# uci-rendering/psdr-cuda

Hardware: AMD Instinct MI355X
Metric: Mpath-samples/s renderC+renderD, cbox 512x512 spp=64; grad rel-L2 vs ref (higher is better)
Workload: dtype f32; 1 GPU; cbox 512x512 spp=64/GPU PathTracer(max_depth=3): renderC + configure + renderD + enoki.forward w.r.t. diffuse albedo, through the psdr_cuda surface; triangles=12, global_spp=64, world_size=1, device=AMD Radeon Graphics, local_rank=0

## Files before the change

### __graft_entry__.py

```python
import os
import subprocess
import sys

ROOT = os.path.dirname(os.path.abspath(__file__))
PKG = os.path.join(ROOT, "psdr-cuda_amd")
for p in (PKG, os.path.join(ROOT, "oracle"), os.path.join(ROOT, "tests")):
    if p not in sys.path:
        sys.path.insert(0, p)

HIPCC_FLAGS = ["--offload-arch=gfx950", "-O3", "-std=c++17", "-fPIC", "-munsafe-fp-atomics",
               "-fno-hip-fp32-correctly-rounded-divide-sqrt", "-fgpu-flush-denormals-to-zero", "-fno-slp-vectorize",
               "-freciprocal-math", "-fapprox-func"]
VARIANTS = (0, 1, 2, 3, 4, 6, 8, 10)


def _stale(target, sources):
    return (not os.path.exists(target)) or any(os.path.getmtime(s) > os.path.getmtime(target) for s in sources)


def build():
    csrc = os.path.join(PKG, "csrc")
    srcs = [os.path.join(csrc, f) for f in os.listdir(csrc)] + [os.path.join(ROOT, "include", "psdr_hip.h")]
    lib = os.path.join(PKG, "lib", "libpsdr_hip.so")
    os.makedirs(os.path.dirname(lib), exist_ok=True)
    defect_job = None
    if _stale(lib, srcs):
        obj_dir = os.path.join(PKG, "lib", "obj")
        os.makedirs(obj_dir, exist_ok=True)
        jobs, objs, unit_cmds = [], [], {}
        for v in VARIANTS:
            o = os.path.join(obj_dir, "variant%d.o" % v)
            objs.append(o)
            unit_cmds[o] = ["hipcc"] + HIPCC_FLAGS + ["-DPSDR_VARIANT_FLAGS=%d" % v, "-c", os.path.join(csrc, "psdr_variant.hip"), "-o", o]
            jobs.append(subprocess.Popen(unit_cmds[o]))
            o = os.path.join(obj_dir, "path_sedge%d.o" % v)
            objs.append(o)
            unit_cmds[o] = ["hipcc"] + HIPCC_FLAGS + ["-DPSDR_VARIANT_FLAGS=%d" % v, "-c", os.path.join(csrc, "psdr_path_sedge.hip"), "-o", o]
            jobs.append(subprocess.Popen(unit_cmds[o]))
        o = os.path.join(obj_dir, "logd_lean.o")
        objs.append(o)
        unit_cmds[o] = ["hipcc"] + HIPCC_FLAGS + ["-c", os.path.join(csrc, "psdr_logd_lean.hip"), "-o", o]
        jobs.append(subprocess.Popen(unit_cmds[o]))
        o = os.path.join(obj_dir, "host.o")
        objs.append(o)
        unit_cmds[o] = ["hipcc"] + HIPCC_FLAGS + ["-c", os.path.join(csrc, "psdr_hip.hip"), "-o", o]
        jobs.append(subprocess.Popen(unit_cmds[o]))
        o = os.path.join(obj_dir, "tables.o")
        objs.append(o)
        unit_cmds[o] = ["hipcc"] + HIPCC_FLAGS + ["-c", os.path.join(csrc, "psdr_tables.hip"), "-o", o]
        jobs.append(subprocess.Popen(unit_cmds[o]))
        defect_job = _start_defect_object(csrc, obj_dir)
        if any(j.wait() != 0 for j in jobs):
            raise RuntimeError("hipcc failed")
        sys.path.insert(0, os.path.join(ROOT, "tools"))
        import check_spill_exec
        fallbacks = (["-mllvm", "-amdgpu-opt-exec-mask-pre-ra=0"], ["-mllvm", "-amdgpu-spill-sgpr-to-vgpr=0"])
        from concurrent.futures import ThreadPoolExecutor
        with ThreadPoolExecutor(max_workers=8) as pool:
            first = dict(zip(unit_cmds, pool.map(lambda o_: check_spill_exec.check_library(o_, verbose=True, min_code_objects=1), list(unit_cmds))))
        for o, cmd in list(unit_cmds.items()):
            hits = first[o]
            for extra in fallbacks:
                if not hits:
                    break
                print("build(): %s trips the spill guard -- rebuilding it with %s" % (os.path.basename(o), " ".join(extra)))
                subprocess.check_call(cmd[:1] + cmd[1:-4] + extra + cmd[-4:])
                hits = check_spill_exec.check_library(o, verbose=True, min_code_objects=1)
            if hits:
                raise RuntimeError("%s: %d kernel(s) spill in front of an exec restore with every fallback (tools/check_spill_exec.py)" % (os.path.basename(o), len(hits)))
        subprocess.check_call(["hipcc", "--offload-arch=gfx950", "-shared", "-fPIC"] + objs + ["-o", lib])
        if len(check_spill_exec.code_objects(lib)) < len(objs):
            raise RuntimeError("the linked library holds fewer gfx code objects than translation units: the spill guard cannot see all of it")
    subprocess.check_call(["make", "-C", os.path.join(ROOT, "oracle"), "-s"])
    hc_dir = os.path.join(ROOT, "tests", "hostcheck")
    hc = os.path.join(hc_dir, "libhostcheck.so")
    if _stale(hc, srcs + [os.path.join(hc_dir, "hostcheck.cpp")]):
        subprocess.check_call(["hipcc", "--offload-arch=gfx950", "-O2", "-std=c++17", "-fPIC", "-shared", "-pthread",
                               os.path.join(hc_dir, "hostcheck.cpp"), "-o", hc])
    hp = os.path.join(hc_dir, "libhostcheck_path_sedge.so")
    if _stale(hp, srcs + [os.path.join(hc_dir, "hostcheck_path_sedge.cpp")]):
        subprocess.check_call(["hipcc", "--offload-arch=gfx950", "-O2", "-std=c++17", "-fPIC", "-shared", "-pthread",
                               os.path.join(hc_dir, "hostcheck_path_sedge.cpp"), "-o", hp])
    po_dir = os.path.join(ROOT, "tests", "poison")
    po = os.path.join(po_dir, "libpoison.so")
    if _stale(po, [os.path.join(po_dir, "poison.hip")]):
        subprocess.check_call(["hipcc", "--offload-arch=gfx950", "-O1", "-fPIC", "-shared", os.path.join(po_dir, "poison.hip"), "-o", po])
    try:
        build_defect_lib(defect_job)
    except Exception as e:
        print("build(): tests/poison/libpsdr_hip_defect.so not built (%s) -- only tests/test_rough_rev_order_gpu.py uses it" % e)
    import psdr_cuda
    from psdr_cuda import _abi
    _abi.load_hip()
    import oracle
    oracle.load_oracle()


def _defect_object_cmd(csrc, obj_dir):
    return ["hipcc"] + HIPCC_FLAGS + ["-DPSDR_VARIANT_FLAGS=10", "-DPSDR_SINK_REG_PRIV_ROUGH=1", "-DPSDR_DPP_ALWAYS=1", "-c",
                                      os.path.join(csrc, "psdr_variant.hip"), "-o", os.path.join(obj_dir, "variant10_defect.o")]


def _start_defect_object(csrc, obj_dir):
    try:
        return subprocess.Popen(_defect_object_cmd(csrc, obj_dir), stdout=subprocess.DEVNULL, stderr=subprocess.DEVNULL)
    except Exception:
        return None


def build_defect_lib(object_job=None):
    csrc = os.path.join(PKG, "csrc")
    srcs = [os.path.join(csrc, f) for f in os.listdir(csrc)] + [os.path.join(ROOT, "include", "psdr_hip.h")]
    obj_dir = os.path.join(PKG, "lib", "obj")
    defect_lib = os.path.join(ROOT, "tests", "poison", "libpsdr_hip_defect.so")
    objs = [os.path.join(obj_dir, "%s%d.o" % (unit, v)) for v in VARIANTS for unit in ("variant", "path_sedge")] + [os.path.join(obj_dir, "logd_lean.o"), os.path.join(obj_dir, "host.o"), os.path.join(obj_dir, "tables.o")]
    if not all(os.path.exists(o) for o in objs):
        return None
    if object_job is not None and object_job.wait() != 0:
        object_job = None
    if _stale(defect_lib, srcs + objs):
        defect_obj = os.path.join(obj_dir, "variant10_defect.o")
        if object_job is None:
            subprocess.check_call(_defect_object_cmd(csrc, obj_dir))
        subprocess.check_call(["hipcc", "--offload-arch=gfx950", "-shared", "-fPIC"] + [defect_obj if o.endswith("variant10.o") else o for o in objs] + ["-o", defect_lib])
    return defect_lib


def smoke():
    import numpy as np
    import torch
    assert torch.cuda.is_available(), "smoke() needs a GPU"
    torch.cuda.set_device(0)
    import oracle
    from helpers import GpuScene, load_scene, rel_l2, tangents_wrt
    from psdr_cuda import _abi
    sc, P = load_scene("cbox", res=32, spp=8, sppe=4, sppse=4, translate=(0, (1.0, 0.0, 0.0)))
    tb = sc.tables(0)
    g = GpuScene(tb)
    o = _abi.make_opts(integrator=_abi.INTEGRATOR_PATH, max_depth=3, spp=8)
    img = g.render_c(o)
    ref = oracle.render(tb, o)
    assert np.isfinite(img).all() and rel_l2(img, ref) < 1e-4, rel_l2(img, ref)
    o = _abi.make_opts(spp=8, sppe=4, sppse=4)
    tan = tangents_wrt(tb, P)
    img, dimg = g.render_d_fwd(o, [tan])
    rimg, rd = oracle.render(tb, o, mode=1, tangents=tan)
    assert rel_l2(img, rimg) < 1e-4 and rel_l2(dimg[0], rd) < 1e-3, (rel_l2(img, rimg), rel_l2(dimg[0], rd))
    import psdr_cuda
    from psdr_cuda.fixtures import scene_path
    s2 = psdr_cuda.Scene()
    s2.load_file(scene_path("cbox"), False)
    s2.opts.width = s2.opts.height = 32
    s2.opts.spp, s2.opts.sppe, s2.opts.sppse, s2.opts.log_level = 4, 0, 0, 0
    s2.configure()
    out = psdr_cuda.DirectIntegrator(1, 1).renderC(s2).numpy()
    assert out.shape == (32 * 32, 3) and np.isfinite(out).all() and out.mean() > 0.05
    print("smoke OK: renderC rel-L2 vs oracle %.2e" % rel_l2(img, rimg))


if __name__ == "__main__":
    build()
    if len(sys.argv) > 1 and sys.argv[1] == "smoke":
        smoke()
    if len(sys.argv) > 1 and sys.argv[1] == "defect":
        print(build_defect_lib())
```

### include/psdr_hip.h

```cpp
#ifndef PSDR_HIP_H
#define PSDR_HIP_H

#include <stdint.h>

#ifdef __cplusplus
extern "C" {
#endif

#define PSDR_TRI_STRIDE   24
#define PSDR_TRIUV_STRIDE  8
#define PSDR_SEDGE_STRIDE 16
#define PSDR_PEDGE_STRIDE  8
#define PSDR_BSDF_STRIDE  16
#define PSDR_EMITTER_F_STRIDE 8
#define PSDR_EMITTER_I_STRIDE 4
#define PSDR_CAM_WORDS    64
#define PSDR_ENV_WORDS    32

#define PSDR_TRI_FACE_NORMALS 0x40000000

#define PSDR_BSDF_DIFFUSE        0
#define PSDR_BSDF_ROUGHCONDUCTOR 1
#define PSDR_SLOT_REFLECTANCE 0
#define PSDR_SLOT_ALPHA_U     1
// ... 32 lines not shown
    const float   *tri_info;
    const float   *tri_uv;
    const int32_t *tri_mesh;
    const int32_t *mesh_bsdf;
    const int32_t *mesh_emitter;
    const int32_t *bsdf_rec;
    const float   *texels;
    const float   *emitter_f;
    const int32_t *emitter_i;
    const float   *face_cmf, *face_pmf;
    const float   *emitter_cmf, *emitter_pmf;
    float          emitter_sum;
    const float   *cam;
    const float   *sec_edge;
    const float   *sec_cmf, *sec_pmf;
    float          sec_sum;
    const float   *prim_edge;
    const float   *prim_cmf, *prim_pmf;
    float          prim_sum;
    int32_t        guide_reso[3];
    const float   *guide_cmf, *guide_pmf;
    float          guide_sum;
    int32_t        env_emitter;
    int32_t        env_tex[3];
    int32_t        env_reso[2];
    const float   *env_f;
    const float   *env_cmf, *env_pmf;
    float          env_sum;
    uint32_t       material_mask;
    const int32_t *sec_edge_faces;
    const float   *prim_edge_z;
} psdr_scene_desc;

#define PSDR_FLAG_FUSED     1
#define PSDR_FLAG_WAVEFRONT 2
#define PSDR_FLAG_LITERAL_FORMS 4
#define PSDR_FLAG_KEEP_RECORDS 8
#define PSDR_FLAG_PATH_SEDGES 16
#define PSDR_PATH_SEDGES_MAX_DEPTH 8

typedef struct psdr_render_opts {
    int32_t integrator;
    int32_t bsdf_samples, light_samples;
    int32_t max_depth;
    int32_t hide_emitters;
    int32_t field;
    int32_t spp, sppe, sppse;
    int32_t spp_begin, spp_end;
    int32_t sppe_begin, sppe_end;
    int32_t sppse_begin, sppse_end;
    int32_t flags;
    uint64_t rng_offset[3];
} psdr_render_opts;

typedef struct psdr_tangents {
    const float *d_tri_info;
    const float *d_texels;
    const float *d_emitter_rad;
    const float *d_cam_to_world;
    const float *d_sec_edge;
    const float *d_prim_edge;
    const float *d_env_f;
} psdr_tangents;

typedef struct psdr_grads {
    float *g_tri_info;
    float *g_texels;
    float *g_emitter_rad;
    float *g_cam_to_world;
    float *g_sec_edge;
    float *g_prim_edge;
    float *g_env_f;
} psdr_grads;

typedef struct psdr_scene_s *psdr_scene_t;

const char *psdr_last_error(void);
const char *psdr_version(void);
int psdr_abi_struct_sizes(int32_t out[4]);

int psdr_scene_create(psdr_scene_t *out);
int psdr_scene_destroy(psdr_scene_t h);
int psdr_scene_set_option(psdr_scene_t h, const char *name, double value);

int psdr_scene_set_tables(psdr_scene_t h, const psdr_scene_desc *desc);

int psdr_bvh_build(psdr_scene_t h, void *stream);
int psdr_bvh_stats(psdr_scene_t h, int32_t out[4]);
int psdr_scene_info(psdr_scene_t h, int32_t out[8]);

int psdr_trace(psdr_scene_t h, int32_t m,
               const float *ox, const float *oy, const float *oz,
               const float *dx, const float *dy, const float *dz,
               const float *tmax,
               int32_t *out_shape, int32_t *out_tri, float *out_u, float *out_v,
               void *stream);

int psdr_render_c(psdr_scene_t h, const psdr_render_opts *opts,
                  float *out_img, void *stream);

int psdr_render_d_fwd(psdr_scene_t h, const psdr_render_opts *opts,
                      int32_t K, const psdr_tangents *tangents,
                      float *out_img, float *out_dimg, void *stream);

int psdr_render_d_rev(psdr_scene_t h, const psdr_render_opts *opts,
                      const float *adj_img, float *out_img,
                      const psdr_grads *grads, void *stream);

int psdr_guide_build(psdr_scene_t h, const psdr_render_opts *opts,
                     const int32_t reso[4], int32_t nrounds,
                     float *out_mass, void *stream);

int psdr_cube_sample_reuse(int32_t ndim, const int32_t *reso, const float *cmf, const float *pmf, float sum,
                           int32_t n, int32_t m, float *samples, float *out_pdf, void *stream);
int psdr_sample_boundary_segment_direct(const psdr_scene_desc *desc, int32_t m, const float *sample3,
                                        const uint8_t *active, float *out_p0, float *out_edge_dir,
                                        float *out_edge2, float *out_p2, float *out_n, float *out_pdf,
                                        uint8_t *out_valid, int32_t *out_edge, float *out_s1, void *stream);

int psdr_geo_world_vertices_fwd(int32_t V, const float *v_raw, const int32_t *vmesh, const float *mats, float *v_world, void *stream);
int psdr_geo_world_vertices_rev(int32_t V, const float *v_raw, const int32_t *vmesh, const float *mats, const float *v_world, const float *a_world, float *a_raw,
                                void *stream);
int psdr_geo_world_vertices_jvp(int32_t V, const float *v_raw, const int32_t *vmesh, const float *mats, const float *v_world, const float *t_raw, const float *t_mats,
                                float *t_world, void *stream);
int psdr_geo_tri_rows_fwd(int32_t V, int32_t T, const float *v, const int32_t *faces, float *vsum, float *rows, int32_t row_stride, void *stream);
int psdr_geo_tri_rows_rev(int32_t V, int32_t T, const float *v, const int32_t *faces, const float *vsum, const float *a_rows, int32_t row_stride,
                          float *a_vsum , float *a_v, void *stream);
int psdr_geo_tri_rows_jvp(int32_t V, int32_t T, const float *v, const int32_t *faces, const float *vsum, const float *t_v, int32_t row_stride,
                          float *t_vsum , float *t_rows, void *stream);
int psdr_geo_sec_edges_fwd(int32_t E, const int32_t *edges, const float *v, const float *rows, int32_t row_stride, float *info, uint8_t *keep, void *stream);
int psdr_geo_sec_edges_rev(int32_t E, const int32_t *edges, const float *a_info, float *a_v, float *a_rows, int32_t row_stride, void *stream);
int psdr_geo_sec_edges_jvp(int32_t E, const int32_t *edges, const float *t_v, const float *t_rows, int32_t row_stride, float *t_info, void *stream);
int psdr_geo_prim_edges_fwd(int32_t E, const int32_t *edges, const uint8_t *face_normals, const float *v, const float *rows, int32_t row_stride,
                            const float *cam22, float *rows8, float *z4, uint8_t *keep, void *stream);
int psdr_geo_prim_edges_rev(int32_t E, const int32_t *edges, const float *v, const float *cam22, const float *a_rows8, float *a_v, float *a_w2s ,
                            void *stream);
int psdr_geo_prim_edges_jvp(int32_t E, const int32_t *edges, const float *v, const float *cam22, const float *t_v, const float *t_w2s , float *t_rows8,
                            void *stream);

int psdr_geo_compact_edges_fwd(int32_t E, const float *rows, int32_t S, const uint8_t *keep, int32_t w0, int32_t wn, const void *aux, int32_t aux_stride, int32_t A,
                               void *scratch, float *rows_out, void *aux_out, int32_t *pos, float *pmf, float *cmf, float *header, void *stream);
int psdr_geo_compact_edges_rev(int32_t E, int32_t S, const int32_t *pos, const float *a_rows_out, float *a_rows, void *stream);
int psdr_geo_compact_edges_jvp(int32_t E, int32_t S, const int32_t *pos, const float *t_rows, float *t_rows_out, void *stream);
int psdr_geo_emitter_tables(int32_t M, const float *rows, int32_t row_stride, const int32_t *face_offset, const int32_t *mesh_emitter, int32_t Ne, const int32_t *emitter_i,
                            const float *radiance, const float *env_weight, float *mesh_area, float *emitter_f, float *emitter_pmf, float *emitter_cmf, float *face_pmf,
                            float *face_cmf, void *stream);

int psdr_scene_rev_layout(psdr_scene_t h, int32_t out[16]);

int psdr_scene_seed_info(psdr_scene_t h, int64_t out[4]);

int psdr_scene_logd_info(psdr_scene_t h, int64_t out[4]);

int psdr_get_counters(psdr_scene_t h, uint64_t out[4]);

#ifdef __cplusplus
}
#endif
#endif
```

### psdr-cuda_amd/csrc/psdr_bvh_build.h

```cpp
#pragma once
#include "psdr_device.h"

#include <algorithm>
#include <cmath>
#include <cstdlib>
#include <cstring>
#include <vector>

namespace psdr {

inline void pack_tiny_prims(const std::vector<float4> &tris, std::vector<float4> &prims) {
    const int n = (int) tris.size() / 3;
    std::vector<char> used((size_t) n, 0);
    struct V { float x[3]; bool operator==(const V &o) const { return x[0] == o.x[0] && x[1] == o.x[1] && x[2] == o.x[2]; } };
    auto vtx = [&](int t, int k) {
        const float4 &a = tris[(size_t) t * 3], &b = tris[(size_t) t * 3 + 1], &c = tris[(size_t) t * 3 + 2];
        V v{{a.x, a.y, a.z}};
        if (k == 1) { v.x[0] += b.x; v.x[1] += b.y; v.x[2] += b.z; }
        if (k == 2) { v.x[0] += c.x; v.x[1] += c.y; v.x[2] += c.z; }
        return v;
    };
    auto tri_id = [&](int t) { int32_t id; std::memcpy(&id, &tris[(size_t) t * 3].w, 4); return id; };
    auto map_code = [](const int c[3], int32_t &code) {
        static const int cs[4] = {0, 1, 0, 1}, ct[4] = {0, 0, 1, 1};
// ... 48 lines not shown
            std::memcpy(&a.w, &ids, 4); std::memcpy(&b.w, &code, 4); std::memcpy(&c.w, &code, 4);
            prims.push_back(a); prims.push_back(b); prims.push_back(c);
        }
    }
}

inline int tiny_plane_form(const std::vector<float4> &prims_in, float4 *rows, int32_t *meta, int32_t *aa_cnt_out = nullptr, bool allow_aa = true, std::vector<int> *row_of_prim = nullptr) {
    const int n = (int) prims_in.size() / 3;
    struct Aa { int axis; double c, cu, cv, hu, hv, S[4]; };
    auto bits = [](const float4 &r) { int32_t v; std::memcpy(&v, &r.w, 4); return v; };
    auto classify = [&](const float4 &a, const float4 &b, const float4 &c, Aa &o) {
        if (((uint32_t) bits(a) >> 16) == 0xffffu) return false;
        const double p0[3] = {a.x, a.y, a.z}, e1[3] = {b.x, b.y, b.z}, e2[3] = {c.x, c.y, c.z};
        int i1 = -1, i2 = -1, n1 = 0, n2 = 0;
        for (int k = 0; k < 3; ++k) { if (e1[k] != 0.0) { i1 = k; n1++; } if (e2[k] != 0.0) { i2 = k; n2++; } }
        if (n1 != 1 || n2 != 1 || i1 == i2) return false;
        for (int k = 0; k < 3; ++k) if (!std::isfinite(p0[k]) || !std::isfinite(e1[k]) || !std::isfinite(e2[k])) return false;
        o.axis = 3 - i1 - i2;
        const int ia = o.axis == 0 ? 1 : 0, ib = o.axis == 2 ? 1 : 2;
        double ctr[3];
        for (int k = 0; k < 3; ++k) ctr[k] = p0[k] + 0.5 * (e1[k] + e2[k]);
        o.c = p0[o.axis]; o.cu = ctr[ia]; o.cv = ctr[ib];
        o.hu = 0.5 * std::fabs(i1 == ia ? e1[ia] : e2[ia]); o.hv = 0.5 * std::fabs(i1 == ib ? e1[ib] : e2[ib]);
        if (i1 == ia) { o.S[0] = 1.0 / e1[i1]; o.S[1] = 0.0; o.S[2] = 0.0; o.S[3] = 1.0 / e2[i2]; }
        else          { o.S[0] = 0.0; o.S[1] = 1.0 / e1[i1]; o.S[2] = 1.0 / e2[i2]; o.S[3] = 0.0; }
        return true;
    };
    std::vector<int> row_of((size_t) n, -1); std::vector<Aa> aa((size_t) n);
    int cnt[3] = {0, 0, 0};
    if (allow_aa && aa_cnt_out)
        for (int i = 0; i < n; ++i) {
            Aa &q = aa[(size_t) i];
            if (classify(prims_in[(size_t) i * 3], prims_in[(size_t) i * 3 + 1], prims_in[(size_t) i * 3 + 2], q) && cnt[q.axis] < kAaPerAxis) row_of[(size_t) i] = q.axis * kAaPerAxis + cnt[q.axis]++;
        }
    const int n_aa = cnt[0] + cnt[1] + cnt[2];
    int next = n_aa > 0 ? kAaSlots : 0;
    for (int r = 0; r < next; ++r) { for (int q = 0; q < 4; ++q) { rows[r * 4 + q] = float4{0.f, 0.f, 0.f, 0.f}; meta[r * 4 + q] = 0; } rows[r * 4].w = -1.f; }
    if (aa_cnt_out) *aa_cnt_out = cnt[0] | (cnt[1] << 8) | (cnt[2] << 16);
    for (int src = 0; src < n; ++src) {
        const bool is_aa = row_of[(size_t) src] >= 0;
        const int i = is_aa ? row_of[(size_t) src] : next++;
        const float4 &a = prims_in[(size_t) src * 3], &b = prims_in[(size_t) src * 3 + 1], &c = prims_in[(size_t) src * 3 + 2];
        int32_t ids = bits(a), codeA = bits(b), codeB = bits(c);
        const float lim = ((uint32_t) ids >> 16) != 0xffffu ? 1.f : 0.f;
        if (is_aa) {
            const Aa &q = aa[(size_t) src];
            const double A = q.S[0] + q.S[2], B = q.S[1] + q.S[3];
            if (B < 0.0) { ids = (int32_t) (((uint32_t) ids >> 16) | ((uint32_t) ids << 16)); std::swap(codeA, codeB); }
            const float rho = (float) (A / B);
            int32_t packed; std::memcpy(&packed, &rho, 4); packed = (packed & ~15) | i;
            rows[i * 4] = float4{(float) q.c, (float) q.cu, (float) q.cv, (float) q.hu};
            rows[i * 4 + 1] = float4{(float) q.hv, 0.f, 0.f, 0.f};
            std::memcpy(&rows[i * 4 + 1].y, &packed, 4); std::memcpy(&rows[i * 4 + 1].w, &ids, 4);
            rows[i * 4 + 2] = float4{(float) q.S[0], (float) q.S[1], (float) q.S[2], (float) q.S[3]};
        } else {
            const double p0[3] = {a.x, a.y, a.z}, e1[3] = {b.x, b.y, b.z}, e2[3] = {c.x, c.y, c.z};
            double nn[3] = {e1[1] * e2[2] - e1[2] * e2[1], e1[2] * e2[0] - e1[0] * e2[2], e1[0] * e2[1] - e1[1] * e2[0]};
            const double len = std::sqrt(nn[0] * nn[0] + nn[1] * nn[1] + nn[2] * nn[2]);
            double a1[3] = {0, 0, 0}, a2[3] = {0, 0, 0};
            if (len > 0.0 && std::isfinite(len)) {
                for (int k = 0; k < 3; ++k) nn[k] /= len;
                const double x1[3] = {e2[1] * nn[2] - e2[2] * nn[1], e2[2] * nn[0] - e2[0] * nn[2], e2[0] * nn[1] - e2[1] * nn[0]};
                const double x2[3] = {nn[1] * e1[2] - nn[2] * e1[1], nn[2] * e1[0] - nn[0] * e1[2], nn[0] * e1[1] - nn[1] * e1[0]};
                for (int k = 0; k < 3; ++k) { a1[k] = x1[k] / len; a2[k] = x2[k] / len; }
            } else nn[0] = nn[1] = nn[2] = 0.0;
            auto dot3 = [](const double *x, const double *y) { return x[0] * y[0] + x[1] * y[1] + x[2] * y[2]; };
            rows[i * 4] = float4{(float) nn[0], (float) nn[1], (float) nn[2], (float) dot3(nn, p0)};
            rows[i * 4 + 1] = float4{(float) a1[0], (float) a1[1], (float) a1[2], (float) (dot3(a1, p0) + 0.5)};
            rows[i * 4 + 2] = float4{(float) a2[0], (float) a2[1], (float) a2[2], (float) (dot3(a2, p0) + 0.5)};
            rows[i * 4 + 3] = float4{lim, 0.f, 0.f, 0.f}; std::memcpy(&rows[i * 4 + 3].y, &ids, 4);
        }
        meta[i * 4] = ids; meta[i * 4 + 1] = codeA; meta[i * 4 + 2] = codeB;
        std::memcpy(&meta[i * 4 + 3], &lim, 4);
        if (row_of_prim) { row_of_prim->resize((size_t) n, -1); (*row_of_prim)[(size_t) src] = i; }
    }
    return next;
}

inline uint32_t tiny_emitter_rows(const int32_t *meta, int n_rows, int32_t aa_cnt, const std::vector<char> &is_emitter_tri) {
    const int cnt[3] = {aa_cnt & 255, (aa_cnt >> 8) & 255, aa_cnt >> 16};
    size_t want = 0, found = 0;
    for (char c : is_emitter_tri) want += c ? 1 : 0;
    uint32_t rows = 0;
    for (int i = 0; i < n_rows && i < 32; ++i) {
        if (aa_cnt != 0 && i < kAaSlots && (i % kAaPerAxis) >= cnt[i / kAaPerAxis]) continue;
        const uint32_t ids = (uint32_t) meta[i * 4];
        const uint32_t t[2] = {ids & 0xffffu, ids >> 16};
        for (int a = 0; a < 2; ++a)
            if (t[a] != 0xffffu && t[a] < is_emitter_tri.size() && is_emitter_tri[t[a]]) { rows |= 1u << i; found++; }
    }
    return (want > 0 && found == want) ? rows : 0u;
}

inline void tiny_occluder_rows(const std::vector<float4> &prims, const std::vector<int> &row_of_prim, int num_tris, const std::vector<char> &is_emitter_tri,
                               std::vector<uint32_t> &occ) {
    const int n = (int) prims.size() / 3;
    occ.assign((size_t) num_tris * num_tris, 0xffffffffu);
    struct P { double c[4][3]; int nc; double nrm[3], d; int tris[2]; int row; };
    std::vector<P> ps((size_t) n);
    double scale = 0.0;
    for (int i = 0; i < n; ++i) {
        const float4 &a = prims[(size_t) i * 3], &b = prims[(size_t) i * 3 + 1], &c = prims[(size_t) i * 3 + 2];
        int32_t ids; std::memcpy(&ids, &a.w, 4);
        P &q = ps[(size_t) i];
        const bool quad = ((uint32_t) ids >> 16) != 0xffffu;
        q.tris[0] = ids & 0xffff; q.tris[1] = quad ? (int) ((uint32_t) ids >> 16) : -1;
        const double p0[3] = {a.x, a.y, a.z}, e1[3] = {b.x, b.y, b.z}, e2[3] = {c.x, c.y, c.z};
        q.nc = quad ? 4 : 3;
        for (int k = 0; k < 3; ++k) { q.c[0][k] = p0[k]; q.c[1][k] = p0[k] + e1[k]; q.c[2][k] = p0[k] + e2[k]; q.c[3][k] = p0[k] + e1[k] + e2[k]; }
        q.nrm[0] = e1[1] * e2[2] - e1[2] * e2[1]; q.nrm[1] = e1[2] * e2[0] - e1[0] * e2[2]; q.nrm[2] = e1[0] * e2[1] - e1[1] * e2[0];
        const double len = std::sqrt(q.nrm[0] * q.nrm[0] + q.nrm[1] * q.nrm[1] + q.nrm[2] * q.nrm[2]);
        for (int k = 0; k < 3; ++k) q.nrm[k] = len > 0.0 ? q.nrm[k] / len : 0.0;
        q.d = q.nrm[0] * p0[0] + q.nrm[1] * p0[1] + q.nrm[2] * p0[2];
        q.row = row_of_prim[(size_t) i];
        for (int v = 0; v < q.nc; ++v) for (int k = 0; k < 3; ++k) scale = std::max(scale, std::fabs(q.c[v][k]));
    }
    const double tol = 1e-6 * std::max(scale, 1e-30);
    int n_emitter_prims = 0;
    for (int i = 0; i < n; ++i) {
        bool em = false;
        for (int a = 0; a < 2; ++a) { const int t = ps[(size_t) i].tris[a]; em = em || (t >= 0 && t < num_tris && is_emitter_tri[(size_t) t]); }
        n_emitter_prims += em ? 1 : 0;
    }
    for (int r = 0; r < n; ++r)
        for (int e = 0; e < n; ++e) {
            uint32_t m = 1u << ps[(size_t) e].row;
            {
                const P &q = ps[(size_t) e];
                bool coplanar = true;
                for (int v = 0; v < ps[(size_t) r].nc; ++v) {
                    const double sd = q.nrm[0] * ps[(size_t) r].c[v][0] + q.nrm[1] * ps[(size_t) r].c[v][1] + q.nrm[2] * ps[(size_t) r].c[v][2] - q.d;
                    coplanar = coplanar && std::fabs(sd) <= tol;
                }
                if (coplanar && n_emitter_prims > 1) m = 0xffffffffu;
            }
            for (int p = 0; p < n; ++p) {
                if (p == e) continue;
                const P &q = ps[(size_t) p];
                double lo = 0.0, hi = 0.0;
                bool finite = true;
                auto side = [&](const P &x) { for (int v = 0; v < x.nc; ++v) { const double sd = q.nrm[0] * x.c[v][0] + q.nrm[1] * x.c[v][1] + q.nrm[2] * x.c[v][2] - q.d;
                                                                          if (!std::isfinite(sd)) finite = false; lo = std::min(lo, sd); hi = std::max(hi, sd); } };
                side(ps[(size_t) r]); side(ps[(size_t) e]);
                if (!finite || (lo < -tol && hi > tol)) m |= 1u << q.row;
            }
            for (int a = 0; a < 2; ++a)
                for (int b = 0; b < 2; ++b) {
                    const int tr = ps[(size_t) r].tris[a], te = ps[(size_t) e].tris[b];
                    if (tr >= 0 && te >= 0 && tr < num_tris && te < num_tris && is_emitter_tri[(size_t) te]) occ[(size_t) tr * num_tris + te] = m;
                }
        }
}

struct BuildTri { float lo[3], hi[3], c[3]; };
struct Builder {
    const float *rows; int T;
    std::vector<BuildTri> tris;
    std::vector<int> order;
    std::vector<BvhNode> nodes;
    std::vector<float4> btris;
    int max_depth = 0;
    float pad = 0.f;
    int kMaxLeaf = 4;
    float kTraversalCost = 2.0f;

    static float area(const float *lo, const float *hi) {
        const float dx = hi[0] - lo[0], dy = hi[1] - lo[1], dz = hi[2] - lo[2];
        return dx * dy + dy * dz + dz * dx;
    }
    void bounds(int first, int count, float *lo, float *hi, float *clo, float *chi) const {
        for (int k = 0; k < 3; ++k) { lo[k] = clo[k] = INFINITY; hi[k] = chi[k] = -INFINITY; }
        for (int i = first; i < first + count; ++i) {
            const BuildTri &t = tris[order[i]];
            for (int k = 0; k < 3; ++k) {
                lo[k] = std::min(lo[k], t.lo[k]); hi[k] = std::max(hi[k], t.hi[k]);
                clo[k] = std::min(clo[k], t.c[k]); chi[k] = std::max(chi[k], t.c[k]);
            }
        }
    }
    int32_t make_leaf(int first, int count) {
        const int base = (int) btris.size() / 3;
        for (int i = first; i < first + count; ++i) {
            const int id = order[i];
            const float *r = rows + (size_t) id * PSDR_TRI_STRIDE;
            float4 a{r[0], r[1], r[2], 0.f};
            std::memcpy(&a.w, &id, 4);
            btris.push_back(a);
            btris.push_back(float4{r[3], r[4], r[5], 0.f});
            btris.push_back(float4{r[6], r[7], r[8], 0.f});
        }
        return ~((base << 3) | (count - 1));
    }
    int32_t build(int first, int count, int depth, float *lo, float *hi) {
        float clo[3], chi[3];
        bounds(first, count, lo, hi, clo, chi);
        max_depth = std::max(max_depth, depth);
        auto leaf_here = [&]() {
            const int32_t leaf = make_leaf(first, count);
            for (int k = 0; k < 3; ++k) { lo[k] -= pad; hi[k] += pad; }
            return leaf;
        };
        if (count == 1) return leaf_here();
        int mid = -1;
        int ax = 0;
        for (int k = 1; k < 3; ++k) if (chi[k] - clo[k] > chi[ax] - clo[ax]) ax = k;
        if (depth < 20 && chi[ax] > clo[ax]) {
            constexpr int NB = 16;
            float best = INFINITY; int best_ax = -1, best_b = -1;
            for (int a = 0; a < 3; ++a) {
                if (!(chi[a] > clo[a])) continue;
                int cnt[NB] = {0}; float blo[NB][3], bhi[NB][3];
                for (int b = 0; b < NB; ++b) for (int k = 0; k < 3; ++k) { blo[b][k] = INFINITY; bhi[b][k] = -INFINITY; }
                const float scale = NB / (chi[a] - clo[a]);
                for (int i = first; i < first + count; ++i) {
                    const BuildTri &t = tris[order[i]];
                    int b = std::min(NB - 1, std::max(0, (int) ((t.c[a] - clo[a]) * scale)));
                    cnt[b]++;
                    for (int k = 0; k < 3; ++k) { blo[b][k] = std::min(blo[b][k], t.lo[k]); bhi[b][k] = std::max(bhi[b][k], t.hi[k]); }
                }
                float ra[NB]; int rc[NB];
                float lo_[3] = {INFINITY, INFINITY, INFINITY}, hi_[3] = {-INFINITY, -INFINITY, -INFINITY}; int c = 0;
                for (int b = NB - 1; b > 0; --b) {
                    for (int k = 0; k < 3; ++k) { lo_[k] = std::min(lo_[k], blo[b][k]); hi_[k] = std::max(hi_[k], bhi[b][k]); }
                    c += cnt[b]; rc[b] = c; ra[b] = c ? area(lo_, hi_) : 0.f;
                }
                for (int k = 0; k < 3; ++k) { lo_[k] = INFINITY; hi_[k] = -INFINITY; }
                c = 0;
                for (int b = 0; b < NB - 1; ++b) {
                    for (int k = 0; k < 3; ++k) { lo_[k] = std::min(lo_[k], blo[b][k]); hi_[k] = std::max(hi_[k], bhi[b][k]); }
                    c += cnt[b];
                    if (c == 0 || rc[b + 1] == 0) continue;
                    const float cost = area(lo_, hi_) * c + ra[b + 1] * rc[b + 1];
                    if (cost < best) { best = cost; best_ax = a; best_b = b; }
                }
            }
            if (count <= kMaxLeaf) {
                const float parent = area(lo, hi);
                const float split_cost = best_ax >= 0 && parent > 0.f ? kTraversalCost + best / parent : INFINITY;
                if (!(split_cost < (float) count)) return leaf_here();
            }
            if (best_ax >= 0) {
                const float scale = NB / (chi[best_ax] - clo[best_ax]);
                auto it = std::partition(order.begin() + first, order.begin() + first + count, [&](int id) {
                    int b = std::min(NB - 1, std::max(0, (int) ((tris[id].c[best_ax] - clo[best_ax]) * scale)));
                    return b <= best_b;
                });
                mid = (int) (it - order.begin());
                if (mid == first || mid == first + count) mid = -1;
            }
        }
        if (mid < 0 && count <= kMaxLeaf) return leaf_here();
        if (mid < 0) {
            mid = first + count / 2;
            std::nth_element(order.begin() + first, order.begin() + mid, order.begin() + first + count,
                             [&](int a, int b) { return tris[a].c[ax] < tris[b].c[ax]; });
        }
        const int idx = (int) nodes.size();
        nodes.push_back(BvhNode{});
        BvhNode n{};
        n.c0 = build(first, mid - first, depth + 1, n.lo0, n.hi0);
        n.c1 = build(mid, first + count - mid, depth + 1, n.lo1, n.hi1);
        nodes[idx] = n;
        return idx;
    }
    const char *run(const float *rows_, int T_, int32_t &root) {
        rows = rows_; T = T_;
        tris.resize(T); order.resize(T);
        float slo[3] = {INFINITY, INFINITY, INFINITY}, shi[3] = {-INFINITY, -INFINITY, -INFINITY};
        for (int i = 0; i < T; ++i) {
            const float *r = rows + (size_t) i * PSDR_TRI_STRIDE;
            BuildTri &t = tris[i];
            for (int k = 0; k < 3; ++k) {
                const float p = r[k], q = r[k] + r[3 + k], w = r[k] + r[6 + k];
                if (!std::isfinite(p) || !std::isfinite(q) || !std::isfinite(w)) return "psdr_bvh_build: non-finite vertex";
                t.lo[k] = std::min(p, std::min(q, w)); t.hi[k] = std::max(p, std::max(q, w));
                t.c[k] = 0.5f * (t.lo[k] + t.hi[k]);
                slo[k] = std::min(slo[k], t.lo[k]); shi[k] = std::max(shi[k], t.hi[k]);
            }
            order[i] = i;
        }
        const float ext = std::max(shi[0] - slo[0], std::max(shi[1] - slo[1], shi[2] - slo[2]));
        pad = std::max(1e-6f, 1e-5f * ext);
        nodes.clear(); btris.clear();
        nodes.reserve(T); btris.reserve((size_t) T * 3);
        float lo[3], hi[3];
        root = build(0, T, 0, lo, hi);
        if (max_depth > kBvhStack - 2) return "psdr_bvh_build: tree too deep for the traversal stack";
        if (root >= 0) {
            std::vector<int> order_bfs; order_bfs.reserve(nodes.size());
            std::vector<int> newid(nodes.size(), -1);
            order_bfs.push_back(root);
            for (size_t i = 0; i < order_bfs.size(); ++i) {
                const BvhNode &n = nodes[order_bfs[i]];
                if (n.c0 >= 0) order_bfs.push_back(n.c0);
                if (n.c1 >= 0) order_bfs.push_back(n.c1);
            }
            for (size_t i = 0; i < order_bfs.size(); ++i) newid[order_bfs[i]] = (int) i;
            std::vector<BvhNode> out(order_bfs.size());
            for (size_t i = 0; i < order_bfs.size(); ++i) {
                BvhNode n = nodes[order_bfs[i]];
                if (n.c0 >= 0) n.c0 = newid[n.c0];
                if (n.c1 >= 0) n.c1 = newid[n.c1];
                out[i] = n;
            }
            nodes.swap(out);
            root = 0;
// ... 185 lines not shown
```

### psdr-cuda_amd/csrc/psdr_hip.hip

```cpp
#define PSDR_WIDE_TREE 2
#include "psdr_host.h"
#include "psdr_bvh_build.h"

#include <cstdlib>
#include <cstring>
#include <rocprim/rocprim.hpp>

namespace {
__global__ __launch_bounds__(kBlock) void k_trace(LaunchCtx cx, int m, const float *__restrict__ ox, const float *__restrict__ oy,
                                                  const float *__restrict__ oz, const float *__restrict__ dx,
                                                  const float *__restrict__ dy, const float *__restrict__ dz,
                                                  const float *__restrict__ tmax, int32_t *__restrict__ out_shape,
                                                  int32_t *__restrict__ out_tri, float *__restrict__ out_u, float *__restrict__ out_v) {
    TraversalStack st; setup_lds(cx, st);
    const SceneView &sc = cx.sc;
    for (int i = blockIdx.x * kBlock + threadIdx.x; i < m; i += gridDim.x * kBlock) {
        const Hit h = closest_hit<false, -1>(sc, st, Vec3f{ox[i], oy[i], oz[i]}, Vec3f{dx[i], dy[i], dz[i]}, tmax[i]);
        out_tri[i] = h.tri;
        out_shape[i] = h.tri >= 0 ? (sc.d.tri_mesh[h.tri] & ~PSDR_TRI_FACE_NORMALS) : -1;
        out_u[i] = h.u; out_v[i] = h.v;
    }
}


// ... 575 lines not shown
int begin_call(psdr_scene_s *h, hipStream_t s) {
    h->last_stream = s;
    if (int rc = ensure_tree_kind(h, s)) return rc;
    h->slots[0] = h->slots[1] = h->slots[2] = 0; h->last_path_depth = 0;
    HIP_TRY(hipMemsetAsync(h->d_counters, 0, sizeof(unsigned long long) * kRayCounters * kRayCounterStride, s));
    return 0;
}


int primary_edge_order(psdr_scene_s *h, const LaunchCtx &cx, long long i0, long long n, const uint32_t **order, hipStream_t s) {
    *order = nullptr;
    if (!h->sort_edges || n < 65536 || n > 0x7fffffffLL) return 0;
    size_t temp = 0;
    const unsigned long long tiles = (unsigned long long) ((cx.sc.d.width + 7) >> 3) * (unsigned long long) ((cx.sc.d.height + 7) >> 3);
    unsigned tile_bits = 0;
    while ((1ull << tile_bits) < tiles) ++tile_bits;
    if (tile_bits + 6 >= 32) return 0;
    const unsigned end_bit = tile_bits + 7;
    const uint32_t invalid_key = 1u << (tile_bits + 6);
    uint32_t *nul = nullptr;
    HIP_TRY(rocprim::radix_sort_pairs(nullptr, temp, nul, nul, nul, nul, (size_t) n, 0, end_bit, s));
    const size_t need = 4 * sizeof(uint32_t) * (size_t) n + temp + 256;
    if (int rc = scratch_reserve(&h->d_sort, &h->sort_bytes, need, s, "primary-edge sort scratch")) return rc;
    uint32_t *k_in = reinterpret_cast<uint32_t *>(h->d_sort), *k_out = k_in + n, *v_in = k_out + n, *v_out = v_in + n;
    void *tmp = reinterpret_cast<void *>((reinterpret_cast<uintptr_t>(v_out + n) + 255) & ~(uintptr_t) 255);
    hipLaunchKernelGGL(k_primary_edge_keys, dim3((unsigned) ((n + kBlock - 1) / kBlock)), dim3(kBlock), 0, s, cx.sc, cx.jump, i0, n, k_in, v_in, invalid_key);
    HIP_TRY(hipGetLastError());
    HIP_TRY(rocprim::radix_sort_pairs(tmp, temp, k_in, k_out, v_in, v_out, (size_t) n, 0, end_bit, s));
    *order = v_out;
    return 0;
}

struct LbvhScratch {
    LbvhInfo *info; uint32_t *bounds; int32_t *node_parent, *leaf_parent; uint32_t *arrivals;
    uint32_t *keys, *keys2; int32_t *vals, *vals2; void *sort_tmp; size_t sort_tmp_bytes, total;
};
LbvhScratch lbvh_layout(void *base, int T, size_t sort_tmp_bytes) {
    LbvhScratch L{};
    size_t off = 0;
    auto take = [&](size_t bytes) { void *p = base ? (char *) base + off : nullptr; off += (bytes + 255) & ~(size_t) 255; return p; };
    L.info = (LbvhInfo *) take(sizeof(LbvhInfo)); L.bounds = (uint32_t *) take(6 * 4);
    L.node_parent = (int32_t *) take((size_t) T * 4); L.leaf_parent = (int32_t *) take((size_t) T * 4);
    L.arrivals = (uint32_t *) take((size_t) T * 4);
    L.keys = (uint32_t *) take((size_t) T * 4); L.keys2 = (uint32_t *) take((size_t) T * 4);
    L.vals = (int32_t *) take((size_t) T * 4); L.vals2 = (int32_t *) take((size_t) T * 4);
    L.sort_tmp = take(sort_tmp_bytes); L.sort_tmp_bytes = sort_tmp_bytes;
    L.total = off;
    return L;
}
int lbvh_fit(psdr_scene_s *h, const LbvhScratch &L, float pad, hipStream_t s) {
    const int T = h->desc.num_tris;
    HIP_TRY(hipMemsetAsync(L.arrivals, 0, (size_t) T * 4, s));
    HIP_TRY(hipMemsetAsync(h->d_refit_area, 0, sizeof(float), s));
    hipLaunchKernelGGL(k_lbvh_fit, dim3((T + kBlock - 1) / kBlock), dim3(kBlock), 0, s, T, h->d_nodes, h->d_btris, L.node_parent, L.leaf_parent, L.arrivals,
                       h->d_refit_area, pad);
    HIP_TRY(hipGetLastError());
    return 0;
}
int lbvh_refit(psdr_scene_s *h, hipStream_t s) {
    const int T = h->tree_tris;
    const LbvhScratch L = lbvh_layout(h->d_lbvh, T, 0);
    hipLaunchKernelGGL(k_refit_leaves, dim3((T + kBlock - 1) / kBlock), dim3(kBlock), 0, s, h->d_btris, h->desc.tri_info, T);
    return lbvh_fit(h, L, h->bvh_pad, s);
}
int lbvh_build(psdr_scene_s *h, hipStream_t s, bool &fallback) {
    const int T = h->desc.num_tris;
    fallback = T <= kLbvhLeaf;
    if (fallback) return 0;
    size_t t1 = 0, t2 = 0;
    uint32_t *nk = nullptr; int32_t *nv = nullptr;
    HIP_TRY(rocprim::radix_sort_pairs(nullptr, t1, nk, nk, nv, nv, (size_t) T, 0, 30, s));
    HIP_TRY(rocprim::radix_sort_pairs_desc(nullptr, t2, nk, nk, nv, nv, (size_t) T, 0, 32, s));
    const size_t sort_tmp = std::max(t1, t2);
    const size_t need = lbvh_layout(nullptr, T, sort_tmp).total;
    if (need > h->lbvh_bytes) {
        if (h->d_lbvh) (void) hipFree(h->d_lbvh);
        h->d_lbvh = nullptr; h->lbvh_bytes = 0;
        HIP_TRY(hipMalloc(&h->d_lbvh, need));
        h->lbvh_bytes = need;
    }
    const LbvhScratch L = lbvh_layout(h->d_lbvh, T, sort_tmp);
    if ((size_t) (T - 1) > h->cap_nodes) {
        if (h->d_nodes) (void) hipFree(h->d_nodes);
        h->cap_nodes = std::max<size_t>((size_t) T, 16);
        HIP_TRY(hipMalloc(&h->d_nodes, h->cap_nodes * sizeof(BvhNode)));
    }
    if ((size_t) T * 3 > h->cap_btris) {
        if (h->d_btris) (void) hipFree(h->d_btris);
        h->cap_btris = (size_t) T * 3;
        HIP_TRY(hipMalloc(&h->d_btris, h->cap_btris * sizeof(float4)));
    }
    if (!h->d_refit_area) HIP_TRY(hipMalloc(&h->d_refit_area, sizeof(float)));
    const dim3 gT((T + kBlock - 1) / kBlock), blk(kBlock);
    HIP_TRY(hipMemsetAsync(L.info, 0, sizeof(LbvhInfo), s));
    HIP_TRY(hipMemsetAsync(L.bounds, 0xff, 3 * 4, s));
    HIP_TRY(hipMemsetAsync(L.bounds + 3, 0, 3 * 4, s));
    hipLaunchKernelGGL(k_lbvh_bounds, gT, blk, 0, s, h->desc.tri_info, T, L.bounds, L.info);
    hipLaunchKernelGGL(k_lbvh_codes, gT, blk, 0, s, h->desc.tri_info, T, L.bounds, L.keys, L.vals, L.info);
    HIP_TRY(hipGetLastError());
    size_t tmp_bytes = L.sort_tmp_bytes;
    HIP_TRY(rocprim::radix_sort_pairs(L.sort_tmp, tmp_bytes, L.keys, L.keys2, L.vals, L.vals2, (size_t) T, 0, 30, s));
    HIP_TRY(hipMemsetAsync(L.leaf_parent, 0xff, (size_t) T * 4, s));
    hipLaunchKernelGGL(k_lbvh_tris, gT, blk, 0, s, h->desc.tri_info, T, L.vals2, h->d_btris);
    hipLaunchKernelGGL(k_lbvh_hierarchy, gT, blk, 0, s, L.keys2, T, h->d_nodes, L.node_parent, L.leaf_parent);
    HIP_TRY(hipGetLastError());
    LbvhInfo info{};
    HIP_TRY(hipMemcpyAsync(&info, L.info, sizeof(info), hipMemcpyDeviceToHost, s));
    HIP_TRY(hipStreamSynchronize(s));
    if (info.bad) return fail("psdr_bvh_build: non-finite vertex");
    if (int rc = lbvh_fit(h, L, info.pad, s)) return rc;
    hipLaunchKernelGGL(k_lbvh_depth, gT, blk, 0, s, T, L.node_parent, L.leaf_parent, L.info);
    constexpr int kMaxHotRows = 200;
    hipLaunchKernelGGL(k_lbvh_area_keys, gT, blk, 0, s, h->desc.tri_info, T, L.keys, L.vals);
    HIP_TRY(hipGetLastError());
    tmp_bytes = L.sort_tmp_bytes;
    HIP_TRY(rocprim::radix_sort_pairs_desc(L.sort_tmp, tmp_bytes, L.keys, L.keys2, L.vals, L.vals2, (size_t) T, 0, 32, s));
    float area = 0.f;
    const int top = std::min(T, kMaxHotRows);
    std::vector<int32_t> by_area((size_t) top);
    HIP_TRY(hipMemcpyAsync(&info, L.info, sizeof(info), hipMemcpyDeviceToHost, s));
    HIP_TRY(hipMemcpyAsync(&area, h->d_refit_area, sizeof(float), hipMemcpyDeviceToHost, s));
    HIP_TRY(hipMemcpyAsync(by_area.data(), L.vals2, (size_t) top * 4, hipMemcpyDeviceToHost, s));
    h->emitter_i.assign((size_t) std::max(h->desc.num_emitters, 0) * PSDR_EMITTER_I_STRIDE, 0);
    if (h->desc.num_emitters > 0 && h->desc.emitter_i)
        HIP_TRY(hipMemcpyAsync(h->emitter_i.data(), h->desc.emitter_i, h->emitter_i.size() * sizeof(int32_t), hipMemcpyDeviceToHost, s));
    HIP_TRY(hipStreamSynchronize(s));
    if (info.depth > kBvhStack - 2) { fallback = true; return 0; }
    std::vector<int32_t> tris;
    {
        auto add = [&](int t) {
            if (t < 0 || t >= T || (int) tris.size() >= kMaxHotRows) return;
            if (std::find(tris.begin(), tris.end(), t) == tris.end()) tris.push_back(t);
        };
        for (int e = 0; e < h->desc.num_emitters; ++e) {
            const int32_t *ei = h->emitter_i.data() + (size_t) e * PSDR_EMITTER_I_STRIDE;
            for (int f = 0; f < ei[2] && f < 64; ++f) add(ei[1] + f);
        }
        for (int i = 0; i < top; ++i) add(by_area[(size_t) i]);
    }
    if ((size_t) T > h->hot_cap) {
        if (h->d_hot_map) (void) hipFree(h->d_hot_map);
        if (h->d_hot_tris) (void) hipFree(h->d_hot_tris);
        h->hot_cap = (size_t) T;
        HIP_TRY(hipMalloc(&h->d_hot_map, h->hot_cap * sizeof(int32_t)));
        HIP_TRY(hipMalloc(&h->d_hot_tris, kMaxHotRows * sizeof(int32_t)));
    }
    HIP_TRY(hipMemsetAsync(h->d_hot_map, 0xff, (size_t) T * sizeof(int32_t), s));
    HIP_TRY(hipMemcpyAsync(h->d_hot_tris, tris.data(), tris.size() * sizeof(int32_t), hipMemcpyHostToDevice, s));
    hipLaunchKernelGGL(k_scatter_hot, dim3(1), dim3(256), 0, s, h->d_hot_map, h->d_hot_tris, (int) tris.size());
    HIP_TRY(hipGetLastError());
    HIP_TRY(hipStreamSynchronize(s));
    h->hot_rows = (int) tris.size(); h->hot_identity = false;
    h->root = 0; h->bvh_depth = info.depth; h->num_nodes = T - 1; h->num_btris = T;
    h->n_tiny = 0; h->aa_cnt = 0; h->n_blas = 0; h->n_inline = 0; h->have_occ = false; h->emit_rows = 0;
    if (use_wide_tree(h, false)) {
        std::vector<BvhNode> host_nodes((size_t) T - 1);
        HIP_TRY(hipMemcpyAsync(host_nodes.data(), h->d_nodes, host_nodes.size() * sizeof(BvhNode), hipMemcpyDeviceToHost, s));
        HIP_TRY(hipStreamSynchronize(s));
        if (int rc = bvh4_build(h, host_nodes, std::vector<int32_t>{0}, false, s)) return rc;
    } else { h->wide = false; h->num_nodes4 = 0; h->stack_need4 = 0; }
    h->tree_tris = T; h->refits_since_build = 0; h->num_builds++; h->bvh_pad = info.pad; h->built_area = area;
    h->level_start.clear();
    h->refit_ok = true; h->lbvh = true; h->have_bvh = true;
    return 0;
}

int bvh4_refill(psdr_scene_s *h, hipStream_t s) {
    if (h->num_nodes4 <= 0) return 0;
    hipLaunchKernelGGL(k_bvh4_fill, dim3((h->num_nodes4 + kBlock - 1) / kBlock), dim3(kBlock), 0, s, h->d_nodes4, h->d_nodes, h->d_topo4,
                       h->d_topo4 + (size_t) h->num_nodes4 * 4, h->num_nodes4);
    HIP_TRY(hipGetLastError());
    return 0;
}
int bvh4_build(psdr_scene_s *h, const std::vector<BvhNode> &nodes, const std::vector<int32_t> &roots2, bool forest, hipStream_t s) {
    h->wide = use_wide_tree(h, forest);
    if (!h->wide && !forest) { h->num_nodes4 = 0; h->stack_need4 = 0; return 0; }
    Bvh4Topology tp;
    collapse_bvh4(nodes, roots2, tp);
    h->num_nodes4 = tp.n4; h->stack_need4 = tp.stack_need;
    h->root4 = roots2.size() == 1 ? tp.roots[0] : 0;
    for (size_t k = 0; k < roots2.size() && k < (size_t) kMaxBlas; ++k) h->blas_root4[k] = tp.roots[k];
    if (tp.n4 == 0) return 0;
    if ((size_t) tp.n4 > h->cap_nodes4) {
        if (h->d_nodes4) (void) hipFree(h->d_nodes4);
        if (h->d_topo4) (void) hipFree(h->d_topo4);
        h->d_nodes4 = nullptr; h->d_topo4 = nullptr;
        h->cap_nodes4 = (size_t) tp.n4;
        HIP_TRY(hipMalloc(&h->d_nodes4, h->cap_nodes4 * sizeof(Bvh4Node)));
        HIP_TRY(hipMalloc(&h->d_topo4, h->cap_nodes4 * 8 * sizeof(int32_t)));
    }
    HIP_TRY(hipMemcpyAsync(h->d_topo4, tp.child.data(), (size_t) tp.n4 * 4 * sizeof(int32_t), hipMemcpyHostToDevice, s));
    HIP_TRY(hipMemcpyAsync(h->d_topo4 + (size_t) tp.n4 * 4, tp.src.data(), (size_t) tp.n4 * 4 * sizeof(int32_t), hipMemcpyHostToDevice, s));
    if (int rc = bvh4_refill(h, s)) return rc;
    HIP_TRY(hipStreamSynchronize(s));
    return 0;
}

bool traced_wavefront(const psdr_scene_s *h) { return h->traced_enabled && h->n_blas > 0 && h->num_nodes4 > 0 && h->d_nodes4 != nullptr; }
int launch_wf_trace(psdr_scene_s *h, const float4 *req, const int32_t *count, long long sub_cap, float4 *hit, hipStream_t s, bool ign) {
    TraceArgs a{};
    a.sec_edge_faces = h->desc.sec_edge_faces;
    if (ign && !a.sec_edge_faces) ign = false;
    std::memcpy(a.blas_lo, h->blas_lo, sizeof(a.blas_lo));
    std::memcpy(a.blas_hi, h->blas_hi, sizeof(a.blas_hi));
    for (int k = 0; k < h->n_blas; ++k) std::memcpy(&a.blas_hi[k].w, &h->blas_root4[k], 4);
    a.nodes4 = h->d_nodes4; a.btris = h->d_btris; a.req = req; a.count = count; a.hit = hit; a.sub_cap = sub_cap; a.n_blas = h->n_blas;
    const int full_S = std::min(h->stack_need4, kTraceStackMax);
    const bool tree_fits = (long long) h->num_nodes4 * kTraceNodeStride + (long long) (full_S + 1) * kTraceBlock * 4 + 1024 <= (long long) h->lds_limit;
    const bool wg2 = h->lds_limit >= 160 * 1024 && (h->opt.trace_wg2 > 0 || (h->opt.trace_wg2 < 0 && (!tree_fits || sub_cap * kWfSub >= (1ll << 25))));
    const int S = std::min(h->stack_need4, wg2 ? std::min(h->opt.trace_wg2 > 0 ? h->opt.trace_wg2 : 8, kTraceStackMax) : kTraceStackMax);
    const bool ovf = h->stack_need4 > S;
    const int stack_bytes = (S + 1) * kTraceBlock * 4;
    const int room = (wg2 ? h->lds_limit / 2 : h->lds_limit) - 1024 - stack_bytes;
    a.n_lnodes = std::max(0, std::min(h->num_nodes4, room / kTraceNodeStride));
    a.off_stack = a.n_lnodes * kTraceNodeStride;
    a.stack_entries = S;
    const int grid = wg2 ? 2 * h->num_cus : h->num_cus;
    if (ovf) {
        a.ovf_stride = grid * kTraceBlock;
        const size_t need = (size_t) a.ovf_stride * (size_t) (h->stack_need4 - S) * sizeof(int32_t);
        if (int rc = scratch_reserve(reinterpret_cast<void **>(&h->d_trace_ovf), &h->trace_ovf_bytes, need, s, "trace kernel's overflow stack columns")) return rc;
        a.ovf = h->d_trace_ovf;
    }
    const int dyn = a.off_stack + stack_bytes;
#define PSDR_LAUNCH_TRACE_I(MULTI, OVF, IGN, WPE)                                                                                                           \
    do { static bool attr_set = false;                                                                                                                      \
         if (!attr_set) { HIP_TRY(hipFuncSetAttribute(reinterpret_cast<const void *>(&k_wf_trace<MULTI, OVF, IGN, WPE>), hipFuncAttributeMaxDynamicSharedMemorySize, 160 * 1024 - 1024)); attr_set = true; } \
         hipLaunchKernelGGL(HIP_KERNEL_NAME(k_wf_trace<MULTI, OVF, IGN, WPE>), dim3(grid), dim3(kTraceBlock), dyn, s, a); } while (0)
#define PSDR_LAUNCH_TRACE(MULTI, OVF) do { if (ign) { if (wg2) PSDR_LAUNCH_TRACE_I(MULTI, OVF, true, 8); else PSDR_LAUNCH_TRACE_I(MULTI, OVF, true, 4); } else if (wg2) PSDR_LAUNCH_TRACE_I(MULTI, OVF, false, 8); else PSDR_LAUNCH_TRACE_I(MULTI, OVF, false, 4); } while (0)
    if (h->n_blas > 1) { if (ovf) PSDR_LAUNCH_TRACE(true, true); else PSDR_LAUNCH_TRACE(true, false); }
    else { if (ovf) PSDR_LAUNCH_TRACE(false, true); else PSDR_LAUNCH_TRACE(false, false); }
#undef PSDR_LAUNCH_TRACE_I
#undef PSDR_LAUNCH_TRACE
    HIP_TRY(hipGetLastError());
    return 0;
}

int probe_buffers(psdr_scene_s *h, long long slots, int rays_per_slot, ProbeBuffers &pb, hipStream_t s, int per_cu) {
    const long long rays = slots * rays_per_slot;
    const long long blocks = ((long long) launch_blocks(h, slots, per_cu) + kWfSub - 1) / kWfSub * kWfSub;
    const long long trips = (slots + blocks * kBlock - 1) / (blocks * kBlock);
    pb.sub_cap = (blocks / kWfSub) * trips * kBlock * rays_per_slot;
    const size_t cnt_bytes = (size_t) kWfSub * kWfCountStride * sizeof(int32_t);
    const size_t need = cnt_bytes + (size_t) rays * sizeof(float4) + (((size_t) slots * 4 + 255) & ~(size_t) 255) + (size_t) 2 * pb.sub_cap * kWfSub * sizeof(float4);
    if (int rc = scratch_reserve(&h->d_probe, &h->probe_bytes, need, s, "probe buffers (hit rows, masks, trace requests)")) return rc;
    char *p = reinterpret_cast<char *>(h->d_probe);
    pb.count = reinterpret_cast<int32_t *>(p); p += cnt_bytes;
    pb.hit = reinterpret_cast<float4 *>(p); p += (size_t) rays * sizeof(float4);
    pb.mask = reinterpret_cast<uint32_t *>(p); p += ((size_t) slots * 4 + 255) & ~(size_t) 255;
    pb.req = reinterpret_cast<float4 *>(p);
    HIP_TRY(hipMemsetAsync(pb.count, 0, cnt_bytes, s));
    return 0;
}

const VariantOps *variant_of(const psdr_scene_s *h) {
    int fl = (h->desc.env_emitter >= 0 ? kSceneEnv : 0) | (h->has_rough ? kSceneRough : 0) | (h->n_blas > 0 ? kSceneForest : 0);
    if (tiny_tables_ok(h)) fl |= kSceneTiny;
    switch (fl) {
        case 0: return variant_ops_0();
        case 1: return variant_ops_1();
        case 2: return variant_ops_2();
        case 3: return variant_ops_3();
        case 4: return variant_ops_4();
        case 8: return variant_ops_8();
        case 10: return variant_ops_10();
        default: return variant_ops_6();
    }
}
const PathSedgeOps *path_sedge_of(const psdr_scene_s *h) {
    int fl = (h->desc.env_emitter >= 0 ? kSceneEnv : 0) | (h->has_rough ? kSceneRough : 0) | (h->n_blas > 0 ? kSceneForest : 0);
    if (tiny_tables_ok(h)) fl |= kSceneTiny;
    switch (fl) {
        case 0: return path_sedge_ops_0();
        case 1: return path_sedge_ops_1();
        case 2: return path_sedge_ops_2();
        case 3: return path_sedge_ops_3();
        case 4: return path_sedge_ops_4();
        case 8: return path_sedge_ops_8();
        case 10: return path_sedge_ops_10();
        default: return path_sedge_ops_6();
    }
}
}
using namespace psdr_host;

extern "C" {

const char *psdr_last_error(void) { return g_err.c_str(); }
const char *psdr_version(void) { return "psdr-hip 0.1 gfx950"; }
int psdr_abi_struct_sizes(int32_t out[4]) {
    out[0] = (int32_t) sizeof(psdr_scene_desc); out[1] = (int32_t) sizeof(psdr_render_opts);
    out[2] = (int32_t) sizeof(psdr_tangents); out[3] = (int32_t) sizeof(psdr_grads);
    return 0;
}

int psdr_scene_create(psdr_scene_t *out) {
    if (!out) return fail("psdr_scene_create: null output");
    psdr_scene_s *h = new psdr_scene_s();
    hipError_t e = hipMalloc(&h->d_counters, sizeof(unsigned long long) * kRayCounters * kRayCounterStride);
    if (e != hipSuccess) { delete h; return fail(std::string("hipMalloc: ") + hipGetErrorString(e)); }
    int dev = 0; hipDeviceProp_t prop;
    if (hipGetDevice(&dev) == hipSuccess && hipGetDeviceProperties(&prop, dev) == hipSuccess) {
        h->num_cus = prop.multiProcessorCount;
        h->lds_limit = (int) std::min<size_t>(prop.sharedMemPerBlock, 160 * 1024);
    }
    *out = h;
    return 0;
}

int psdr_scene_set_option(psdr_scene_t h, const char *name, double value) {
    if (!h || !name) return fail("psdr_scene_set_option: null argument");
    const std::string n(name);
    const int iv = (int) value;
    if (n == "bvh_refit") h->refit_enabled = iv != 0;
    else if (n == "forest_min_inline") { h->forest_min_inline = iv; h->have_bvh = false; }
    else if (n == "scratch_plain") g_scratch_plain = iv;
    else if (n == "own_pixels") h->opt.own_pixels = iv;
    else if (n == "emitter_pretest") h->opt.emitter_pretest = iv;
    else if (n == "occ_rows") { h->opt.occ_rows = iv; h->have_bvh = false; }
    else if (n == "aa_prims") { h->aa_enabled = iv != 0; h->have_bvh = false; }
    else if (n == "tiny_scene") h->tiny_enabled = iv != 0;
    else if (n == "two_level") h->two_level_enabled = iv != 0;
    else if (n == "wf_binned") h->wf_binned = iv != 0;
    else if (n == "wf_traced") h->traced_enabled = iv != 0;
    else if (n == "bvh_build") h->bvh_device_mode = iv;
    else if (n == "sort_edges") h->sort_edges = iv != 0;
    else if (n == "blocks_per_cu") h->opt.blocks_per_cu = iv;
    else if (n == "camera_blocks") h->opt.camera_blocks = iv;
    else if (n == "tiny_variants") h->opt.tiny_variants = iv;
    else if (n == "wide") h->opt.wide = iv;
    else if (n == "lds_budget") h->opt.lds_budget = iv;
    else if (n == "sink_rep") h->opt.sink_rep = std::max(1, std::min(16, iv));
    else if (n == "sink_private") h->opt.sink_private = iv;
    else if (n == "rev_split") h->opt.rev_split = iv;
    else if (n == "tangent_live") h->opt.tangent_live = iv;
    else if (n == "wf_geo") h->opt.wf_geo = iv;
    else if (n == "logd") h->opt.logd = iv;
    else if (n == "seed_cache") h->opt.seed_cache = iv;
    else if (n == "logd_park") h->opt.logd_park = iv;
    else if (n == "seed_cache_log2") h->opt.seed_cache_log2 = std::max(0, std::min(40, iv));
    else if (n == "keep_records") h->opt.keep_records = iv;
    else if (n == "rev_sorted") h->opt.rev_sorted = iv;
    else if (n == "sedge_split") h->opt.sedge_split = iv;
    else if (n == "pt_sedge") h->opt.pt_sedge = iv & 3;
    else if (n == "pt_sedge_walk") h->opt.pt_sedge_walk = iv;
    else if (n == "probe") h->opt.probe = iv;
    else if (n == "trace_wg2") h->opt.trace_wg2 = iv;
    else if (n == "chunk_log2") h->opt.chunk_log2 = std::max(0, std::min(30, iv));
    else if (n == "bvh_maxleaf") h->opt.bvh_maxleaf = std::max(1, std::min(8, iv));
    else if (n == "bvh_tcost") h->opt.bvh_tcost = (float) value;
    else return fail("psdr_scene_set_option: unknown option '" + n + "'");
    h->kept.valid = false;
    if (n == "tiny_scene" || n == "two_level" || n == "bvh_build" || n == "wide" || n == "bvh_maxleaf" || n == "bvh_tcost" || n == "tiny_variants") h->have_bvh = false;
    return 0;
}

int psdr_scene_destroy(psdr_scene_t h) {
    if (!h) return 0;
    if (h->d_nodes) (void) hipFree(h->d_nodes);
    if (h->d_btris) (void) hipFree(h->d_btris);
    if (h->d_counters) (void) hipFree(h->d_counters);
    if (h->d_refit_area) (void) hipFree(h->d_refit_area);
    if (h->d_sort) (void) hipFree(h->d_sort);
    if (h->d_ws) (void) hipFree(h->d_ws);
    if (h->d_live) (void) hipFree(h->d_live);
    if (h->d_logd_bad) (void) hipFree(h->d_logd_bad);
    if (h->d_seed) (void) hipFree(h->d_seed);
    if (h->seed_event) (void) hipEventDestroy(h->seed_event);
    if (h->d_hot_map) (void) hipFree(h->d_hot_map);
    if (h->d_hot_tris) (void) hipFree(h->d_hot_tris);
    if (h->d_occ) (void) hipFree(h->d_occ);
    if (h->d_top) (void) hipFree(h->d_top);
    if (h->d_inline_ids) (void) hipFree(h->d_inline_ids);
    if (h->d_lbvh) (void) hipFree(h->d_lbvh);
    if (h->d_nodes4) (void) hipFree(h->d_nodes4);
    if (h->d_topo4) (void) hipFree(h->d_topo4);
    if (h->d_rev) (void) hipFree(h->d_rev);
    if (h->d_se_list) (void) hipFree(h->d_se_list);
    if (h->d_rev_deep) (void) hipFree(h->d_rev_deep);
    if (h->d_pe_rep) (void) hipFree(h->d_pe_rep);
    if (h->d_trace_ovf) (void) hipFree(h->d_trace_ovf);
    if (h->d_probe) (void) hipFree(h->d_probe);
    delete h;
    return 0;
}

int psdr_scene_set_tables(psdr_scene_t h, const psdr_scene_desc *desc) {
    if (!h || !desc) return fail("psdr_scene_set_tables: null argument");
    psdr_scene_desc d = *desc;
    if (d.num_tris <= 0 || !d.tri_info || !d.tri_mesh) return fail("Missing meshes!");
    if (!d.cam) return fail("Missing sensor!");
    if (reinterpret_cast<uintptr_t>(d.tri_info) & 15) return fail("psdr_scene_set_tables: tri_info must be 16-byte aligned");
    if (d.width <= 0 || d.height <= 0) return fail("Invalid film resolution");
    if (d.num_meshes <= 0 || !d.mesh_bsdf || !d.mesh_emitter) return fail("psdr_scene_set_tables: mesh_bsdf / mesh_emitter missing");
    if (d.num_bsdfs > 0 && (!d.bsdf_rec || !d.texels)) return fail("psdr_scene_set_tables: bsdf_rec / texels missing");
    if (d.num_emitters > 0 && (!d.emitter_f || !d.emitter_i)) return fail("psdr_scene_set_tables: emitter tables missing");
    if (d.num_emitters > 1 && (!d.emitter_cmf || !d.emitter_pmf)) return fail("psdr_scene_set_tables: emitter distribution missing");
    if (d.num_sec_edges > 0 && (!d.sec_edge || !d.sec_cmf || !d.sec_pmf)) return fail("psdr_scene_set_tables: secondary-edge tables missing");
    if (d.num_prim_edges > 0 && (!d.prim_edge || !d.prim_cmf || !d.prim_pmf)) return fail("psdr_scene_set_tables: primary-edge tables missing");
    if (d.num_prim_edges <= 0) d.prim_edge_z = nullptr;
    if (d.num_guide_cells > 0 && (!d.guide_cmf || !d.guide_pmf)) return fail("psdr_scene_set_tables: guiding tables missing");
    if (!d.env_f) d.env_emitter = -1;
    if (d.env_emitter >= 0) {
        if (d.env_emitter >= d.num_emitters || !d.env_cmf || !d.env_pmf || d.env_reso[0] <= 0 || d.env_reso[1] <= 0 || d.env_tex[1] < 2 ||
            d.env_tex[2] < 2)
            return fail("psdr_scene_set_tables: inconsistent environment-map record");
    }
    if (h->have_tables && (d.tri_info != h->desc.tri_info || d.num_tris != h->desc.num_tris)) h->have_bvh = false;
    if (h->have_tables && (d.emitter_i != h->desc.emitter_i || d.num_emitters != h->desc.num_emitters)) h->have_bvh = false;
    if (!h->have_tables || std::memcmp(&h->desc, &d, sizeof(d)) != 0) { ++h->tables_gen; h->kept.valid = false; }
    h->desc = d;
    h->has_rough = d.material_mask == 0 || (d.material_mask & (1u << PSDR_BSDF_ROUGHCONDUCTOR)) != 0;
    h->have_tables = true;
    return 0;
}

static hipError_t copy_on_stream(void *dst, const void *src, size_t bytes, hipMemcpyKind kind, hipStream_t s) {
    if (hipError_t e = hipMemcpyAsync(dst, src, bytes, kind, s)) return e;
    return hipStreamSynchronize(s);
}
static void update_emit_rows(psdr_scene_s *h) {
    std::vector<char> is_em((size_t) std::max(h->desc.num_tris, 0), 0);
    for (int e = 0; e < h->desc.num_emitters && (size_t) (e + 1) * PSDR_EMITTER_I_STRIDE <= h->emitter_i.size(); ++e) {
        const int32_t *ei = h->emitter_i.data() + (size_t) e * PSDR_EMITTER_I_STRIDE;
        if (e == h->desc.env_emitter) { h->emit_rows = 0; return; }
        for (int f = 0; f < ei[2]; ++f) if (ei[1] + f >= 0 && ei[1] + f < h->desc.num_tris) is_em[(size_t) (ei[1] + f)] = 1;
    }
    h->emit_rows = h->n_tiny > 0 ? tiny_emitter_rows(h->tiny_meta, h->n_tiny, h->aa_cnt, is_em) : 0u;
}
int psdr_bvh_build(psdr_scene_t h, void *stream) {
    if (!h || !h->have_tables) return fail("Scene not loaded yet!");
    hipStream_t s = (hipStream_t) stream;
    const int T = h->desc.num_tris;
    h->kept.valid = false;
    const bool tiny = h->tiny_enabled && T <= kTinyTris;
    bool emitters_same = (size_t) std::max(h->desc.num_emitters, 0) * PSDR_EMITTER_I_STRIDE == h->emitter_i.size();
    if (emitters_same && !h->emitter_i.empty() && h->refit_enabled && !tiny && h->refit_ok && h->tree_tris == T && h->num_nodes > 0) {
        std::vector<int32_t> now(h->emitter_i.size());
        emitters_same = h->desc.emitter_i != nullptr;
        if (emitters_same) {
            HIP_TRY(copy_on_stream(now.data(), h->desc.emitter_i, now.size() * sizeof(int32_t), hipMemcpyDeviceToHost, s));
            emitters_same = std::memcmp(now.data(), h->emitter_i.data(), now.size() * sizeof(int32_t)) == 0;
        }
    }
    const bool forest_stands = !(forest_tables(h) && !small_tables_fit(h));
    if (h->refit_enabled && !tiny && h->refit_ok && emitters_same && forest_stands && h->tree_tris == T && h->num_nodes > 0 && h->refits_since_build < kMaxRefits) {
        float prev_area = h->built_area;
        if (h->refits_since_build > 0) {
            HIP_TRY(hipMemcpyAsync(&prev_area, h->d_refit_area, sizeof(float), hipMemcpyDeviceToHost, h->refit_stream));
            HIP_TRY(hipStreamSynchronize(h->refit_stream));
        }
        if (prev_area <= kRefitAreaGrowth * h->built_area && h->lbvh) {
            h->refit_stream = s;
            if (int rc = lbvh_refit(h, s)) return rc;
            if (int rc = bvh4_refill(h, s)) return rc;
            h->refits_since_build++;
            h->num_refits++;
            h->have_bvh = true;
            return 0;
        }
        if (prev_area <= kRefitAreaGrowth * h->built_area) {
            bool refit_fits = true;
            h->refit_stream = s;
            HIP_TRY(hipMemsetAsync(h->d_refit_area, 0, sizeof(float), s));
            hipLaunchKernelGGL(k_refit_leaves, dim3((h->num_btris + kBlock - 1) / kBlock), dim3(kBlock), 0, s, h->d_btris, h->desc.tri_info, h->num_btris);
            for (int l = (int) h->level_start.size() - 2; l >= 0; --l) {
                const int first = h->level_start[l], count = h->level_start[l + 1] - first;
                hipLaunchKernelGGL(k_refit_level, dim3((count + kBlock - 1) / kBlock), dim3(kBlock), 0, s, h->d_nodes, h->d_btris, first, count, h->bvh_pad,
                                   h->d_refit_area);
            }
            HIP_TRY(hipGetLastError());
            if (int rc = bvh4_refill(h, s)) return rc;
            if (h->n_blas > 0) {
                float4 top[kMaxInlineTris * 3 + 2 * kMaxBlas];
                hipLaunchKernelGGL(k_gather_top, dim3(1), dim3(64), 0, s, h->d_top, h->d_nodes, h->desc.tri_info, h->d_inline_ids, h->n_inline, h->n_blas);
                HIP_TRY(hipMemcpyAsync(top, h->d_top, sizeof(top), hipMemcpyDeviceToHost, s));
                HIP_TRY(hipStreamSynchronize(s));
                std::vector<float4> tris(top, top + 3 * (size_t) h->n_inline), prims;
                pack_tiny_prims(tris, prims);
                refit_fits = (int) prims.size() / 3 <= kTinyTris;
                if (refit_fits) {
                    h->n_tiny = tiny_plane_form(prims, h->tiny, h->tiny_meta, &h->aa_cnt, h->aa_enabled);
                    update_emit_rows(h);
                    for (int k = 0; k < h->n_blas; ++k) {
                        const float w = h->blas_lo[k].w;
                        h->blas_lo[k] = top[kMaxInlineTris * 3 + k]; h->blas_lo[k].w = w;
                        h->blas_hi[k] = top[kMaxInlineTris * 3 + kMaxBlas + k];
                    }
                }
            }
            if (refit_fits) {
                h->refits_since_build++;
                h->num_refits++;
                h->have_bvh = true;
                return 0;
            }
        }
    }
    h->lbvh = false;
    if (!tiny && (h->bvh_device_mode == 1 || (h->bvh_device_mode < 0 && T >= kLbvhAutoTris))) {
        bool fallback = false;
        if (int rc = lbvh_build(h, s, fallback)) return rc;
        if (!fallback) return 0;
    }
    std::vector<float> rows((size_t) T * PSDR_TRI_STRIDE);
    HIP_TRY(hipMemcpyAsync(rows.data(), h->desc.tri_info, rows.size() * sizeof(float), hipMemcpyDeviceToHost, s));
    HIP_TRY(hipStreamSynchronize(s));
    h->emitter_i.assign((size_t) std::max(h->desc.num_emitters, 0) * PSDR_EMITTER_I_STRIDE, 0);
    if (h->desc.num_emitters > 0 && h->desc.emitter_i)
        HIP_TRY(copy_on_stream(h->emitter_i.data(), h->desc.emitter_i, h->emitter_i.size() * sizeof(int32_t), hipMemcpyDeviceToHost, s));
    std::vector<int32_t> tri_mesh;
    bool forest = false;
    if (h->two_level_enabled && h->tiny_enabled && T > kTinyTris && h->desc.num_meshes > 0 && h->desc.env_emitter < 0) {
        tri_mesh.resize((size_t) T);
        HIP_TRY(copy_on_stream(tri_mesh.data(), h->desc.tri_mesh, tri_mesh.size() * sizeof(int32_t), hipMemcpyDeviceToHost, s));
        forest = ForestBuilder::eligible(tri_mesh.data(), T, h->desc.num_meshes) && (!PSDR_FOREST_LDS_TABLES || small_tables_fit(h));
    }
    Builder b;
    ForestBuilder fb;
    b.kMaxLeaf = fb.max_leaf = h->opt.bvh_maxleaf; b.kTraversalCost = fb.traversal_cost = h->opt.bvh_tcost;
    std::vector<float4> top_prims;
    int32_t root = 0;
    if (forest) {
        if (const char *err = fb.run(rows.data(), tri_mesh.data(), T, h->desc.num_meshes)) return fail(err);
        pack_tiny_prims(fb.inline_tris, top_prims);
        if ((int) top_prims.size() / 3 > kTinyTris || (int) fb.inline_tris.size() / 3 < h->forest_min_inline) { forest = false; fb = ForestBuilder(); }
    }
    if (!forest) { if (const char *err = b.run(rows.data(), T, root)) return fail(err); }
    std::vector<BvhNode> &nodes = forest ? fb.nodes : b.nodes;
    std::vector<float4> &btris = forest ? fb.btris : b.btris;
    if (nodes.size() > h->cap_nodes) {
        if (h->d_nodes) (void) hipFree(h->d_nodes);
        h->cap_nodes = std::max<size_t>(nodes.size(), 16);
        HIP_TRY(hipMalloc(&h->d_nodes, h->cap_nodes * sizeof(BvhNode)));
    }
    if (btris.size() > h->cap_btris) {
        if (h->d_btris) (void) hipFree(h->d_btris);
        h->cap_btris = btris.size();
        HIP_TRY(hipMalloc(&h->d_btris, h->cap_btris * sizeof(float4)));
    }
    if (!nodes.empty()) HIP_TRY(hipMemcpyAsync(h->d_nodes, nodes.data(), nodes.size() * sizeof(BvhNode), hipMemcpyHostToDevice, s));
    HIP_TRY(hipMemcpyAsync(h->d_btris, btris.data(), btris.size() * sizeof(float4), hipMemcpyHostToDevice, s));
    HIP_TRY(hipStreamSynchronize(s));
    {
        constexpr int kMaxHotRows = 200;
        std::vector<int32_t> map((size_t) T, -1), tris;
        auto add = [&](int t) { if (t >= 0 && t < T && map[t] < 0 && (int) tris.size() < kMaxHotRows) { map[t] = (int32_t) tris.size(); tris.push_back(t); } };
        h->hot_identity = tiny;
        if (tiny) for (int t = 0; t < T; ++t) add(t);
        for (int e = 0; e < h->desc.num_emitters; ++e) {
            const int32_t *ei = h->emitter_i.data() + (size_t) e * PSDR_EMITTER_I_STRIDE;
            for (int f = 0; f < ei[2] && f < 64; ++f) add(ei[1] + f);
        }
        std::vector<int> by_area((size_t) T);
        for (int i = 0; i < T; ++i) by_area[i] = i;
        const int top = std::min(T, kMaxHotRows);
        std::partial_sort(by_area.begin(), by_area.begin() + top, by_area.end(),
                          [&](int a, int c) { return rows[(size_t) a * PSDR_TRI_STRIDE + 21] > rows[(size_t) c * PSDR_TRI_STRIDE + 21]; });
        for (int i = 0; i < top; ++i) add(by_area[i]);
        if ((size_t) T > h->hot_cap) {
            if (h->d_hot_map) (void) hipFree(h->d_hot_map);
            if (h->d_hot_tris) (void) hipFree(h->d_hot_tris);
            h->hot_cap = (size_t) T;
            HIP_TRY(hipMalloc(&h->d_hot_map, h->hot_cap * sizeof(int32_t)));
            HIP_TRY(hipMalloc(&h->d_hot_tris, kMaxHotRows * sizeof(int32_t)));
        }
        HIP_TRY(copy_on_stream(h->d_hot_map, map.data(), map.size() * sizeof(int32_t), hipMemcpyHostToDevice, s));
        HIP_TRY(copy_on_stream(h->d_hot_tris, tris.data(), tris.size() * sizeof(int32_t), hipMemcpyHostToDevice, s));
        h->hot_rows = (int) tris.size();
    }
    h->root = root;
    h->bvh_depth = forest ? fb.max_depth : b.max_depth; h->num_nodes = (int) nodes.size(); h->num_btris = (int) btris.size() / 3;
    if (int rc = bvh4_build(h, nodes, forest ? fb.roots : std::vector<int32_t>{root}, forest, s)) return rc;
    h->have_bvh = true;
    h->n_tiny = 0; h->aa_cnt = 0; h->n_blas = 0; h->n_inline = 0; h->have_occ = false; h->emit_rows = 0;
    if (forest) {
        h->n_tiny = tiny_plane_form(top_prims, h->tiny, h->tiny_meta, &h->aa_cnt, h->aa_enabled);
        update_emit_rows(h);
        h->n_inline = (int) fb.inline_ids.size();
        h->n_blas = (int) fb.roots.size();
        for (int k = 0; k < h->n_blas; ++k) {
            float lo[3], hi[3];
            fb.tree_box(k, lo, hi);
            h->blas_lo[k] = float4{lo[0], lo[1], lo[2], 0.f}; h->blas_hi[k] = float4{hi[0], hi[1], hi[2], 0.f};
            std::memcpy(&h->blas_lo[k].w, &fb.roots[(size_t) k], 4);
        }
        if (!h->d_top) HIP_TRY(hipMalloc(&h->d_top, sizeof(float4) * (kMaxInlineTris * 3 + 2 * kMaxBlas)));
        if (!h->d_inline_ids) HIP_TRY(hipMalloc(&h->d_inline_ids, sizeof(int32_t) * kMaxInlineTris));
        if (h->n_inline) HIP_TRY(copy_on_stream(h->d_inline_ids, fb.inline_ids.data(), sizeof(int32_t) * (size_t) h->n_inline, hipMemcpyHostToDevice, s));
    } else if (tiny) {
        std::vector<float4> prims;
        std::vector<int> row_of_prim;
        pack_tiny_prims(b.btris, prims);
        h->n_tiny = tiny_plane_form(prims, h->tiny, h->tiny_meta, &h->aa_cnt, h->aa_enabled, &row_of_prim);
        update_emit_rows(h);
        h->have_occ = false;
        if (T <= 32 && h->n_tiny <= 32) {
            std::vector<char> is_em((size_t) T, 0);
            for (int e = 0; e < h->desc.num_emitters; ++e) {
                const int32_t *ei = h->emitter_i.data() + (size_t) e * PSDR_EMITTER_I_STRIDE;
                for (int f = 0; f < ei[2]; ++f) if (ei[1] + f >= 0 && ei[1] + f < T) is_em[(size_t) (ei[1] + f)] = 1;
            }
            std::vector<uint32_t> occ;
            if (h->opt.occ_rows != 0) tiny_occluder_rows(prims, row_of_prim, T, is_em, occ);
            else occ.assign((size_t) T * T, 0xffffffffu);
            if (occ.size() > h->occ_cap) {
                if (h->d_occ) (void) hipFree(h->d_occ);
                h->occ_cap = std::max<size_t>(occ.size(), 32 * 32);
                HIP_TRY(hipMalloc(&h->d_occ, h->occ_cap * sizeof(uint32_t)));
            }
            HIP_TRY(copy_on_stream(h->d_occ, occ.data(), occ.size() * sizeof(uint32_t), hipMemcpyHostToDevice, s));
            h->have_occ = true;
            h->occ_max_rows = 0;
            for (int r = 0; r < T; ++r) for (int e = 0; e < T; ++e) if (is_em[(size_t) e]) h->occ_max_rows = std::max(h->occ_max_rows, (int) __builtin_popcount(occ[(size_t) r * T + e] & ((1u << h->n_tiny) - 1u)));
        }
    }
    h->tree_tris = T; h->refits_since_build = 0; h->num_builds++; h->bvh_pad = forest ? fb.pad : b.pad;
    h->level_start.clear();
    double area = 0.0;
    auto node_area = [](const BvhNode &n) {
        const float dx = std::max(n.hi0[0], n.hi1[0]) - std::min(n.lo0[0], n.lo1[0]), dy = std::max(n.hi0[1], n.hi1[1]) - std::min(n.lo0[1], n.lo1[1]),
                    dz = std::max(n.hi0[2], n.hi1[2]) - std::min(n.lo0[2], n.lo1[2]);
        return (double) (dx * dy + dy * dz + dz * dx);
    };
    if (forest) {
        h->level_start = fb.level_start;
        for (const BvhNode &n : nodes) area += node_area(n);
    } else if (root >= 0) {
        std::vector<int> depth(b.nodes.size(), 0);
        for (size_t i = 0; i < b.nodes.size(); ++i) {
            const BvhNode &n = b.nodes[i];
            if (n.c0 >= 0) depth[n.c0] = depth[i] + 1;
            if (n.c1 >= 0) depth[n.c1] = depth[i] + 1;
            if (i == 0 || depth[i] != depth[i - 1]) h->level_start.push_back((int) i);
            area += node_area(n);
        }
        h->level_start.push_back((int) b.nodes.size());
    }
    h->refit_ok = true;
    if (forest) for (int32_t r : fb.roots) if (r < 0) h->refit_ok = false;
    h->built_area = (float) area;
    if (!h->d_refit_area) HIP_TRY(hipMalloc(&h->d_refit_area, sizeof(float)));
    return 0;
}

int psdr_trace(psdr_scene_t h, int32_t m, const float *ox, const float *oy, const float *oz, const float *dx, const float *dy,
               const float *dz, const float *tmax, int32_t *out_shape, int32_t *out_tri, float *out_u, float *out_v, void *stream) {
    if (!h || !h->have_tables) return fail("Scene not loaded yet!");
    if (!h->have_bvh) return fail("Input scene must be configured!");
    if (m <= 0) return 0;
    LaunchCtx cx{};
    cx.sc.d = h->desc; cx.sc.nodes = h->d_nodes; cx.sc.btris = h->d_btris; cx.sc.root = h->root;
    fill_top(h, cx.sc);
    plan_lds(h, cx);
    hipLaunchKernelGGL(k_trace, dim3(launch_blocks(h, m)), dim3(kBlock), lds_bytes(cx, h), (hipStream_t) stream, cx, m, ox, oy, oz, dx, dy, dz, tmax,
                       out_shape, out_tri, out_u, out_v);
    HIP_TRY(hipGetLastError());
    return 0;
}

int psdr_render_c(psdr_scene_t h, const psdr_render_opts *o, float *out_img, void *stream) {
    if (!h || !o || !out_img) return fail("psdr_render_c: null argument");
    if (!h->have_tables) return fail("Scene not loaded yet!");
    if (int rc = check_counts(h, o)) return rc;
    hipStream_t s = (hipStream_t) stream;
    if (int rc = begin_call(h, s)) return rc;
    if (o->integrator == PSDR_INTEGRATOR_PATH) h->last_path_depth = o->max_depth;
    const long long WH = (long long) h->desc.width * h->desc.height;
    HIP_TRY(hipMemsetAsync(out_img, 0, sizeof(float) * WH * 3, s));
    return variant_of(h)->render_c(h, o, out_img, s);
}

int psdr_render_d_fwd(psdr_scene_t h, const psdr_render_opts *o, int32_t K, const psdr_tangents *tangents, float *out_img,
                      float *out_dimg, void *stream) {
    if (!h || !o || !out_img || !out_dimg || !tangents) return fail("psdr_render_d_fwd: null argument");
    if (!h->have_tables) return fail("Scene not loaded yet!");
    if (int rc = check_counts(h, o)) return rc;
    if (int rc = check_path_sedges(o)) return rc;
    hipStream_t s = (hipStream_t) stream;
    if (int rc = begin_call(h, s)) return rc;
    if (K != 1 && K != 3) return fail("psdr_render_d_fwd: K must be 1 or 3");
    if (int rc = variant_of(h)->render_fwd(h, o, K, tangents, out_img, out_dimg, s)) return rc;
    return path_sedge_of(h)->fwd(h, o, K, tangents, out_dimg, s);
}

int psdr_render_d_rev(psdr_scene_t h, const psdr_render_opts *o, const float *adj_img, float *out_img, const psdr_grads *grads,
                      void *stream) {
    if (!h || !o || !adj_img || !grads) return fail("psdr_render_d_rev: null argument");
    if (!h->have_tables) return fail("Scene not loaded yet!");
    if (int rc = check_counts(h, o)) return rc;
    if (int rc = check_path_sedges(o)) return rc;
    if (o->flags & PSDR_FLAG_LITERAL_FORMS) return fail("psdr_render_d_rev: PSDR_FLAG_LITERAL_FORMS is a forward-mode diagnostic (no literal-form adjoint)");
    if (o->integrator == PSDR_INTEGRATOR_PATH && o->max_depth > kMaxRevDepthDeep)
        return fail("psdr_render_d_rev: PathTracer max_depth > 250 is not supported in reverse mode");
    hipStream_t s = (hipStream_t) stream;
    if (int rc = begin_call(h, s)) return rc;
    std::fill(std::begin(h->rev_layout), std::end(h->rev_layout), 0);
    h->rev_layout[8] = -1;
    if (int rc = variant_of(h)->render_rev(h, o, adj_img, out_img, grads, s)) return rc;
    return path_sedge_of(h)->rev(h, o, adj_img, grads, s);
}

int psdr_guide_build(psdr_scene_t h, const psdr_render_opts *o, const int32_t reso[4], int32_t nrounds, float *out_mass, void *stream) {
    if (!h || !o || !reso || !out_mass) return fail("psdr_guide_build: null argument");
    if (nrounds <= 0) return fail("psdr_guide_build: nrounds must be positive");
    if (h->desc.num_sec_edges <= 0) return fail("psdr_guide_build: scene has no secondary edges");
    hipStream_t s = (hipStream_t) stream;
    if (int rc = begin_call(h, s)) return rc;
    LaunchCtx cx;
    if (int rc = make_ctx(h, o, 2, cx)) return rc;
    cx.sc.d.guide_cmf = nullptr; cx.sc.d.num_guide_cells = 0;
    const long long cells = (long long) reso[0] * reso[1] * reso[2];
    const long long n = cells * reso[3];
    if (n <= 0 || n > 0x7fffffffLL) return fail("psdr_guide_build: invalid resolution");
    HIP_TRY(hipMemsetAsync(out_mass, 0, sizeof(float) * cells, s));
    return variant_of(h)->guide(h, cx, reso, nrounds, n, out_mass, s);
}

int psdr_cube_sample_reuse(int32_t ndim, const int32_t *reso, const float *cmf, const float *pmf, float sum, int32_t n, int32_t m, float *samples,
                           float *out_pdf, void *stream) {
    if (!reso || !cmf || !pmf || !samples || !out_pdf) return fail("psdr_cube_sample_reuse: null argument");
    if (ndim != 2 && ndim != 3) return fail("psdr_cube_sample_reuse: ndim must be 2 or 3");
    long long cells = 1;
    for (int d = 0; d < ndim; ++d) {
        if (reso[d] <= 0) return fail("psdr_cube_sample_reuse: invalid resolution");
        cells *= reso[d];
    }
    if (cells != (long long) n) return fail("psdr_cube_sample_reuse: n must be the product of the resolution");
    if (m < 0) return fail("psdr_cube_sample_reuse: negative sample count");
    if (m == 0) return 0;
    const dim3 grid((unsigned) ((m + kBlock - 1) / kBlock));
    hipStream_t s = (hipStream_t) stream;
    if (ndim == 2)
        hipLaunchKernelGGL(k_cube_sample_reuse<2>, grid, dim3(kBlock), 0, s, m, cmf, pmf, sum, n, reso[0], reso[1], 1, samples, out_pdf);
    else
        hipLaunchKernelGGL(k_cube_sample_reuse<3>, grid, dim3(kBlock), 0, s, m, cmf, pmf, sum, n, reso[0], reso[1], reso[2], samples, out_pdf);
    HIP_TRY(hipGetLastError());
    return 0;
}

int psdr_sample_boundary_segment_direct(const psdr_scene_desc *desc, int32_t m, const float *sample3, const uint8_t *active, float *out_p0,
                                        float *out_edge_dir, float *out_edge2, float *out_p2, float *out_n, float *out_pdf, uint8_t *out_valid,
                                        int32_t *out_edge, float *out_s1, void *stream) {
    if (!desc || !sample3 || !out_p0 || !out_edge_dir || !out_edge2 || !out_p2 || !out_n || !out_pdf || !out_valid || !out_edge || !out_s1)
        return fail("psdr_sample_boundary_segment_direct: null argument");
    const psdr_scene_desc &d = *desc;
    if (d.num_sec_edges <= 0 || !d.sec_edge || !d.sec_cmf || !d.sec_pmf) return fail("Scene has no secondary edges");
    if (d.num_emitters <= 0 || !d.emitter_f || !d.emitter_i) return fail("No Emitter!");
    if (d.num_emitters > 1 && (!d.emitter_cmf || !d.emitter_pmf)) return fail("psdr_sample_boundary_segment_direct: emitter distribution missing");
    const bool env = d.env_f != nullptr && d.env_emitter >= 0;
    if (env && (d.env_emitter >= d.num_emitters || !d.env_cmf || !d.env_pmf || d.env_reso[0] <= 0 || d.env_reso[1] <= 0))
        return fail("psdr_sample_boundary_segment_direct: inconsistent environment-map record");
    if (d.num_emitters > (env ? 1 : 0) && (d.num_tris <= 0 || !d.tri_info || !d.face_cmf || !d.face_pmf))
        return fail("psdr_sample_boundary_segment_direct: area-light tables missing");
    if (m < 0) return fail("psdr_sample_boundary_segment_direct: negative sample count");
    if (m == 0) return 0;
    SceneView sc{};
    sc.d = d;
    if (!env) sc.d.env_emitter = -1;
    const dim3 grid((unsigned) ((m + kBlock - 1) / kBlock));
    hipStream_t s = (hipStream_t) stream;
    if (env)
        hipLaunchKernelGGL(k_boundary_segment_direct<kSceneEnv>, grid, dim3(kBlock), 0, s, sc, m, sample3, active, out_p0, out_edge_dir, out_edge2, out_p2, out_n,
                           out_pdf, out_valid, out_edge, out_s1);
    else
        hipLaunchKernelGGL(k_boundary_segment_direct<0>, grid, dim3(kBlock), 0, s, sc, m, sample3, active, out_p0, out_edge_dir, out_edge2, out_p2, out_n,
                           out_pdf, out_valid, out_edge, out_s1);
    HIP_TRY(hipGetLastError());
    return 0;
}

int psdr_bvh_stats(psdr_scene_t h, int32_t out[4]) {
    if (!h || !out) return fail("psdr_bvh_stats: null argument");
    out[0] = h->num_builds; out[1] = h->num_refits; out[2] = h->num_nodes; out[3] = h->bvh_depth;
    return 0;
}

int psdr_scene_info(psdr_scene_t h, int32_t out[8]) {
    if (!h || !out) return fail("psdr_scene_info: null argument");
    const int n_slab = (h->aa_cnt & 255) + ((h->aa_cnt >> 8) & 255) + (h->aa_cnt >> 16);
    out[0] = h->n_tiny - (h->aa_cnt != 0 ? kAaSlots - n_slab : 0); out[1] = h->n_blas; out[2] = h->n_inline; out[3] = h->num_btris; out[4] = h->lbvh ? 1 : 0;
    out[5] = n_slab; out[6] = h->have_occ ? 1 : 0; out[7] = h->have_occ ? h->occ_max_rows : 0;
    return 0;
}

int psdr_scene_rev_layout(psdr_scene_t h, int32_t out[16]) {
    if (!h || !out) return fail("psdr_scene_rev_layout: null argument");
    std::copy(std::begin(h->rev_layout), std::end(h->rev_layout), out);
    return 0;
}

int psdr_scene_logd_info(psdr_scene_t h, int64_t out[4]) {
    if (!h || !out) return fail("psdr_scene_logd_info: null argument");
    out[0] = h->logd_launches; out[1] = h->logd_lean_launches; out[2] = h->logd_lean_seeded; out[3] = (int64_t) h->logd_lean_lds + h->logd_lean_park;
    return 0;
}
int psdr_scene_seed_info(psdr_scene_t h, int64_t out[4]) {
    if (!h || !out) return fail("psdr_scene_seed_info: null argument");
    out[0] = h->seed_valid ? h->seed_key[0] * h->seed_key[3] : 0; out[1] = (int64_t) (h->seed_cap * sizeof(ulonglong2)); out[2] = h->seed_fills; out[3] = h->seed_launches;
    return 0;
}

int psdr_get_counters(psdr_scene_t h, uint64_t out[4]) {
    if (!h || !out) return fail("psdr_get_counters: null argument");
    unsigned long long all[kRayCounters * kRayCounterStride], c[1] = {0};
    HIP_TRY(hipMemcpyAsync(all, h->d_counters, sizeof(all), hipMemcpyDeviceToHost, h->last_stream));
    HIP_TRY(hipStreamSynchronize(h->last_stream));
    for (int i = 0; i < kRayCounters; ++i) c[0] += all[i * kRayCounterStride];
#ifdef PSDR_STAGE_CLOCKS
    {
        unsigned long long ph[12] = {0};
        for (int i = 0; i < kRayCounters; ++i) for (int k = 0; k < 12; ++k) ph[k] += all[i * kRayCounterStride + 1 + k];
        std::fprintf(stderr, "stage clocks:");
        for (int k = 0; k < 12; ++k) std::fprintf(stderr, " %llu", ph[k]);
        std::fprintf(stderr, "\n");
    }
#endif
    out[0] = c[0]; out[1] = h->slots[0]; out[2] = h->slots[1]; out[3] = h->slots[2];
    return 0;
}

}
```

### psdr-cuda_amd/csrc/psdr_host.h

```cpp
#pragma once
#include "psdr_device.h"
#include "psdr_reverse.h"

#include <algorithm>
#include <type_traits>
#include <cmath>
#include <cstdio>
#include <cstdlib>
#include <cstring>
#include <string>
#include <vector>

using namespace psdr;

struct LaunchCtx {
    SceneView sc;
    LiParams lp;
    RngJump jump;
    int32_t off_stack;
    int32_t off_pathrec;
    int32_t off_sink;
    int32_t off_park;
};

static_assert(offsetof(LaunchCtx, sc) == 0, "closest_hit reads SceneView::tiny through the kernel-argument segment pointer: LaunchCtx (SceneView first) must be the first kernel argument");

__device__ __forceinline__ void setup_lds(const LaunchCtx &cx, TraversalStack &st) {
#if defined(__HIP_DEVICE_COMPILE__)
    const SceneView &sc = cx.sc;
    float4 *dst = reinterpret_cast<float4 *>(psdr_dyn_lds);
    const float4 *src = sc.nodes4 != nullptr ? reinterpret_cast<const float4 *>(sc.nodes4) : reinterpret_cast<const float4 *>(sc.nodes);
    for (int i = threadIdx.x; i < sc.n_lnodes * 4; i += kBlock) dst[sc.off_lnodes / 16 + (i >> 2) * (kLdsNodeStride / 16) + (i & 3)] = src[i];
    for (int i = threadIdx.x; i < sc.n_lbtris * 3; i += kBlock) dst[sc.off_lbtris / 16 + i] = sc.btris[i];
    src = reinterpret_cast<const float4 *>(sc.d.tri_info);
    for (int i = threadIdx.x; i < sc.n_ltri * 6; i += kBlock) dst[sc.off_ltri / 16 + i] = src[i];
    {
        float *m = reinterpret_cast<float *>(psdr_dyn_lds + sc.off_lprim);
#pragma unroll 1
        for (int i = 0; i < sc.n_tiny; ++i) {
            int32_t tri; float k[6];
            const int w = threadIdx.x & 7;
            const float4 Sm = sc.tiny[i * 4 + 2];
            const float S[4] = {Sm.x, Sm.y, Sm.z, Sm.w};
            tiny_hit_row(sc.tiny_meta + i * 4, (threadIdx.x >> 3) & 1, tri, k, (sc.aa_cnt != 0 && i < kAaSlots) ? S : nullptr);
            const float val = w == 0 ? __int_as_float(tri) : (w == 1 ? k[0] : w == 2 ? k[1] : w == 3 ? k[2] : w == 4 ? k[3] : w == 5 ? k[4] : w == 6 ? k[5] : 0.f);
            if (threadIdx.x < kTinyHitWords) m[i * kTinyHitWords + threadIdx.x] = val;
        }
    }
    if (sc.lt_meshbsdf >= 0) {
        auto stage = [&](int off, const void *table, int words) {
            if (off < 0 || table == nullptr) return;
            const uint32_t *g = static_cast<const uint32_t *>(table);
            uint32_t *l = reinterpret_cast<uint32_t *>(psdr_dyn_lds + off);
#pragma unroll 1
            for (int i = threadIdx.x; i < words; i += kBlock) l[i] = g[i];
        };
        stage(sc.lt_trimesh, sc.d.tri_mesh, sc.d.num_tris);
        stage(sc.lt_meshbsdf, sc.d.mesh_bsdf, sc.d.num_meshes);
        stage(sc.lt_meshemitter, sc.d.mesh_emitter, sc.d.num_meshes);
        stage(sc.lt_bsdf, sc.d.bsdf_rec, sc.d.num_bsdfs * PSDR_BSDF_STRIDE);
        stage(sc.lt_emf, sc.d.emitter_f, sc.d.num_emitters * PSDR_EMITTER_F_STRIDE);
        stage(sc.lt_emi, sc.d.emitter_i, sc.d.num_emitters * PSDR_EMITTER_I_STRIDE);
        stage(sc.lt_ecmf, sc.d.emitter_cmf, sc.d.num_emitters);
        stage(sc.lt_epmf, sc.d.emitter_pmf, sc.d.num_emitters);
        stage(sc.lt_fcmf, sc.d.face_cmf, sc.lt_nfaces);
        stage(sc.lt_fpmf, sc.d.face_pmf, sc.lt_nfaces);
        stage(sc.lt_uv, sc.d.tri_uv, sc.d.num_tris * PSDR_TRIUV_STRIDE);
        stage(sc.lt_tex, sc.d.texels, sc.d.num_texels);
        stage(sc.lt_occ, sc.occ, sc.d.num_tris * sc.d.num_tris);
    }
    st.base = reinterpret_cast<int32_t *>(psdr_dyn_lds + cx.off_stack) + threadIdx.x;
    __syncthreads();
#else
    (void) cx; (void) st;
#endif
}
template <class TVT> __device__ __forceinline__ void setup_lds(const LaunchCtx &cx, TraversalStack &st, const TVT &tv) {
    setup_lds(cx, st);
#if defined(__HIP_DEVICE_COMPILE__)
    if constexpr (Tab<TVT::flags>::lds_small && TVT::k > 0) {
        constexpr int K = TVT::k;
        static_assert(K <= 3, "plan_lds reserves three tangent texel pools");
        if (cx.sc.lt_tex >= 0) {
            float *l = reinterpret_cast<float *>(psdr_dyn_lds + cx.sc.lt_tex);
            const int nt = cx.sc.d.num_texels;
            for (int k = 0; k < K; ++k) {
                const float *g = tv.t[k].d_texels;
                for (int i = threadIdx.x; i < nt; i += kBlock) l[(k + 1) * nt + i] = g ? g[i] : 0.f;
            }
            __syncthreads();
        }
    }
#endif
}

constexpr int kSinkCacheWords = 6144;
struct SinkLayout {
    int tex_off, tex_n;
    int rad_off, rad_n;
    int cam_off;
    int env_off, env_n;
    int hot_off, hot_rows;
    const int32_t *hot_map, *hot_tris;
    int total;
    int rep, stride;
    int priv_off, priv_rows;
    int priv_tri[2], priv_slot[2], priv_emitter;
    int priv_regs;
    int pend_off, pend_rows;
};
constexpr int kPendWords = 10;
constexpr int kPrivRowWords = 13;
constexpr int kPrivWords = 2 * kPrivRowWords + 3;

struct psdr_scene_options {
    int blocks_per_cu = 0;
    int camera_blocks = 0;
    int tiny_variants = 1;
    int wide = -1;
    int lds_budget = 0;
    int sink_rep = 4;
    int sink_private = 1;
    int rev_split = -1;
    int tangent_live = 1;
    int wf_geo = 1;
    int own_pixels = 1;
    int emitter_pretest = 1;
    int occ_rows = 1;
    int logd = 1;
    int keep_records = 1;
    int rev_sorted = 1;
    int pt_sedge = 3;
    int pt_sedge_walk = 1;
    int sedge_split = -1;
    int chunk_log2 = 0;
    int probe = 1;
    int trace_wg2 = -1;
    int seed_cache = 1;
    int seed_cache_log2 = 25;
    int logd_park = 1;
    int bvh_maxleaf = 4;
    float bvh_tcost = 2.0f;
};

struct psdr_scene_s {
    psdr_scene_options opt;
    psdr_scene_desc desc{};
    bool have_tables = false;
    bool has_rough = true;
    int num_cus = 256;
    int lds_limit = 64 * 1024;

    BvhNode *d_nodes = nullptr;
    float4 *d_btris = nullptr;
    size_t cap_nodes = 0, cap_btris = 0;
    int32_t root = 0;
    bool have_bvh = false;
    int bvh_depth = 0, num_nodes = 0, num_btris = 0;
    Bvh4Node *d_nodes4 = nullptr;
    int32_t *d_topo4 = nullptr;
    size_t cap_nodes4 = 0;
    int num_nodes4 = 0, stack_need4 = 0;
    bool wide = false;
    int32_t *d_trace_ovf = nullptr;
    size_t trace_ovf_bytes = 0;
    bool traced_enabled = true;
    int32_t root4 = 0, blas_root4[kMaxBlas] = {};
    bool refit_enabled = true;
    int tree_tris = -1, refits_since_build = 0, num_builds = 0, num_refits = 0;
    std::vector<int> level_start;
    float bvh_pad = 0.f, built_area = 0.f;
    float *d_refit_area = nullptr;

    int bvh_device_mode = -1;
    bool lbvh = false;
    int lbvh_leaves = 0;
    void *d_lbvh = nullptr;
    size_t lbvh_bytes = 0;

    bool tiny_enabled = true, aa_enabled = true;
    int n_tiny = 0, aa_cnt = 0;
    float4 tiny[kTinyRows * 4] = {};
    int32_t tiny_meta[kTinyRows * 4] = {};
    bool two_level_enabled = true, refit_ok = true, wf_binned = true;
    int n_blas = 0, n_inline = 0;
    float4 blas_lo[kMaxBlas] = {}, blas_hi[kMaxBlas] = {};
    float4 *d_top = nullptr;
    int32_t *d_inline_ids = nullptr;

    unsigned long long *d_counters = nullptr;
    hipStream_t last_stream = nullptr;
    hipStream_t refit_stream = nullptr;
    uint64_t slots[3] = {0, 0, 0};
    int last_path_depth = 0;
    int32_t rev_layout[16] = {};

    std::vector<int32_t> emitter_i;
    int32_t *d_hot_map = nullptr, *d_hot_tris = nullptr;
    uint32_t *d_occ = nullptr; size_t occ_cap = 0; bool have_occ = false; int occ_max_rows = 0;
    int hot_rows = 0;
    bool hot_identity = false;
    size_t hot_cap = 0;

    bool sort_edges = true;
    void *d_sort = nullptr;
    size_t sort_bytes = 0;

    void *d_pe_rep = nullptr;
    size_t pe_rep_bytes = 0;

    void *d_rev_deep = nullptr;
    size_t rev_deep_bytes = 0;

    void *d_se_list = nullptr;
    size_t se_list_bytes = 0;

    void *d_rev = nullptr;
    size_t rev_bytes = 0;
    void *d_logd_bad = nullptr; size_t logd_bad_bytes = 0;
    struct KeptRecords { bool valid = false; psdr_render_opts o{}; uint64_t gen = 0; long long n = 0; int kind = 0; } kept;
    uint64_t tables_gen = 0;

    void *d_seed = nullptr;
    size_t seed_cap = 0;
    long long seed_key[4] = {0, 0, 0, 0};
    bool seed_valid = false;
    hipStream_t seed_stream = nullptr;
    hipEvent_t seed_event = nullptr;
    long long seed_fills = 0, seed_launches = 0;
    long long logd_launches = 0, logd_lean_launches = 0, logd_lean_seeded = 0;
    int logd_lean_lds = 0, logd_lean_park = 0;
    void *d_ws = nullptr;
    size_t ws_bytes = 0;
    void *d_live = nullptr;
    size_t live_bytes = 0;
    void *d_probe = nullptr;
    size_t probe_bytes = 0;
    uint32_t emit_rows = 0;
    int forest_min_inline = 0;
};

constexpr int kRayCounters = 64, kRayCounterStride = 16;
constexpr int kWfSub = 64, kWfCountStride = 32;

namespace psdr_host {
int fail(const std::string &m);
int scratch_reserve(void **buf, size_t *have, size_t need, hipStream_t s, const char *what);
long long fit_chunk(long long chunk, size_t bytes_per_slot, size_t fixed_bytes, size_t have);
inline int workspace_reserve(psdr_scene_s *h, size_t need, hipStream_t s) { return scratch_reserve(&h->d_ws, &h->ws_bytes, need, s, "wavefront workspace (path-state streams + trace requests)"); }
int launch_blocks(const psdr_scene_s *h, long long n, int per_cu = 16);
int plan_lds(const psdr_scene_s *h, LaunchCtx &cx, int reserved = 0);
int lds_bytes(const LaunchCtx &cx, const psdr_scene_s *h);
void fill_top(const psdr_scene_s *h, SceneView &sc);
constexpr int kMaxInlineTris = 2 * kTinyTris;
int make_ctx(psdr_scene_s *h, const psdr_render_opts *o, int sampler, LaunchCtx &cx);
bool use_wavefront(const psdr_scene_s *h, const psdr_render_opts *o);
bool traced_wavefront(const psdr_scene_s *h);
int launch_wf_trace(psdr_scene_s *h, const float4 *req, const int32_t *count, long long sub_cap, float4 *hit, hipStream_t s, bool ign = false);
struct ProbeBuffers { float4 *hit; uint32_t *mask; float4 *req; int32_t *count; long long sub_cap; };
int probe_buffers(psdr_scene_s *h, long long slots, int rays_per_slot, ProbeBuffers &pb, hipStream_t s, int per_cu = 16);
SinkLayout make_sink_layout(const psdr_scene_s *h, const psdr_grads *g);
inline int sink_bytes_base(const SinkLayout &L) { return (L.priv_rows > 0 && !L.priv_regs) ? (L.priv_off + kPrivWords * kBlock) * 4 : (L.rep * L.stride * 4 + 15) / 16 * 16; }
inline int sink_bytes(const SinkLayout &L) { return L.pend_rows > 0 ? (L.pend_off + L.pend_rows * kPendWords * kBlock) * 4 : sink_bytes_base(L); }
inline void sink_reserve_pending(SinkLayout &L, int rows) { L.pend_rows = 0; L.pend_off = (sink_bytes_base(L) / 4 + 3) / 4 * 4; L.pend_rows = rows; }
int check_counts(const psdr_scene_s *h, const psdr_render_opts *o);
int begin_call(psdr_scene_s *h, hipStream_t s);
int primary_edge_order(psdr_scene_s *h, const LaunchCtx &cx, long long i0, long long n, const uint32_t **order, hipStream_t s);
constexpr int kMaxRefits = 64;
constexpr float kRefitAreaGrowth = 1.3f;

struct VariantOps {
    int (*render_c)(psdr_scene_s *h, const psdr_render_opts *o, float *img, hipStream_t s);
    int (*render_fwd)(psdr_scene_s *h, const psdr_render_opts *o, int K, const psdr_tangents *tangents, float *img, float *dimg, hipStream_t s);
    int (*render_rev)(psdr_scene_s *h, const psdr_render_opts *o, const float *adj_img, float *out_img, const psdr_grads *grads, hipStream_t s);
    int (*guide)(psdr_scene_s *h, LaunchCtx &cx, const int32_t reso[4], int nrounds, long long n, float *out_mass, hipStream_t s);
};
struct PathSedgeOps {
    int (*fwd)(psdr_scene_s *h, const psdr_render_opts *o, int K, const psdr_tangents *tangents, float *dimg, hipStream_t s);
    int (*rev)(psdr_scene_s *h, const psdr_render_opts *o, const float *adj_img, const psdr_grads *grads, hipStream_t s);
};
const PathSedgeOps *path_sedge_ops_0();
const PathSedgeOps *path_sedge_ops_1();
const PathSedgeOps *path_sedge_ops_2();
const PathSedgeOps *path_sedge_ops_3();
const PathSedgeOps *path_sedge_ops_4();
const PathSedgeOps *path_sedge_ops_6();
const PathSedgeOps *path_sedge_ops_8();
const PathSedgeOps *path_sedge_ops_10();
int logd_lean_launch_8(psdr_scene_s *h, const psdr_render_opts *o, const LaunchCtx &cx, const psdr::TangentView<1, psdr::kSceneTiny> &tv, float *img, float *dimg, hipStream_t s, bool *ran);
const VariantOps *variant_ops_0();
const VariantOps *variant_ops_1();
const VariantOps *variant_ops_2();
const VariantOps *variant_ops_3();
const VariantOps *variant_ops_4();
const VariantOps *variant_ops_6();
const VariantOps *variant_ops_8();
const VariantOps *variant_ops_10();
}

#define HIP_TRY(expr)                                                                              \
    do { hipError_t e_ = (expr); if (e_ != hipSuccess) return psdr_host::fail(std::string(#expr) + ": " + hipGetErrorString(e_)); } while (0)
```

### psdr-cuda_amd/csrc/psdr_kernels.h

```cpp
#pragma once
#include "psdr_host.h"

namespace {
using namespace psdr_host;

__device__ __forceinline__ float wave_shfl_down(float v, int off) { return __shfl_down(v, off, 64); }

template <int CTRL, int ROW_MASK> __device__ __forceinline__ float dpp_add(float v) {
    return v + __int_as_float(__builtin_amdgcn_update_dpp(0, __float_as_int(v), CTRL, ROW_MASK, 0xf, true));
}
__device__ __forceinline__ float wave_total(float v) {
    v = dpp_add<0x111, 0xf>(v); v = dpp_add<0x112, 0xf>(v); v = dpp_add<0x114, 0xf>(v); v = dpp_add<0x118, 0xf>(v);
    v = dpp_add<0x142, 0xa>(v); v = dpp_add<0x143, 0xc>(v);
    return __int_as_float(__builtin_amdgcn_readlane(__float_as_int(v), 63));
}
#ifndef PSDR_DPP_ALWAYS
#define PSDR_DPP_ALWAYS 0
#endif
template <int N, bool DPP = (N <= 6 || PSDR_DPP_ALWAYS)> __device__ __forceinline__ bool wave_segmented_sum(int key, float (&v)[N]) {
    const int lane = threadIdx.x & 63;
    if (DPP && __ballot(key != __builtin_amdgcn_readfirstlane(key)) == 0ull) {
#pragma unroll
        for (int i = 0; i < N; ++i) v[i] = wave_total(v[i]);
        return lane == 0;
// ... 1409 lines not shown
    }
    sink.n_pending = 0;
}

template <int FL> struct PrimaryEdgeSink {
    static constexpr int flags = FL;
    static constexpr bool has_env = (FL & kSceneEnv) != 0;
    float *g_prim_edge;
    long long rep_stride;
    int reps;
    __device__ __forceinline__ void add_pedge(int e, int word, float v) const {
        if (v != 0.f && isfinite(v)) atomicAdd(g_prim_edge + (size_t) (blockIdx.x % (unsigned) reps) * rep_stride + (size_t) e * PSDR_PEDGE_STRIDE + word, v);
    }
};
__global__ __launch_bounds__(kBlock) void k_sum_replicas(float *__restrict__ dst, const float *__restrict__ rep, long long n, int reps) {
    const long long i = (long long) blockIdx.x * kBlock + threadIdx.x;
    if (i >= n) return;
    float s = 0.f;
    for (int r = 0; r < reps; ++r) s += rep[(size_t) r * n + i];
    if (s != 0.f) dst[i] += s;
}
template <int FL, int INTEG>
__global__ __launch_bounds__(kBlock, PSDR_WAVES_PE) void k_primary_edge_rev(LaunchCtx cx, PrimaryEdgeSink<FL> sink, long long i0, long long n, float inv_sppe,
                                                                            const float *__restrict__ adj_img, unsigned long long *counters,
                                                                            const uint32_t *__restrict__ order) {
    TraversalStack st; setup_lds(cx, st);
    uint32_t nrays = 0;
    const long long nceil = (n + kBlock - 1) / kBlock * kBlock;
    for (long long j = (long long) blockIdx.x * kBlock + threadIdx.x; j < nceil; j += (long long) gridDim.x * kBlock) {
        float w[4] = {0.f, 0.f, 0.f, 0.f};
        int edge = -1;
        if (j < n)
            edge = primary_edge_reverse_values<INTEG, FL>(cx.sc, st, cx.lp, cx.jump, (uint64_t) (i0 + (order ? (long long) order[j] : j)), inv_sppe, adj_img,
                                                          nrays, w);
        const bool head = wave_run_sum<4>(edge, w);
        if (head && edge >= 0) {
#pragma unroll
            for (int i = 0; i < 4; ++i) sink.add_pedge(edge, i, w[i]);
        }
    }
    count_rays(counters, nrays);
}

template <int FL>
__global__ __launch_bounds__(kBlock) void k_secondary_edge_rev(LaunchCtx cx, DeviceSink<FL> sink, long long i0, long long n, float inv_sppse,
                                                               const float *__restrict__ adj_img, unsigned long long *counters,
                                                               const uint32_t *__restrict__ list, const int *__restrict__ list_n) {
    TraversalStack st; setup_lds(cx, st);
    sink.begin(dyn_lds_floats(cx.off_sink));
    uint32_t nrays = 0;
    const bool guided = cx.sc.d.guide_cmf != nullptr && cx.sc.d.num_guide_cells > 0;
    if (list != nullptr) n = *list_n;
    for (long long jj = (long long) blockIdx.x * kBlock + threadIdx.x; jj < n; jj += (long long) gridDim.x * kBlock) {
        const long long j = list != nullptr ? (long long) list[jj] : jj;
        Rng rng; rng.init((uint64_t) (i0 + j), cx.jump);
        float s3[3] = {rng.next(), rng.next(), rng.next()};
        const float pdf0 = guided ? guide_sample_reuse(cx.sc, s3) : 1.f;
        secondary_edge_reverse(sink, cx.sc, st, s3, (pdf0 > kEpsilon ? 1.f / pdf0 : 1.f) * inv_sppse, adj_img, nrays, list == nullptr);
    }
    sink.end();
    count_rays(counters, nrays);
}


inline int camera_blocks_per_cu(const psdr_scene_s *h, long long n) {
    if (h->opt.camera_blocks > 0) return h->opt.camera_blocks;
    if (h->has_rough) return 16;
    if (h->n_tiny > 0 && h->n_blas == 0) return 40;
    const long long fit = n / ((long long) kBlock * h->num_cus * 2);
    return (int) std::max(16LL, std::min(64LL, fit));
}
inline int big_launch_per_cu(const psdr_scene_s *h, long long n) { return (int) std::max(16LL, std::min(40LL, n / ((long long) kBlock * h->num_cus * 8))); }
inline long long launch_chunk(const psdr_scene_s *h, int log2_default) { return 1ll << (h->opt.chunk_log2 > 0 ? h->opt.chunk_log2 : log2_default); }
inline bool probe_direct(const psdr_scene_s *h, const psdr_render_opts *o, long long n) {
    return traced_wavefront(h) && h->opt.probe != 0 && o->bsdf_samples == 1 && o->light_samples == 1 && !(o->flags & PSDR_FLAG_FUSED) && n >= (1ll << 16);
}
inline const ulonglong2 *seed_table(psdr_scene_s *h, const psdr_render_opts *o, long long WH, int nsp, long long n, hipStream_t s) {
    if (h->opt.seed_cache == 0 || n <= 0 || n > (1ll << std::max(0, std::min(40, h->opt.seed_cache_log2)))) return nullptr;
    const long long key[4] = {WH, (long long) o->spp, (long long) o->spp_begin, (long long) nsp};
    if (h->d_seed != nullptr && h->seed_valid && std::equal(key, key + 4, h->seed_key)) {
        if (s != h->seed_stream && h->seed_event != nullptr && hipStreamWaitEvent(s, h->seed_event, 0) != hipSuccess) { (void) hipGetLastError(); return nullptr; }
        return reinterpret_cast<const ulonglong2 *>(h->d_seed);
    }
    h->seed_valid = false;
    if ((size_t) n > h->seed_cap) {
        if (h->d_seed) { (void) hipFreeAsync(h->d_seed, s); h->d_seed = nullptr; h->seed_cap = 0; }
        void *nb = nullptr;
        if (hipMallocAsync(&nb, (size_t) n * sizeof(ulonglong2), s) != hipSuccess) { (void) hipGetLastError(); return nullptr; }
        h->d_seed = nb; h->seed_cap = (size_t) n;
    }
    if (h->seed_event == nullptr && hipEventCreateWithFlags(&h->seed_event, hipEventDisableTiming) != hipSuccess) { (void) hipGetLastError(); h->seed_event = nullptr; return nullptr; }
    hipLaunchKernelGGL(k_seed_fill, dim3((unsigned) ((n + kBlock - 1) / kBlock)), dim3(kBlock), 0, s, reinterpret_cast<ulonglong2 *>(h->d_seed), n, o->spp, o->spp_begin, SlotDiv(nsp));
    if (hipGetLastError() != hipSuccess || hipEventRecord(h->seed_event, s) != hipSuccess) { (void) hipGetLastError(); return nullptr; }
    std::copy(key, key + 4, h->seed_key);
    h->seed_valid = true; h->seed_stream = s; h->seed_fills++;
    return reinterpret_cast<const ulonglong2 *>(h->d_seed);
}
template <class G, class R, int FL> constexpr bool seeded_render_c() { return (FL & kSceneTiny) != 0 && (FL & kScenePre) == 0 && std::is_same<G, float>::value && std::is_same<R, float>::value; }
template <class G, class R, int FL>
int run_camera(psdr_scene_s *h, const psdr_render_opts *o, const TV<R, FL> &tv, float *img, float *dimg, hipStream_t s) {
    const long long WH = (long long) h->desc.width * h->desc.height;
    const int nsp = o->spp_end - o->spp_begin;
    if (o->spp <= 0 || nsp <= 0) return 0;
    LaunchCtx cx;
    if (int rc = make_ctx(h, o, 0, cx)) return rc;
    const long long n = WH * nsp;
    h->slots[0] += (uint64_t) n;
    const int own = (h->opt.own_pixels != 0 && nsp <= 64 && 64 % nsp == 0) ? 1 : 0;
    if constexpr ((FL & kSceneForest) != 0) {
        if (o->integrator == PSDR_INTEGRATOR_DIRECT && probe_direct(h, o, n)) {
            const TangentView<0, FL> tv0{};
            TV<R, FL | kScenePre> tvp;
            for (int k = 0; k < (ad_traits<R>::K > 0 ? ad_traits<R>::K : 1); ++k) tvp.t[k] = tv.t[k];
            tvp.live = tv.live;
            LaunchCtx cxp = cx;
            plan_lds(h, cxp, 1 << 30);
            cxp.sc.n_lnodes = cxp.sc.n_lbtris = cxp.sc.n_ltri = 0;
            const long long chunk = std::min<long long>(n, launch_chunk(h, 25));
            for (long long c0 = 0; c0 < n; c0 += chunk) {
                const long long nc = std::min(chunk, n - c0);
                ProbeBuffers pb;
                const int probe_per_cu = big_launch_per_cu(h, nc);
                if (int rc = probe_buffers(h, nc, 3, pb, s, probe_per_cu)) return rc;
                const TraceQueue tq{pb.req, pb.count, pb.sub_cap};
                const int blocks = (launch_blocks(h, nc, probe_per_cu) + kWfSub - 1) / kWfSub * kWfSub;
                hipLaunchKernelGGL(k_direct_probe<FL>, dim3(blocks), dim3(kBlock), lds_bytes(cx, h), s, cx, tv0, o->spp, o->spp_begin, SlotDiv(nsp), c0, nc, tq, pb.hit, pb.mask,
                                   make_rng_jump(o->rng_offset[0] + 2));
                HIP_TRY(hipGetLastError());
                if (int rc = launch_wf_trace(h, pb.req, pb.count, pb.sub_cap, pb.hit, s)) return rc;
                hipLaunchKernelGGL(HIP_KERNEL_NAME(k_camera<G, R, PSDR_INTEGRATOR_DIRECT, FL | kScenePre, false>), dim3(launch_blocks(h, nc, camera_blocks_per_cu(h, nc))), dim3(kBlock), cxp.off_stack, s,
                                   cxp, tvp, o->spp, o->spp_begin, SlotDiv(nsp), nc, 1.f / (float) o->spp, img, dimg, WH * 3, h->d_counters, c0, ProbeView{pb.hit, pb.mask}, own);
                HIP_TRY(hipGetLastError());
            }
            return 0;
        }
    }
    bool gated = false;
    if constexpr (logd_instance<G, R, PSDR_INTEGRATOR_PATH, FL>()) {
        constexpr int K = ad_traits<R>::K;
        bool texels_only = o->integrator == PSDR_INTEGRATOR_PATH && h->opt.logd != 0 && h->desc.num_texels > 0 && h->desc.texels != nullptr;
        for (int k = 0; k < K && texels_only; ++k) {
            const psdr_tangents &t = tv.t[k];
            texels_only = t.d_texels != nullptr && !t.d_tri_info && !t.d_emitter_rad && !t.d_cam_to_world && !t.d_sec_edge && !t.d_prim_edge && !t.d_env_f;
        }
        if (texels_only) {
            if (int rc = scratch_reserve(&h->d_logd_bad, &h->logd_bad_bytes, sizeof(int), s, "log-derivative gate")) return rc;
            int *bad = reinterpret_cast<int *>(h->d_logd_bad);
            HIP_TRY(hipMemsetAsync(bad, 0, sizeof(int), s));
            TangentView<K, 0> tvk;
            for (int k = 0; k < K; ++k) tvk.t[k] = tv.t[k];
            hipLaunchKernelGGL(k_logd_check<K>, dim3((unsigned) ((h->desc.num_texels + kBlock - 1) / kBlock)), dim3(kBlock), 0, s, h->desc.texels, tvk, h->desc.num_texels, h->d_counters, bad);
            hipLaunchKernelGGL(k_logd_gate, dim3(1), dim3(64), 0, s, h->d_counters, bad);
            bool lean = false;
            if constexpr (K == 1 && FL == kSceneTiny) { if (int rc = logd_lean_launch_8(h, o, cx, tv, img, dimg, s, &lean)) return rc; }
            if (!lean)
                hipLaunchKernelGGL(HIP_KERNEL_NAME(k_camera_logd<K, FL, ((FL & kSceneTiny) != 0)>), dim3(launch_blocks(h, n, camera_blocks_per_cu(h, n))), dim3(kBlock), lds_bytes(cx, h), s, cx, tv,
                                   o->spp, o->spp_begin, SlotDiv(nsp), n, 1.f / (float) o->spp, img, dimg, WH * 3, h->d_counters, own);
            HIP_TRY(hipGetLastError());
            h->logd_launches++;
            gated = true;
        }
    }
#define PSDR_LAUNCH_CAMERA_T(INTEG, NOTREE)                                                                                        \
    hipLaunchKernelGGL(HIP_KERNEL_NAME(k_camera<G, R, INTEG, FL, NOTREE>), dim3(launch_blocks(h, n, camera_blocks_per_cu(h, n))), dim3(kBlock), lds_bytes(cx, h), s, cx, tv, o->spp, \
                       o->spp_begin, nsp, n, 1.f / (float) o->spp, img, dimg, WH * 3, h->d_counters, 0ll, ProbeView{nullptr, nullptr}, own)
#define PSDR_LAUNCH_CAMERA(INTEG) PSDR_LAUNCH_CAMERA_T(INTEG, ((FL & kSceneTiny) != 0))
    if constexpr (seeded_render_c<G, R, FL>()) {
        if (o->integrator == PSDR_INTEGRATOR_PATH) {
            if (const ulonglong2 *seed = seed_table(h, o, WH, nsp, n, s)) {
                hipLaunchKernelGGL(HIP_KERNEL_NAME(k_camera_seeded<G, R, PSDR_INTEGRATOR_PATH, FL, true>), dim3(launch_blocks(h, n, camera_blocks_per_cu(h, n))), dim3(kBlock), lds_bytes(cx, h), s, cx, tv,
                                   o->spp, o->spp_begin, SlotDiv(nsp), n, 1.f / (float) o->spp, img, dimg, WH * 3, h->d_counters, own, seed);
                HIP_TRY(hipGetLastError());
                h->seed_launches++;
                return 0;
            }
        }
    }
    switch (o->integrator) {
        case PSDR_INTEGRATOR_DIRECT: PSDR_LAUNCH_CAMERA(PSDR_INTEGRATOR_DIRECT); break;
        case PSDR_INTEGRATOR_PATH: PSDR_LAUNCH_CAMERA(PSDR_INTEGRATOR_PATH); break;
        case PSDR_INTEGRATOR_FIELD: PSDR_LAUNCH_CAMERA(PSDR_INTEGRATOR_FIELD); break;
        default: return fail("Unknown integrator");
    }
#undef PSDR_LAUNCH_CAMERA
#undef PSDR_LAUNCH_CAMERA_T
    HIP_TRY(hipGetLastError());
    if (gated) HIP_TRY(hipMemsetAsync(h->d_counters + kLogdGateWord, 0, sizeof(unsigned long long), s));
    return 0;
}


constexpr int kWfMaxDepth = 256;
struct WfRecArgs { float *disk; long long stride, c0, nc; };
template <class M, int FL>
int run_camera_wavefront(psdr_scene_s *h, const psdr_render_opts *o, const TV<M, FL> &tv, float *img, float *dimg, hipStream_t s, const WfRecArgs *rec = nullptr) {
    constexpr int K = ad_traits<M>::K;
    const long long WH = (long long) h->desc.width * h->desc.height;
    const int nsp = o->spp_end - o->spp_begin;
    if (o->spp <= 0 || nsp <= 0) return 0;
    const long long n_all = WH * nsp;
    const long long n = rec ? rec->nc : n_all;
    bool traced = false;
    if constexpr ((FL & kSceneForest) != 0) traced = traced_wavefront(h);
    const bool binned = !traced && (FL & kSceneForest) != 0 && h->n_blas > 0 && h->wf_binned;
    const int depth = o->max_depth;
    const size_t words = 8 + 6 * (1 + K) + (traced ? 8 : 0);
    const long long cap = rec ? n : std::min(n, fit_chunk(binned ? launch_chunk(h, 24) : launch_chunk(h, traced ? 26 : 25), 2 * words * 4 * 5 / 4 + (traced ? 80 : 0), 64u << 20, h->ws_bytes));
    const auto wf_per_cu = [&](long long slots) { return traced ? big_launch_per_cu(h, slots) : 16; };
    const long long max_blocks = ((long long) launch_blocks(h, cap, wf_per_cu(cap)) + kWfSub - 1) / kWfSub * kWfSub;
    const long long binned_sub_cap = (((cap + kBlock - 1) / kBlock + kWfSub) / kWfGroups + 2) * kBlock;
    const long long cap_alloc = ((binned ? binned_sub_cap * kWfSub : cap + max_blocks * kBlock) + 63) / 64 * 64;
    const size_t cnt_ints = (size_t) (kWfMaxDepth + 1) * kWfStageInts + (traced ? (size_t) (kWfMaxDepth + 1) * kWfSub * kWfCountStride : 0);
    const size_t cnt_bytes = cnt_ints * sizeof(int32_t);
    const size_t req_bytes = traced ? (size_t) 2 * cap_alloc * 2 * sizeof(float4) : 0;
    const size_t need = 2 * words * 4 * (size_t) cap_alloc + cnt_bytes + req_bytes;
    if (int rc = workspace_reserve(h, need, s)) return rc;
    int32_t *cnt = reinterpret_cast<int32_t *>(h->d_ws);
    int32_t *req_cnt = cnt + (size_t) (kWfMaxDepth + 1) * kWfStageInts;
    PathStream st[2];
    for (int i = 0; i < 2; ++i) {
        float *b = reinterpret_cast<float *>(reinterpret_cast<char *>(h->d_ws) + cnt_bytes) + (size_t) i * words * cap_alloc;
        const long long c = cap_alloc;
        st[i].cap = c;
        st[i].pixel = reinterpret_cast<int32_t *>(b); st[i].slot = reinterpret_cast<uint32_t *>(b + c); st[i].tri = reinterpret_cast<int32_t *>(b + 2 * c);
        st[i].hu = b + 3 * c; st[i].hv = b + 4 * c; st[i].dir = b + 5 * c; st[i].beta = b + 8 * c; st[i].acc = b + (8 + 3 * (1 + K)) * c;
        st[i].hit = traced ? reinterpret_cast<float4 *>(b + (8 + 6 * (1 + K)) * c) : nullptr;
        st[i].prev_t = nullptr;
        st[i].binned = binned ? 1 : 0;
    }
    TraceQueue tq{};
    tq.req = traced ? reinterpret_cast<float4 *>(reinterpret_cast<char *>(h->d_ws) + cnt_bytes + 2 * words * 4 * (size_t) cap_alloc) : nullptr;
    if (!rec) h->slots[0] += (uint64_t) n;
    const float inv_spp = 1.f / (float) o->spp;
    const long long j_first = rec ? rec->c0 : 0;
    for (long long j0 = j_first; j0 < j_first + n; j0 += cap) {
        const long long cn = std::min(cap, j_first + n - j0);
        LaunchCtx cx;
        if (int rc = make_ctx(h, o, 0, cx)) return rc;
        HIP_TRY(hipMemsetAsync(cnt, 0, (size_t) (std::min(depth, kWfMaxDepth) + 1) * kWfStageInts * sizeof(int32_t), s));
        if (traced) HIP_TRY(hipMemsetAsync(req_cnt, 0, (size_t) (std::min(depth, kWfMaxDepth) + 1) * kWfSub * kWfCountStride * sizeof(int32_t), s));
        const int blocks = (launch_blocks(h, cn, wf_per_cu(cn)) + kWfSub - 1) / kWfSub * kWfSub;
        const long long trips = (cn + (long long) blocks * kBlock - 1) / ((long long) blocks * kBlock);
        st[0].sub_cap = st[1].sub_cap = binned ? binned_sub_cap : (blocks / kWfSub) * trips * kBlock;
        st[0].count = cnt;
        if constexpr ((FL & kSceneForest) != 0) {
            if (traced) {
                tq.sub_cap = 2 * st[0].sub_cap;
                tq.count = req_cnt;
                LaunchCtx cxp = cx;
                plan_lds(h, cxp, 1 << 30);
                cxp.sc.n_lnodes = cxp.sc.n_lbtris = cxp.sc.n_ltri = 0;
                const int dyn_p = cxp.off_stack;
                WfRec wr{};
                bool recording = false;
                if constexpr (K == 0) {
                    if (rec) { recording = true; wr = WfRec{rec->disk + (j0 - rec->c0), rec->stride, o->spp, o->spp_begin, nsp, j0, 0}; }
                }
                if (recording) {
                    if constexpr (K == 0)
                        hipLaunchKernelGGL(HIP_KERNEL_NAME(k_wf_camera<M, FL, true, true>), dim3(blocks), dim3(kBlock), lds_bytes(cx, h), s, cx, tv, o->spp, o->spp_begin, nsp, j0, cn,
                                           inv_spp, img, dimg, WH * 3, st[0], 1 | (depth == 1 ? 2 : 0), h->d_counters, make_rng_jump(o->rng_offset[0] + 2), tq, wr);
                } else
                hipLaunchKernelGGL(HIP_KERNEL_NAME(k_wf_camera<M, FL, true>), dim3(blocks), dim3(kBlock), lds_bytes(cx, h), s, cx, tv, o->spp, o->spp_begin, nsp, j0, cn,
                                   inv_spp, img, dimg, WH * 3, st[0], 1 | (depth == 1 ? 2 : 0), h->d_counters, make_rng_jump(o->rng_offset[0] + 2), tq, wr);
                HIP_TRY(hipGetLastError());
                for (int k = 0; k < depth; ++k) {
                    if (int rc = launch_wf_trace(h, tq.req, tq.count, tq.sub_cap, st[k & 1].hit, s)) return rc;
                    st[(k + 1) & 1].count = cnt + (size_t) (k + 1) * kWfStageInts;
                    tq.count = req_cnt + (size_t) (k + 1) * kWfSub * kWfCountStride;
                    cxp.jump = make_rng_jump(o->rng_offset[0] + 2 + 5 * (uint64_t) k);
                    wr.stage = k;
                    if (recording) {
                        if constexpr (K == 0)
                            hipLaunchKernelGGL(HIP_KERNEL_NAME(k_wf_bounce<M, FL, true, true>), dim3(blocks), dim3(kBlock), dyn_p, s, cxp, tv, inv_spp, img, dimg, WH * 3,
                                               st[k & 1], st[(k + 1) & 1], (k + 1 < depth ? 1 : 0) | (k + 2 == depth ? 2 : 0), h->d_counters, make_rng_jump(o->rng_offset[0] + 2 + 5 * (uint64_t) (k + 1)), tq, wr);
                    } else
                    hipLaunchKernelGGL(HIP_KERNEL_NAME(k_wf_bounce<M, FL, true>), dim3(blocks), dim3(kBlock), dyn_p, s, cxp, tv, inv_spp, img, dimg, WH * 3,
                                       st[k & 1], st[(k + 1) & 1], (k + 1 < depth ? 1 : 0) | (k + 2 == depth ? 2 : 0), h->d_counters, make_rng_jump(o->rng_offset[0] + 2 + 5 * (uint64_t) (k + 1)), tq, wr);
                    HIP_TRY(hipGetLastError());
                }
                continue;
            }
        }
        if (binned) {
            hipLaunchKernelGGL(HIP_KERNEL_NAME(k_wf_camera<M, FL>), dim3(blocks), dim3(kBlock), lds_bytes(cx, h), s, cx, tv, o->spp, o->spp_begin, nsp, j0, cn,
                               inv_spp, img, dimg, WH * 3, st[0], 1 | (depth == 1 ? 2 : 0), h->d_counters, make_rng_jump(o->rng_offset[0] + 2), tq, WfRec{});
            HIP_TRY(hipGetLastError());
            for (int k = 0; k < depth; ++k) {
                st[(k + 1) & 1].count = cnt + (size_t) (k + 1) * kWfStageInts;
                cx.jump = make_rng_jump(o->rng_offset[0] + 2 + 5 * (uint64_t) k);
                hipLaunchKernelGGL(HIP_KERNEL_NAME(k_wf_bounce<M, FL>), dim3(blocks), dim3(kBlock), lds_bytes(cx, h), s, cx, tv, inv_spp, img, dimg, WH * 3,
                                   st[k & 1], st[(k + 1) & 1], (k + 1 < depth ? 1 : 0) | (k + 2 == depth ? 2 : 0), h->d_counters, make_rng_jump(o->rng_offset[0] + 2 + 5 * (uint64_t) (k + 1)), tq, WfRec{});
                HIP_TRY(hipGetLastError());
            }
            continue;
        }
        hipLaunchKernelGGL(HIP_KERNEL_NAME(k_wf_camera<M, FL>), dim3(blocks), dim3(kBlock), lds_bytes(cx, h), s, cx, tv, o->spp, o->spp_begin, nsp, j0, cn,
                           inv_spp, img, dimg, WH * 3, st[0], (depth > 1 ? 1 : 0) | (depth == 2 ? 2 : 0), h->d_counters, make_rng_jump(o->rng_offset[0] + 2 + 5), tq, WfRec{});
        HIP_TRY(hipGetLastError());
        for (int k = 1; k < depth; ++k) {
            st[k & 1].count = cnt + (size_t) k * kWfStageInts;
            cx.jump = make_rng_jump(o->rng_offset[0] + 2 + 5 * (uint64_t) k);
            hipLaunchKernelGGL(HIP_KERNEL_NAME(k_wf_bounce<M, FL>), dim3(blocks), dim3(kBlock), lds_bytes(cx, h), s, cx, tv, inv_spp, img, dimg, WH * 3,
                               st[(k - 1) & 1], st[k & 1], (k + 1 < depth ? 1 : 0) | (k + 2 == depth ? 2 : 0), h->d_counters, make_rng_jump(o->rng_offset[0] + 2 + 5 * (uint64_t) (k + 1)), tq, WfRec{});
            HIP_TRY(hipGetLastError());
        }
    }
    return 0;
}

template <int K, int FL>
int run_camera_wavefront_geo(psdr_scene_s *h, const psdr_render_opts *o, const TangentView<K, FL> &tv, float *img, float *dimg, hipStream_t s) {
    const long long WH = (long long) h->desc.width * h->desc.height;
    const int nsp = o->spp_end - o->spp_begin;
    if (o->spp <= 0 || nsp <= 0) return 0;
    const long long n = WH * nsp;
    const int depth = o->max_depth;
    const size_t words = 8 + 6 * (1 + K) + 3 * K + 8;
    const long long cap = std::min(n, fit_chunk(launch_chunk(h, 26), 2 * words * 4 * 5 / 4 + 80, 64u << 20, h->ws_bytes));
    const auto wf_per_cu = [&](long long slots) { return big_launch_per_cu(h, slots); };
    const long long max_blocks = ((long long) launch_blocks(h, cap, wf_per_cu(cap)) + kWfSub - 1) / kWfSub * kWfSub;
// ... 477 lines not shown
```

### psdr-cuda_amd/csrc/psdr_logd_lean.hip

```cpp
#define PSDR_WIDE_TREE 0
#define PSDR_LEAF_PAIR 0
#include "psdr_kernels.h"
#include "psdr_logd_lean.h"

namespace {

constexpr int kLeanFlags = kSceneTiny;

template <int K, int FL, bool SEEDED>
__global__ __launch_bounds__(kBlock, PSDR_LOGD_WAVES_K1) void k_camera_logd_lean(LaunchCtx cx, TV<Dual<K>, FL> tv, int spp, int s_begin, SlotDiv nsp, long long n, float inv_spp,
                                                                                  float *__restrict__ img, float *__restrict__ dimg, long long plane, unsigned long long *counters, int own,
                                                                                  const ulonglong2 *__restrict__ seed) {
    constexpr int NV = 3 * (1 + K);
    if (counters[kLogdGateWord] != 1ull) return;
    TraversalStack st; setup_lds(cx, st, tv);
    Park pk{nullptr};
#if defined(__HIP_DEVICE_COMPILE__)
    pk.base = reinterpret_cast<float *>(psdr_dyn_lds + cx.off_park) + threadIdx.x;
#endif
    uint32_t nrays = 0;
    const long long nceil = (n + kBlock - 1) / kBlock * kBlock;
    for (long long jb = (long long) blockIdx.x * kBlock; jb < nceil; jb += (long long) gridDim.x * kBlock) {
        const long long j = jb + threadIdx.x;
        const bool in = j < n;
        int pixel = 0x7fffffff, s_in = 0;
        if (in) slot_to_pixel(j, nsp, pixel, s_in);
        Rng rng;
        if constexpr (SEEDED) {
            const ulonglong2 sd = in ? seed[j] : ulonglong2{0ull, 0ull};
            rng.init_seeded(sd.x, sd.y, cx.jump);
        } else {
            rng.init((uint64_t) pixel * (uint64_t) spp + (uint64_t) (s_begin + s_in), cx.jump);
        }
        const float j0 = rng.next(), j1 = rng.next();
        const int W = cx.sc.d.width;
        const float sx = ((float) (pixel % W) + j0) / (float) W, sy = ((float) (pixel / W) + j1) / (float) cx.sc.d.height;
        const TangentView<0, FL> tv0{};
        const RayT<float> ray = primary_ray<float>(cx.sc, tv0, sx, sy);
        const Vec3<Dual<K>> r = zero_nonfinite(li_path_logd_lean<K>(cx.sc, tv, st, cx.lp, rng, ray, in, nrays, pk));
        float v[NV];
        v[0] = in ? r.x.v * inv_spp : 0.f; v[1] = in ? r.y.v * inv_spp : 0.f; v[2] = in ? r.z.v * inv_spp : 0.f;
#pragma unroll
        for (int k = 0; k < K; ++k) { v[3 + 3 * k] = in ? r.x.d[k] * inv_spp : 0.f; v[4 + 3 * k] = in ? r.y.d[k] * inv_spp : 0.f; v[5 + 3 * k] = in ? r.z.d[k] * inv_spp : 0.f; }
        const bool head = wave_segmented_sum<NV>(pixel, v);
        if (head && in) {
            float *p = img + (size_t) pixel * 3;
            if (own) {
                p[0] = v[0]; p[1] = v[1]; p[2] = v[2];
#pragma unroll
                for (int k = 0; k < K; ++k) { float *q = dimg + (size_t) k * plane + (size_t) pixel * 3; q[0] = v[3 + 3 * k]; q[1] = v[4 + 3 * k]; q[2] = v[5 + 3 * k]; }
            } else {
                if (v[0] != 0.f) atomicAdd(p, v[0]);
                if (v[1] != 0.f) atomicAdd(p + 1, v[1]);
                if (v[2] != 0.f) atomicAdd(p + 2, v[2]);
#pragma unroll
                for (int k = 0; k < K; ++k) {
                    float *q = dimg + (size_t) k * plane + (size_t) pixel * 3;
                    if (v[3 + 3 * k] != 0.f) atomicAdd(q, v[3 + 3 * k]);
                    if (v[4 + 3 * k] != 0.f) atomicAdd(q + 1, v[4 + 3 * k]);
                    if (v[5 + 3 * k] != 0.f) atomicAdd(q + 2, v[5 + 3 * k]);
                }
            }
        }
    }
    count_rays(counters, nrays);
}

}

namespace psdr_host {
int logd_lean_launch_8(psdr_scene_s *h, const psdr_render_opts *o, const LaunchCtx &cx0, const psdr::TangentView<1, psdr::kSceneTiny> &tv, float *img, float *dimg, hipStream_t s, bool *ran) {
    *ran = false;
    if (h->opt.logd_park == 0) return 0;
    constexpr int kCuLds = 160 * 1024, park = ParkLayout<1>::cols * kBlock * 4;
    const int lds = (lds_bytes(cx0, h) + 15) / 16 * 16;
    const int limit = h->opt.lds_budget > 0 ? std::min(h->opt.lds_budget, kCuLds / PSDR_LOGD_WAVES_K1) : kCuLds / PSDR_LOGD_WAVES_K1;
    if (lds + park > limit) return 0;
    LaunchCtx cx = cx0;
    cx.off_park = lds;
    const long long WH = (long long) h->desc.width * h->desc.height;
    const int nsp = o->spp_end - o->spp_begin;
    const long long n = WH * nsp;
    const int own = (h->opt.own_pixels != 0 && nsp <= 64 && 64 % nsp == 0) ? 1 : 0;
    const dim3 grid(launch_blocks(h, n, camera_blocks_per_cu(h, n)));
    const ulonglong2 *seed = seed_table(h, o, WH, nsp, n, s);
    if (seed != nullptr)
        hipLaunchKernelGGL(HIP_KERNEL_NAME(k_camera_logd_lean<1, kLeanFlags, true>), grid, dim3(kBlock), lds + park, s, cx, tv, o->spp, o->spp_begin, SlotDiv(nsp), n, 1.f / (float) o->spp, img, dimg,
                           WH * 3, h->d_counters, own, seed);
    else
        hipLaunchKernelGGL(HIP_KERNEL_NAME(k_camera_logd_lean<1, kLeanFlags, false>), grid, dim3(kBlock), lds + park, s, cx, tv, o->spp, o->spp_begin, SlotDiv(nsp), n, 1.f / (float) o->spp, img, dimg,
                           WH * 3, h->d_counters, own, seed);
    h->logd_lean_launches++;
    if (seed != nullptr) { h->logd_lean_seeded++; h->seed_launches++; }
    h->logd_lean_lds = lds; h->logd_lean_park = park;
    *ran = true;
    return 0;
}
}
```

### psdr-cuda_amd/psdr_cuda/_abi.py

```python
import ctypes as C
import os

_HERE = os.path.dirname(os.path.abspath(__file__))
PKG_ROOT = os.path.dirname(_HERE)
REPO_ROOT = os.path.dirname(PKG_ROOT)

TRI_STRIDE = 24
TRIUV_STRIDE = 8
SEDGE_STRIDE = 16
PEDGE_STRIDE = 8
BSDF_STRIDE = 16
EMITTER_F_STRIDE = 8
EMITTER_I_STRIDE = 4
CAM_WORDS = 64
ENV_WORDS = 32
TRI_FACE_NORMALS = 0x40000000

BSDF_DIFFUSE, BSDF_ROUGHCONDUCTOR = 0, 1
SLOT_REFLECTANCE, SLOT_ALPHA_U, SLOT_ALPHA_V, SLOT_ETA, SLOT_K = range(5)
CAM_SAMPLE_TO_CAMERA, CAM_TO_WORLD, CAM_WORLD_TO_SAMPLE, CAM_POS, CAM_DIR, CAM_INV_AREA = 0, 16, 32, 48, 51, 54
INTEGRATOR_DIRECT, INTEGRATOR_PATH, INTEGRATOR_FIELD = 0, 1, 2
FLAG_FUSED, FLAG_WAVEFRONT, FLAG_LITERAL_FORMS, FLAG_KEEP_RECORDS, FLAG_PATH_SEDGES = 1, 2, 4, 8, 16
MAX_PATH_SEDGE_DEPTH = 8
FIELDS = {"silhouette": 0, "position": 1, "depth": 2, "geoNormal": 3, "shNormal": 4, "uv": 5}

_fp = C.c_void_p


class SceneDesc(C.Structure):
    _fields_ = [
        ("width", C.c_int32), ("height", C.c_int32),
        ("num_tris", C.c_int32), ("num_meshes", C.c_int32), ("num_bsdfs", C.c_int32), ("num_emitters", C.c_int32),
        ("num_sec_edges", C.c_int32), ("num_prim_edges", C.c_int32), ("num_texels", C.c_int32),
        ("num_guide_cells", C.c_int32),
        ("tri_info", _fp), ("tri_uv", _fp), ("tri_mesh", _fp), ("mesh_bsdf", _fp), ("mesh_emitter", _fp),
        ("bsdf_rec", _fp), ("texels", _fp), ("emitter_f", _fp), ("emitter_i", _fp),
        ("face_cmf", _fp), ("face_pmf", _fp), ("emitter_cmf", _fp), ("emitter_pmf", _fp),
        ("emitter_sum", C.c_float),
        ("cam", _fp),
        ("sec_edge", _fp), ("sec_cmf", _fp), ("sec_pmf", _fp), ("sec_sum", C.c_float),
        ("prim_edge", _fp), ("prim_cmf", _fp), ("prim_pmf", _fp), ("prim_sum", C.c_float),
        ("guide_reso", C.c_int32 * 3),
        ("guide_cmf", _fp), ("guide_pmf", _fp), ("guide_sum", C.c_float),
        ("env_emitter", C.c_int32), ("env_tex", C.c_int32 * 3), ("env_reso", C.c_int32 * 2),
        ("env_f", _fp), ("env_cmf", _fp), ("env_pmf", _fp), ("env_sum", C.c_float),
        ("material_mask", C.c_uint32),
        ("sec_edge_faces", _fp),
        ("prim_edge_z", _fp),
    ]


class RenderOpts(C.Structure):
    _fields_ = [
        ("integrator", C.c_int32), ("bsdf_samples", C.c_int32), ("light_samples", C.c_int32),
        ("max_depth", C.c_int32), ("hide_emitters", C.c_int32), ("field", C.c_int32),
        ("spp", C.c_int32), ("sppe", C.c_int32), ("sppse", C.c_int32),
        ("spp_begin", C.c_int32), ("spp_end", C.c_int32),
        ("sppe_begin", C.c_int32), ("sppe_end", C.c_int32),
        ("sppse_begin", C.c_int32), ("sppse_end", C.c_int32),
        ("flags", C.c_int32),
        ("rng_offset", C.c_uint64 * 3),
    ]


class Tangents(C.Structure):
    _fields_ = [("d_tri_info", _fp), ("d_texels", _fp), ("d_emitter_rad", _fp), ("d_cam_to_world", _fp),
                ("d_sec_edge", _fp), ("d_prim_edge", _fp), ("d_env_f", _fp)]


class Grads(C.Structure):
    _fields_ = [("g_tri_info", _fp), ("g_texels", _fp), ("g_emitter_rad", _fp), ("g_cam_to_world", _fp),
                ("g_sec_edge", _fp), ("g_prim_edge", _fp), ("g_env_f", _fp)]


TANGENT_FIELDS = ("tri_info", "texels", "emitter_rad", "cam_to_world", "sec_edge", "prim_edge", "env_f")

HIP_SYMBOLS = (
    "psdr_last_error", "psdr_version", "psdr_abi_struct_sizes", "psdr_scene_create", "psdr_scene_destroy", "psdr_scene_set_option", "psdr_scene_set_tables",
    "psdr_bvh_build", "psdr_bvh_stats", "psdr_scene_info", "psdr_trace", "psdr_render_c", "psdr_render_d_fwd", "psdr_render_d_rev",
    "psdr_guide_build", "psdr_get_counters", "psdr_scene_rev_layout", "psdr_scene_seed_info", "psdr_scene_logd_info",
    "psdr_geo_world_vertices_fwd", "psdr_geo_world_vertices_rev", "psdr_geo_tri_rows_fwd", "psdr_geo_tri_rows_rev", "psdr_geo_sec_edges_fwd", "psdr_geo_sec_edges_rev", "psdr_geo_prim_edges_fwd", "psdr_geo_prim_edges_rev",
    "psdr_geo_compact_edges_fwd", "psdr_geo_compact_edges_rev", "psdr_geo_emitter_tables",
    "psdr_geo_world_vertices_jvp", "psdr_geo_tri_rows_jvp", "psdr_geo_sec_edges_jvp", "psdr_geo_prim_edges_jvp", "psdr_geo_compact_edges_jvp",
    "psdr_cube_sample_reuse", "psdr_sample_boundary_segment_direct",
)

HIP_LIB_PATH = os.path.join(PKG_ROOT, "lib", "libpsdr_hip.so")


def use_library(path):
    global HIP_LIB_PATH
    if _hip is not None:
        raise RuntimeError("psdr_cuda._abi.use_library: the library is already loaded (%s)" % HIP_LIB_PATH)
    HIP_LIB_PATH = os.path.abspath(path)


_hip = None


def load_hip():
    global _hip
    if _hip is not None:
        return _hip
    if not os.path.exists(HIP_LIB_PATH):
        raise RuntimeError("libpsdr_hip.so not built (%s): run `python -c 'import __graft_entry__ as g; g.build()'`"
                           % HIP_LIB_PATH)
    lib = C.CDLL(HIP_LIB_PATH)
    lib.psdr_last_error.restype = C.c_char_p
    lib.psdr_version.restype = C.c_char_p
    vp, i32 = C.c_void_p, C.c_int32
    lib.psdr_scene_create.argtypes = [C.POINTER(vp)]
    lib.psdr_scene_destroy.argtypes = [vp]
    lib.psdr_scene_set_option.argtypes = [vp, C.c_char_p, C.c_double]
    lib.psdr_scene_set_tables.argtypes = [vp, C.POINTER(SceneDesc)]
    lib.psdr_bvh_build.argtypes = [vp, vp]
    lib.psdr_trace.argtypes = [vp, i32] + [vp] * 7 + [vp] * 4 + [vp]
    lib.psdr_render_c.argtypes = [vp, C.POINTER(RenderOpts), vp, vp]
    lib.psdr_render_d_fwd.argtypes = [vp, C.POINTER(RenderOpts), i32, C.POINTER(Tangents), vp, vp, vp]
    lib.psdr_render_d_rev.argtypes = [vp, C.POINTER(RenderOpts), vp, vp, C.POINTER(Grads), vp]
    lib.psdr_guide_build.argtypes = [vp, C.POINTER(RenderOpts), C.POINTER(i32), i32, vp, vp]
    lib.psdr_get_counters.argtypes = [vp, C.POINTER(C.c_uint64)]
    lib.psdr_scene_info.argtypes = [vp, C.POINTER(i32)]
    lib.psdr_scene_rev_layout.argtypes = [vp, C.POINTER(i32)]
    lib.psdr_scene_seed_info.argtypes = [vp, C.POINTER(C.c_int64)]
    lib.psdr_scene_logd_info.argtypes = [vp, C.POINTER(C.c_int64)]
    lib.psdr_geo_world_vertices_fwd.argtypes = [i32, vp, vp, vp, vp, vp]
    lib.psdr_geo_world_vertices_rev.argtypes = [i32, vp, vp, vp, vp, vp, vp, vp]
    lib.psdr_geo_tri_rows_fwd.argtypes = [i32, i32, vp, vp, vp, vp, i32, vp]
    lib.psdr_geo_tri_rows_rev.argtypes = [i32, i32, vp, vp, vp, vp, i32, vp, vp, vp]
    lib.psdr_geo_sec_edges_fwd.argtypes = [i32, vp, vp, vp, i32, vp, vp, vp]
    lib.psdr_geo_sec_edges_rev.argtypes = [i32, vp, vp, vp, vp, i32, vp]
    lib.psdr_geo_prim_edges_fwd.argtypes = [i32, vp, vp, vp, vp, i32, vp, vp, vp, vp, vp]
    lib.psdr_geo_prim_edges_rev.argtypes = [i32, vp, vp, vp, vp, vp, vp, vp]
    lib.psdr_geo_compact_edges_fwd.argtypes = [i32, vp, i32, vp, i32, i32, vp, i32, i32, vp, vp, vp, vp, vp, vp, vp, vp]
    lib.psdr_geo_compact_edges_rev.argtypes = [i32, i32, vp, vp, vp, vp]
    lib.psdr_geo_world_vertices_jvp.argtypes = [i32, vp, vp, vp, vp, vp, vp, vp, vp]
    lib.psdr_geo_tri_rows_jvp.argtypes = [i32, i32, vp, vp, vp, vp, i32, vp, vp, vp]
    lib.psdr_geo_sec_edges_jvp.argtypes = [i32, vp, vp, vp, i32, vp, vp]
    lib.psdr_geo_prim_edges_jvp.argtypes = [i32, vp, vp, vp, vp, vp, vp, vp]
    lib.psdr_geo_compact_edges_jvp.argtypes = [i32, i32, vp, vp, vp, vp]
    lib.psdr_geo_emitter_tables.argtypes = [i32, vp, i32, vp, vp, i32, vp, vp, vp, vp, vp, vp, vp, vp, vp, vp]
    lib.psdr_cube_sample_reuse.argtypes = [i32, C.POINTER(i32), vp, vp, C.c_float, i32, i32, vp, vp, vp]
    lib.psdr_sample_boundary_segment_direct.argtypes = [C.POINTER(SceneDesc), i32] + [vp] * 12
    for name in HIP_SYMBOLS:
        if name not in ("psdr_last_error", "psdr_version"):
            getattr(lib, name).restype = C.c_int
    sizes = (C.c_int32 * 4)()
    lib.psdr_abi_struct_sizes(sizes)
    mine = (C.sizeof(SceneDesc), C.sizeof(RenderOpts), C.sizeof(Tangents), C.sizeof(Grads))
    if tuple(sizes) != mine:
        raise RuntimeError("psdr_cuda/_abi.py is out of sync with include/psdr_hip.h: %s vs %s" % (tuple(sizes), mine))
    _hip = lib
    return lib


def check(lib, rc):
    if rc != 0:
        msg = lib.psdr_last_error()
        raise RuntimeError(msg.decode() if msg else "psdr_hip call failed (rc=%d)" % rc)


def scene_stats(handle):
    lib = load_hip()
    out = (C.c_int32 * 8)()
    check(lib, lib.psdr_scene_info(handle, out))
    return {"n_tiny": out[0], "n_blas": out[1], "n_inline": out[2], "leaf_tris": out[3], "device_built": out[4], "n_slab": out[5], "occ_rows": out[6], "occ_max_rows": out[7]}


REV_LAUNCH_KINDS = {-1: "none", 0: "fused", 1: "split", 2: "split_wavefront", 3: "kept_records", 4: "probe"}


def rev_layout(handle):
    lib = load_hip()
    out = (C.c_int32 * 16)()
    check(lib, lib.psdr_scene_rev_layout(handle, out))
    return {"tex_n": out[0], "rad_n": out[1], "env_n": out[2], "hot_rows": out[3], "rep": out[4], "priv_rows": out[5], "priv_regs": out[6],
            "pend_rows": out[7], "launch": REV_LAUNCH_KINDS[out[8]], "pe_reps": out[9], "hot_identity": out[10], "deep_rec": out[11],
            "priv_slot": (out[12], out[13]), "tree_hot_rows": out[14], "pe_sorted": out[15]}


def seed_cache_info(handle):
    lib = load_hip()
    out = (C.c_int64 * 4)()
    check(lib, lib.psdr_scene_seed_info(handle, out))
    return {"slots": int(out[0]), "bytes": int(out[1]), "fills": int(out[2]), "launches": int(out[3])}


def logd_info(handle):
    lib = load_hip()
    out = (C.c_int64 * 4)()
    check(lib, lib.psdr_scene_logd_info(handle, out))
    return {"launches": int(out[0]), "lean": int(out[1]), "lean_seeded": int(out[2]), "lean_lds_bytes": int(out[3])}


def make_opts(integrator=INTEGRATOR_DIRECT, bsdf_samples=1, light_samples=1, max_depth=1, hide_emitters=False,
              field=0, spp=1, sppe=0, sppse=0, spp_range=None, sppe_range=None, sppse_range=None,
              rng_offset=(0, 0, 0), flags=0):
    o = RenderOpts()
    o.flags = flags
    o.integrator, o.bsdf_samples, o.light_samples = integrator, bsdf_samples, light_samples
    o.max_depth, o.hide_emitters, o.field = max_depth, int(bool(hide_emitters)), field
    o.spp, o.sppe, o.sppse = spp, sppe, sppse
    o.spp_begin, o.spp_end = spp_range if spp_range is not None else (0, spp)
    o.sppe_begin, o.sppe_end = sppe_range if sppe_range is not None else (0, sppe)
    o.sppse_begin, o.sppse_end = sppse_range if sppse_range is not None else (0, sppse)
    for i in range(3):
        o.rng_offset[i] = int(rng_offset[i])
    return o


def draws_per_slot(opts):
    if opts.integrator == INTEGRATOR_DIRECT:
        li = 3 * opts.bsdf_samples + 2 * opts.light_samples
    elif opts.integrator == INTEGRATOR_PATH:
        li = 5 * opts.max_depth
    else:
        li = 0
    se = 3
    if opts.integrator == INTEGRATOR_PATH and (opts.flags & FLAG_PATH_SEDGES) and opts.max_depth >= 2:
        se = 11 * opts.max_depth - 9
    return (2 + li, 1 + 2 * li, se)
```

Baseline: 20830 Mpath-samples/s.

## Add terminal-bounce row masks to prune tiny-scene tests in path kernels

Precomputes on the host, for each triangle, a bitmask of the tiny-plane rows that can occlude a path's last bounce toward any emitter. The mask table is uploaded to device, staged into LDS, and used by new specialized renderC and logd kernels (k_camera_term, k_camera_logd_term) so the final-bounce shadow/emitter tests only visit the relevant rows. The lighter last-bounce intersection fill also skips frame and UV work. These kernels take priority over the existing seeded and lean paths, at the cost of extra LDS per block, which may reduce occupancy.

Measured after the change: 20410 Mpath-samples/s. -2.1%, worse.

```diff
diff --git a/__graft_entry__.py b/__graft_entry__.py
--- a/__graft_entry__.py
+++ b/__graft_entry__.py
@@ -41,6 +41,10 @@
         objs.append(o)
         unit_cmds[o] = ["hipcc"] + HIPCC_FLAGS + ["-c", os.path.join(csrc, "psdr_logd_lean.hip"), "-o", o]
         jobs.append(subprocess.Popen(unit_cmds[o]))
+        o = os.path.join(obj_dir, "term.o")
+        objs.append(o)
+        unit_cmds[o] = ["hipcc"] + HIPCC_FLAGS + ["-c", os.path.join(csrc, "psdr_term.hip"), "-o", o]
+        jobs.append(subprocess.Popen(unit_cmds[o]))
         o = os.path.join(obj_dir, "host.o")
         objs.append(o)
         unit_cmds[o] = ["hipcc"] + HIPCC_FLAGS + ["-c", os.path.join(csrc, "psdr_hip.hip"), "-o", o]
@@ -81,6 +85,10 @@
     if _stale(hp, srcs + [os.path.join(hc_dir, "hostcheck_path_sedge.cpp")]):
         subprocess.check_call(["hipcc", "--offload-arch=gfx950", "-O2", "-std=c++17", "-fPIC", "-shared", "-pthread",
                                os.path.join(hc_dir, "hostcheck_path_sedge.cpp"), "-o", hp])
+    ht = os.path.join(hc_dir, "libhostcheck_term.so")
+    if _stale(ht, srcs + [os.path.join(hc_dir, "hostcheck_term.cpp")]):
+        subprocess.check_call(["hipcc", "--offload-arch=gfx950", "-O2", "-std=c++17", "-fPIC", "-shared",
+                               os.path.join(hc_dir, "hostcheck_term.cpp"), "-o", ht])
     po_dir = os.path.join(ROOT, "tests", "poison")
     po = os.path.join(po_dir, "libpoison.so")
     if _stale(po, [os.path.join(po_dir, "poison.hip")]):
@@ -113,7 +121,7 @@
     srcs = [os.path.join(csrc, f) for f in os.listdir(csrc)] + [os.path.join(ROOT, "include", "psdr_hip.h")]
     obj_dir = os.path.join(PKG, "lib", "obj")
     defect_lib = os.path.join(ROOT, "tests", "poison", "libpsdr_hip_defect.so")
-    objs = [os.path.join(obj_dir, "%s%d.o" % (unit, v)) for v in VARIANTS for unit in ("variant", "path_sedge")] + [os.path.join(obj_dir, "logd_lean.o"), os.path.join(obj_dir, "host.o"), os.path.join(obj_dir, "tables.o")]
+    objs = [os.path.join(obj_dir, "%s%d.o" % (unit, v)) for v in VARIANTS for unit in ("variant", "path_sedge")] + [os.path.join(obj_dir, "logd_lean.o"), os.path.join(obj_dir, "term.o"), os.path.join(obj_dir, "host.o"), os.path.join(obj_dir, "tables.o")]
     if not all(os.path.exists(o) for o in objs):
         return None
     if object_job is not None and object_job.wait() != 0:
diff --git a/include/psdr_hip.h b/include/psdr_hip.h
--- a/include/psdr_hip.h
+++ b/include/psdr_hip.h
@@ -208,6 +208,8 @@
 
 int psdr_scene_logd_info(psdr_scene_t h, int64_t out[4]);
 
+int psdr_scene_term_info(psdr_scene_t h, int64_t out[4]);
+
 int psdr_get_counters(psdr_scene_t h, uint64_t out[4]);
 
 #ifdef __cplusplus
diff --git a/psdr-cuda_amd/csrc/psdr_bvh_build.h b/psdr-cuda_amd/csrc/psdr_bvh_build.h
--- a/psdr-cuda_amd/csrc/psdr_bvh_build.h
+++ b/psdr-cuda_amd/csrc/psdr_bvh_build.h
@@ -224,6 +224,57 @@
         }
 }
 
+inline void tiny_terminal_rows(const std::vector<float4> &prims, const std::vector<int> &row_of_prim, int num_tris, const std::vector<char> &is_emitter_tri, int slab_rows,
+                               std::vector<uint32_t> &term) {
+    const int n = (int) prims.size() / 3;
+    term.assign((size_t) num_tris, 0xffffffffu);
+    struct P { double c[4][3]; int nc; double nrm[3], d; int tris[2]; int row; bool em; };
+    std::vector<P> ps((size_t) n);
+    double scale = 0.0;
+    bool any_emitter = false;
+    for (int i = 0; i < n; ++i) {
+        const float4 &a = prims[(size_t) i * 3], &b = prims[(size_t) i * 3 + 1], &c = prims[(size_t) i * 3 + 2];
+        int32_t ids; std::memcpy(&ids, &a.w, 4);
+        P &q = ps[(size_t) i];
+        const bool quad = ((uint32_t) ids >> 16) != 0xffffu;
+        q.tris[0] = ids & 0xffff; q.tris[1] = quad ? (int) ((uint32_t) ids >> 16) : -1;
+        const double p0[3] = {a.x, a.y, a.z}, e1[3] = {b.x, b.y, b.z}, e2[3] = {c.x, c.y, c.z};
+        q.nc = quad ? 4 : 3;
+        for (int k = 0; k < 3; ++k) { q.c[0][k] = p0[k]; q.c[1][k] = p0[k] + e1[k]; q.c[2][k] = p0[k] + e2[k]; q.c[3][k] = p0[k] + e1[k] + e2[k]; }
+        q.nrm[0] = e1[1] * e2[2] - e1[2] * e2[1]; q.nrm[1] = e1[2] * e2[0] - e1[0] * e2[2]; q.nrm[2] = e1[0] * e2[1] - e1[1] * e2[0];
+        const double len = std::sqrt(q.nrm[0] * q.nrm[0] + q.nrm[1] * q.nrm[1] + q.nrm[2] * q.nrm[2]);
+        for (int k = 0; k < 3; ++k) q.nrm[k] = len > 0.0 ? q.nrm[k] / len : 0.0;
+        q.d = q.nrm[0] * p0[0] + q.nrm[1] * p0[1] + q.nrm[2] * p0[2];
+        q.row = row_of_prim[(size_t) i];
+        q.em = false;
+        for (int a2 = 0; a2 < 2; ++a2) { const int t = q.tris[a2]; q.em = q.em || (t >= 0 && t < num_tris && is_emitter_tri[(size_t) t]); }
+        any_emitter = any_emitter || q.em;
+        if (q.row < 0 || q.row >= 32) return;
+        for (int v = 0; v < q.nc; ++v) for (int k = 0; k < 3; ++k) scale = std::max(scale, std::fabs(q.c[v][k]));
+    }
+    if (!any_emitter) return;
+    const double tol = 1e-6 * std::max(scale, 1e-30);
+    for (int r = 0; r < n; ++r) {
+        uint32_t m = ps[(size_t) r].row >= slab_rows ? 1u << ps[(size_t) r].row : 0u;
+        for (int e = 0; e < n; ++e) {
+            if (!ps[(size_t) e].em) continue;
+            m |= 1u << ps[(size_t) e].row;
+            for (int p = 0; p < n; ++p) {
+                if (p == e) continue;
+                const P &q = ps[(size_t) p];
+                double lo = 0.0, hi = 0.0;
+                bool finite = true, touches = false;
+                auto side = [&](const P &x, bool emitter) { for (int v = 0; v < x.nc; ++v) { const double sd = q.nrm[0] * x.c[v][0] + q.nrm[1] * x.c[v][1] + q.nrm[2] * x.c[v][2] - q.d;
+                                                                                         if (!std::isfinite(sd)) finite = false; lo = std::min(lo, sd); hi = std::max(hi, sd);
+                                                                                         if (emitter && std::fabs(sd) <= tol) touches = true; } };
+                side(ps[(size_t) r], false); side(ps[(size_t) e], true);
+                if (!finite || touches || (lo < -tol && hi > tol)) m |= 1u << q.row;
+            }
+        }
+        for (int a = 0; a < 2; ++a) { const int tr = ps[(size_t) r].tris[a]; if (tr >= 0 && tr < num_tris) term[(size_t) tr] = m; }
+    }
+}
+
 struct BuildTri { float lo[3], hi[3], c[3]; };
 struct Builder {
     const float *rows; int T;
diff --git a/psdr-cuda_amd/csrc/psdr_hip.hip b/psdr-cuda_amd/csrc/psdr_hip.hip
--- a/psdr-cuda_amd/csrc/psdr_hip.hip
+++ b/psdr-cuda_amd/csrc/psdr_hip.hip
@@ -751,7 +751,7 @@
     HIP_TRY(hipStreamSynchronize(s));
     h->hot_rows = (int) tris.size(); h->hot_identity = false;
     h->root = 0; h->bvh_depth = info.depth; h->num_nodes = T - 1; h->num_btris = T;
-    h->n_tiny = 0; h->aa_cnt = 0; h->n_blas = 0; h->n_inline = 0; h->have_occ = false; h->emit_rows = 0;
+    h->n_tiny = 0; h->aa_cnt = 0; h->n_blas = 0; h->n_inline = 0; h->have_occ = false; h->have_term = false; h->emit_rows = 0;
     if (use_wide_tree(h, false)) {
         std::vector<BvhNode> host_nodes((size_t) T - 1);
         HIP_TRY(hipMemcpyAsync(host_nodes.data(), h->d_nodes, host_nodes.size() * sizeof(BvhNode), hipMemcpyDeviceToHost, s));
@@ -936,6 +936,7 @@
     else if (n == "wf_geo") h->opt.wf_geo = iv;
     else if (n == "logd") h->opt.logd = iv;
     else if (n == "seed_cache") h->opt.seed_cache = iv;
+    else if (n == "terminal_rows") h->opt.terminal_rows = iv;
     else if (n == "logd_park") h->opt.logd_park = iv;
     else if (n == "seed_cache_log2") h->opt.seed_cache_log2 = std::max(0, std::min(40, iv));
     else if (n == "keep_records") h->opt.keep_records = iv;
@@ -969,6 +970,7 @@
     if (h->d_hot_map) (void) hipFree(h->d_hot_map);
     if (h->d_hot_tris) (void) hipFree(h->d_hot_tris);
     if (h->d_occ) (void) hipFree(h->d_occ);
+    if (h->d_term) (void) hipFree(h->d_term);
     if (h->d_top) (void) hipFree(h->d_top);
     if (h->d_inline_ids) (void) hipFree(h->d_inline_ids);
     if (h->d_lbvh) (void) hipFree(h->d_lbvh);
@@ -1172,7 +1174,7 @@
     h->bvh_depth = forest ? fb.max_depth : b.max_depth; h->num_nodes = (int) nodes.size(); h->num_btris = (int) btris.size() / 3;
     if (int rc = bvh4_build(h, nodes, forest ? fb.roots : std::vector<int32_t>{root}, forest, s)) return rc;
     h->have_bvh = true;
-    h->n_tiny = 0; h->aa_cnt = 0; h->n_blas = 0; h->n_inline = 0; h->have_occ = false; h->emit_rows = 0;
+    h->n_tiny = 0; h->aa_cnt = 0; h->n_blas = 0; h->n_inline = 0; h->have_occ = false; h->have_term = false; h->emit_rows = 0;
     if (forest) {
         h->n_tiny = tiny_plane_form(top_prims, h->tiny, h->tiny_meta, &h->aa_cnt, h->aa_enabled);
         update_emit_rows(h);
@@ -1210,6 +1212,19 @@
             }
             HIP_TRY(copy_on_stream(h->d_occ, occ.data(), occ.size() * sizeof(uint32_t), hipMemcpyHostToDevice, s));
             h->have_occ = true;
+            std::vector<uint32_t> term;
+            tiny_terminal_rows(prims, row_of_prim, T, is_em, h->aa_cnt != 0 ? kAaSlots : 0, term);
+            if (h->desc.env_f != nullptr) term.assign((size_t) T, 0xffffffffu);
+            h->term_max_rows = 0;
+            for (int r = 0; r < T; ++r) h->term_max_rows = std::max(h->term_max_rows, (int) __builtin_popcount(term[(size_t) r] & ((1u << h->n_tiny) - 1u)));
+            term.resize((size_t) 2 * T, 0xffffffffu);
+            if (term.size() > h->term_cap) {
+                if (h->d_term) (void) hipFree(h->d_term);
+                h->term_cap = std::max<size_t>(term.size(), 64);
+                HIP_TRY(hipMalloc(&h->d_term, h->term_cap * sizeof(uint32_t)));
+            }
+            HIP_TRY(copy_on_stream(h->d_term, term.data(), term.size() * sizeof(uint32_t), hipMemcpyHostToDevice, s));
+            h->have_term = true;
             h->occ_max_rows = 0;
             for (int r = 0; r < T; ++r) for (int e = 0; e < T; ++e) if (is_em[(size_t) e]) h->occ_max_rows = std::max(h->occ_max_rows, (int) __builtin_popcount(occ[(size_t) r * T + e] & ((1u << h->n_tiny) - 1u)));
         }
@@ -1394,6 +1409,11 @@
     out[0] = h->logd_launches; out[1] = h->logd_lean_launches; out[2] = h->logd_lean_seeded; out[3] = (int64_t) h->logd_lean_lds + h->logd_lean_park;
     return 0;
 }
+int psdr_scene_term_info(psdr_scene_t h, int64_t out[4]) {
+    if (!h || !out) return fail("psdr_scene_term_info: null argument");
+    out[0] = h->term_c_launches; out[1] = h->term_d_launches; out[2] = h->have_term ? 1 : 0; out[3] = h->have_term ? h->term_max_rows : 0;
+    return 0;
+}
 int psdr_scene_seed_info(psdr_scene_t h, int64_t out[4]) {
     if (!h || !out) return fail("psdr_scene_seed_info: null argument");
     out[0] = h->seed_valid ? h->seed_key[0] * h->seed_key[3] : 0; out[1] = (int64_t) (h->seed_cap * sizeof(ulonglong2)); out[2] = h->seed_fills; out[3] = h->seed_launches;
diff --git a/psdr-cuda_amd/csrc/psdr_host.h b/psdr-cuda_amd/csrc/psdr_host.h
--- a/psdr-cuda_amd/csrc/psdr_host.h
+++ b/psdr-cuda_amd/csrc/psdr_host.h
@@ -139,6 +139,7 @@
     int seed_cache = 1;
     int seed_cache_log2 = 25;
     int logd_park = 1;
+    int terminal_rows = 1;
     int bvh_maxleaf = 4;
     float bvh_tcost = 2.0f;
 };
@@ -198,6 +199,7 @@
     std::vector<int32_t> emitter_i;
     int32_t *d_hot_map = nullptr, *d_hot_tris = nullptr;
     uint32_t *d_occ = nullptr; size_t occ_cap = 0; bool have_occ = false; int occ_max_rows = 0;
+    uint32_t *d_term = nullptr; size_t term_cap = 0; bool have_term = false; int term_max_rows = 0;
     int hot_rows = 0;
     bool hot_identity = false;
     size_t hot_cap = 0;
@@ -229,6 +231,7 @@
     hipEvent_t seed_event = nullptr;
     long long seed_fills = 0, seed_launches = 0;
     long long logd_launches = 0, logd_lean_launches = 0, logd_lean_seeded = 0;
+    long long term_c_launches = 0, term_d_launches = 0;
     int logd_lean_lds = 0, logd_lean_park = 0;
     void *d_ws = nullptr;
     size_t ws_bytes = 0;
@@ -288,6 +291,9 @@
 const PathSedgeOps *path_sedge_ops_8();
 const PathSedgeOps *path_sedge_ops_10();
 int logd_lean_launch_8(psdr_scene_s *h, const psdr_render_opts *o, const LaunchCtx &cx, const psdr::TangentView<1, psdr::kSceneTiny> &tv, float *img, float *dimg, hipStream_t s, bool *ran);
+int term_render_c_launch_8(psdr_scene_s *h, const psdr_render_opts *o, const LaunchCtx &cx, float *img, hipStream_t s, bool *ran);
+int term_logd_launch_8(psdr_scene_s *h, const psdr_render_opts *o, const LaunchCtx &cx, const psdr::TangentView<1, psdr::kSceneTiny> &tv, float *img, float *dimg, hipStream_t s, bool *ran);
+inline int term_table_bytes(const psdr_scene_s *h) { return (h->opt.terminal_rows != 0 && h->have_term && h->d_term != nullptr) ? (h->desc.num_tris * 4 + 15) / 16 * 16 : 0; }
 const VariantOps *variant_ops_0();
 const VariantOps *variant_ops_1();
 const VariantOps *variant_ops_2();
diff --git a/psdr-cuda_amd/csrc/psdr_kernels.h b/psdr-cuda_amd/csrc/psdr_kernels.h
--- a/psdr-cuda_amd/csrc/psdr_kernels.h
+++ b/psdr-cuda_amd/csrc/psdr_kernels.h
@@ -1585,7 +1585,10 @@
             hipLaunchKernelGGL(k_logd_check<K>, dim3((unsigned) ((h->desc.num_texels + kBlock - 1) / kBlock)), dim3(kBlock), 0, s, h->desc.texels, tvk, h->desc.num_texels, h->d_counters, bad);
             hipLaunchKernelGGL(k_logd_gate, dim3(1), dim3(64), 0, s, h->d_counters, bad);
             bool lean = false;
-            if constexpr (K == 1 && FL == kSceneTiny) { if (int rc = logd_lean_launch_8(h, o, cx, tv, img, dimg, s, &lean)) return rc; }
+            if constexpr (K == 1 && FL == kSceneTiny) {
+                if (int rc = term_logd_launch_8(h, o, cx, tv, img, dimg, s, &lean)) return rc;
+                if (!lean) { if (int rc = logd_lean_launch_8(h, o, cx, tv, img, dimg, s, &lean)) return rc; }
+            }
             if (!lean)
                 hipLaunchKernelGGL(HIP_KERNEL_NAME(k_camera_logd<K, FL, ((FL & kSceneTiny) != 0)>), dim3(launch_blocks(h, n, camera_blocks_per_cu(h, n))), dim3(kBlock), lds_bytes(cx, h), s, cx, tv,
                                    o->spp, o->spp_begin, SlotDiv(nsp), n, 1.f / (float) o->spp, img, dimg, WH * 3, h->d_counters, own);
@@ -1600,6 +1603,11 @@
 #define PSDR_LAUNCH_CAMERA(INTEG) PSDR_LAUNCH_CAMERA_T(INTEG, ((FL & kSceneTiny) != 0))
     if constexpr (seeded_render_c<G, R, FL>()) {
         if (o->integrator == PSDR_INTEGRATOR_PATH) {
+            if constexpr (FL == kSceneTiny) {
+                bool ran = false;
+                if (int rc = term_render_c_launch_8(h, o, cx, img, s, &ran)) return rc;
+                if (ran) { HIP_TRY(hipGetLastError()); return 0; }
+            }
             if (const ulonglong2 *seed = seed_table(h, o, WH, nsp, n, s)) {
                 hipLaunchKernelGGL(HIP_KERNEL_NAME(k_camera_seeded<G, R, PSDR_INTEGRATOR_PATH, FL, true>), dim3(launch_blocks(h, n, camera_blocks_per_cu(h, n))), dim3(kBlock), lds_bytes(cx, h), s, cx, tv,
                                    o->spp, o->spp_begin, SlotDiv(nsp), n, 1.f / (float) o->spp, img, dimg, WH * 3, h->d_counters, own, seed);
diff --git a/psdr-cuda_amd/csrc/psdr_logd_lean.hip b/psdr-cuda_amd/csrc/psdr_logd_lean.hip
--- a/psdr-cuda_amd/csrc/psdr_logd_lean.hip
+++ b/psdr-cuda_amd/csrc/psdr_logd_lean.hip
@@ -75,7 +75,7 @@
     constexpr int kCuLds = 160 * 1024, park = ParkLayout<1>::cols * kBlock * 4;
     const int lds = (lds_bytes(cx0, h) + 15) / 16 * 16;
     const int limit = h->opt.lds_budget > 0 ? std::min(h->opt.lds_budget, kCuLds / PSDR_LOGD_WAVES_K1) : kCuLds / PSDR_LOGD_WAVES_K1;
-    if (lds + park > limit) return 0;
+    if (lds + park + term_table_bytes(h) > limit) return 0;
     LaunchCtx cx = cx0;
     cx.off_park = lds;
     const long long WH = (long long) h->desc.width * h->desc.height;
diff --git a/psdr-cuda_amd/csrc/psdr_term.h b/psdr-cuda_amd/csrc/psdr_term.h
--- /dev/null
+++ b/psdr-cuda_amd/csrc/psdr_term.h
@@ -0,0 +1,186 @@
+#pragma once
+#include "psdr_logd_lean.h"
+
+namespace psdr {
+
+template <class TVT> __host__ __device__ __forceinline__ void fill_its_term(Its<float> &its, const SceneView &sc, const TVT &tv, const Hit &h, const RayT<float> &ray, bool last) {
+    its.valid = true; its.tri = h.tri; its.hu = h.u; its.hv = h.v;
+    const int tm = Tab<TVT::flags>::tri_mesh(sc, h.tri);
+    its.mesh = tm & ~PSDR_TRI_FACE_NORMALS;
+    const TriRow<float> T = load_tri<float>(sc, tv, h.tri);
+    its.n = T.fn;
+    const float bu = h.u, bv = h.v;
+    its.p = bary_point(T.p0, T.e1, T.e2, bu, bv);
+    Vec3f dir = its.p - ray.o;
+    its.t = norm(dir);
+    dir = dir / its.t;
+    const Vec3f sh_n = (tm & PSDR_TRI_FACE_NORMALS) ? its.n : normalize(bary_point(T.n0, T.n1 - T.n0, T.n2 - T.n0, bu, bv));
+    if (last) {
+        its.sh.n = sh_n; its.sh.s = Vec3f(0.f); its.sh.t = Vec3f(0.f);
+        its.wi = Vec3f{0.f, 0.f, dot(-dir, sh_n)};
+        its.uvx = 0.f; its.uvy = 0.f;
+        return;
+    }
+    its.sh = Frame<float>(sh_n);
+    its.wi = its.sh.to_local(-dir);
+    if (sc.d.tri_uv) {
+        const float *q = Tab<TVT::flags>::tri_uv(sc, h.tri);
+        its.uvx = (q[2] - q[0]) * bu + ((q[4] - q[0]) * bv + q[0]);
+        its.uvy = (q[3] - q[1]) * bu + ((q[5] - q[1]) * bv + q[1]);
+    } else { its.uvx = 0.f; its.uvy = 0.f; }
+}
+
+template <int K, bool PARK, class TVT>
+__host__ __device__ __forceinline__ void li_path_term(const SceneView &sc, const TVT &tv, TraversalStack &st, const LiParams &lp, Rng &rng, const RayT<float> &ray0, bool active0, uint32_t &nrays,
+                                             const Park &pk, const uint32_t *term, Vec3f &out, float (&out_d)[K > 0 ? K : 1][3]) {
+    using L = ParkLayout<K>;
+    using TV0 = TangentView<0, TVT::flags>;
+    constexpr int KK = K > 0 ? K : 1;
+    const TV0 tv0{};
+    Vec3f result(0.f), beta(1.f), c(0.f);
+    float rd[KK][3], s[KK][3];
+#pragma unroll
+    for (int k = 0; k < KK; ++k) { rd[k][0] = rd[k][1] = rd[k][2] = 0.f; s[k][0] = s[k][1] = s[k][2] = 0.f; }
+    auto park_state = [&]() {
+        pk.put3(L::result, result); pk.put3(L::beta, beta);
+#pragma unroll
+        for (int k = 0; k < K; ++k) {
+            pk.put(L::rd + 3 * k, rd[k][0]); pk.put(L::rd + 3 * k + 1, rd[k][1]); pk.put(L::rd + 3 * k + 2, rd[k][2]);
+            pk.put(L::s + 3 * k, s[k][0]); pk.put(L::s + 3 * k + 1, s[k][1]); pk.put(L::s + 3 * k + 2, s[k][2]);
+        }
+        pk.put64(L::rng, rng.state); pk.put64(L::rng + 2, rng.inc);
+    };
+    RayT<float> ray = ray0;
+    bool active = active0;
+    bool tracing = active0;
+    Vec3f pf(0.f); float pdf_s = 0.f;
+    int tri_from = 0;
+    if constexpr (PARK) { park_state(); pk.put3(L::vtx, c); Park::fence(); }
+    for (int depth = 0; ; ++depth) {
+        const bool first = depth == 0, last = depth >= lp.max_depth;
+        Its<float> its;
+        its.valid = false; its.tri = its.mesh = -1; its.J = 1.f; its.t = INFINITY;
+        if (tracing) {
+            nrays++;
+            const uint32_t rows = (last && !first) ? wave_or_hd(term[tri_from]) : 0xffffffffu;
+            const Hit h = closest_hit<false, 2, true>(sc, st, ray.o, ray.d, INFINITY, -1, -1, kPreBsdfRay, rows);
+            if (h.tri >= 0) fill_its_term(its, sc, tv0, h, ray, last);
+        }
+        if constexpr (PARK) {
+            Park::fence();
+            c = pk.get3(L::vtx);
+            result = pk.get3(L::result); beta = pk.get3(L::beta);
+#pragma unroll
+            for (int k = 0; k < K; ++k) {
+                rd[k][0] = pk.get(L::rd + 3 * k); rd[k][1] = pk.get(L::rd + 3 * k + 1); rd[k][2] = pk.get(L::rd + 3 * k + 2);
+                s[k][0] = pk.get(L::s + 3 * k); s[k][1] = pk.get(L::s + 3 * k + 1); s[k][2] = pk.get(L::s + 3 * k + 2);
+            }
+            rng.state = pk.get64(L::rng); rng.inc = pk.get64(L::rng + 2);
+            Park::fence();
+        }
+        const bool a_hit = tracing && its.valid;
+        if (first) {
+            active = a_hit;
+            if (!lp.hide_emitters) result = Le<float>(sc, tv0, its, active);
+        } else {
+            const bool a1 = a_hit && emitter_of(sc, tv0, its) >= 0;
+            Vec3f bsdf_val(0.f); float pdf0(0.f);
+            if (a_hit) {
+                const float Gv = abs_(dot(its.n, -ray.d)) / sqr(its.t);
+                pdf0 = pdf_s * Gv;
+                bsdf_val = pf;
+            }
+            if (a1) {
+                const float wb = mis_weight(pdf0, float(emitter_position_pdf(sc, tv0, ray.o, its)));
+                const Vec3f lb = Le<float>(sc, tv0, its, true) * bsdf_val;
+                c = c + lb * wb;
+            }
+            if (active) {
+                const Vec3f bc = beta * c;
+                result = result + bc;
+#pragma unroll
+                for (int k = 0; k < K; ++k) {
+                    rd[k][0] = fmaf(bc.x, s[k][0], rd[k][0]); rd[k][1] = fmaf(bc.y, s[k][1], rd[k][1]); rd[k][2] = fmaf(bc.z, s[k][2], rd[k][2]);
+                }
+                active = a_hit;
+                if (active) {
+                    beta = beta * bsdf_val;
+                    if (!(beta.x != 0.f || beta.y != 0.f || beta.z != 0.f)) active = false;
+                }
+            }
+        }
+        if (last) break;
+        if constexpr (K > 0) {
+            if (active) {
+                float g[KK][3];
+                albedo_logd<KK>(sc, tv, its, g);
+#pragma unroll
+                for (int k = 0; k < K; ++k) { s[k][0] += g[k][0]; s[k][1] += g[k][1]; s[k][2] += g[k][2]; }
+            }
+        }
+        int bsdf_id = active ? Tab<TVT::flags>::mesh_bsdf(sc, its.mesh) : 0;
+        bool act = active;
+        if (bsdf_id < 0) { act = false; bsdf_id = 0; }
+        const Bsdf<float, float> bsdf(sc, tv0, bsdf_id);
+        const float sb0 = rng.next(), sb1 = rng.next(), sb2 = rng.next();
+        const float s0 = rng.next(), s1 = rng.next();
+        if constexpr (PARK) {
+            park_state();
+            pk.put(L::vtx, sb1); pk.put(L::vtx + 1, sb2);
+            Park::fence();
+        }
+        c = Vec3f(0.f);
+        if (act) {
+            const PosSample<float> ps = sample_emitter_position<float>(sc, tv0, its.p, s0, s1, false);
+            Vec3f wo = ps.p - its.p;
+            const float d2 = dot(wo, wo), dist = safe_sqrt(d2);
+            wo = wo / dist;
+            const RayT<float> ray1{its.p, wo};
+            const Vec3f wl = its.sh.to_local(wo);
+            const bool lit = PSDR_SKIP_UNLIT ? (wl.z > 0.f && its.wi.z > 0.f) : true;
+            auto trace_light = [&]() {
+                if constexpr (PSDR_OCC_ROWS) return intersect<float, TV0, true>(sc, tv0, st, ray1, ps.valid && lit, kDetached, nrays, -1, -1, kPreLightRay, occ_rows(sc, its.tri, ps.tri));
+                else return intersect<float>(sc, tv0, st, ray1, ps.valid && lit, kDetached, nrays, -1, -1, kPreLightRay);
+            };
+            const Its<float> its1 = trace_light();
+            if (its1.valid && its1.t > dist - kShadowEpsilon && emitter_of(sc, tv0, its1) >= 0) {
+                const float Gv = abs_(dot(its1.n, -wo)) / d2;
+                const Vec3f bsdf_val = bsdf.eval(sc, tv0, its, wl, true) * to_m<float>(Gv * ps.J / ps.pdf);
+                float pdf1 = bsdf.pdf(sc, tv0, its, wl, true);
+                pdf1 = pdf1 * Gv;
+                const float w = mis_weight(float(ps.pdf), pdf1);
+                c = c + Le<float>(sc, tv0, its1, true) * bsdf_val * w;
+            }
+        }
+        float sb[3] = {sb0, sb1, sb2};
+        if constexpr (PARK) {
+            Park::fence();
+            sb[1] = pk.get(L::vtx); sb[2] = pk.get(L::vtx + 1);
+            Park::fence();
+            pk.put3(L::vtx, c);
+            Park::fence();
+        }
+        RayT<float> nray{Vec3f(0.f), Vec3f(0.f)};
+        Vec3f npf(0.f); float npdf = 0.f; int ntri = 0; bool ntracing = false;
+        if (act) {
+            Vec3f wo_s;
+            ntracing = bsdf.sample(sc, tv0, its, sb, true, wo_s, npdf);
+            Vec3f shn = its.sh.n;
+#if defined(__HIP_DEVICE_COMPILE__)
+            asm volatile("" : "+v"(shn.x), "+v"(shn.y), "+v"(shn.z));
+#endif
+            const Frame<float> fr(shn);
+            nray.o = its.p;
+            nray.d = fr.s * wo_s.x + fr.t * wo_s.y + shn * wo_s.z;
+            npf = bsdf.eval(sc, tv0, its, wo_s, true);
+            npf = npf / npdf;
+            ntri = its.tri;
+        }
+        ray = nray; pf = npf; pdf_s = npdf; tri_from = ntri; tracing = ntracing;
+    }
+    out = result;
+#pragma unroll
+    for (int k = 0; k < KK; ++k) { out_d[k][0] = rd[k][0]; out_d[k][1] = rd[k][1]; out_d[k][2] = rd[k][2]; }
+}
+
+}
diff --git a/psdr-cuda_amd/csrc/psdr_term.hip b/psdr-cuda_amd/csrc/psdr_term.hip
--- /dev/null
+++ b/psdr-cuda_amd/csrc/psdr_term.hip
@@ -0,0 +1,166 @@
+#define PSDR_WIDE_TREE 0
+#define PSDR_LEAF_PAIR 0
+#include "psdr_kernels.h"
+#include "psdr_term.h"
+
+#ifndef PSDR_TERM_PARK_C
+#define PSDR_TERM_PARK_C 1
+#endif
+
+namespace {
+
+constexpr int kTermFlags = kSceneTiny;
+
+template <int K, bool SEEDED, bool PARK>
+__device__ __forceinline__ void term_kernel_body(const LaunchCtx &cx, const TangentView<K, kTermFlags> &tv, int spp, int s_begin, const SlotDiv &nsp, long long n, float inv_spp,
+                                                 float *__restrict__ img, float *__restrict__ dimg, long long plane, unsigned long long *counters, int own,
+                                                 const ulonglong2 *__restrict__ seed, const uint32_t *__restrict__ term_g, int off_term) {
+    constexpr int NV = 3 * (1 + K), KK = K > 0 ? K : 1;
+    TraversalStack st; setup_lds(cx, st, tv);
+    Park pk{nullptr};
+    const uint32_t *term = nullptr;
+#if defined(__HIP_DEVICE_COMPILE__)
+    pk.base = reinterpret_cast<float *>(psdr_dyn_lds + cx.off_park) + threadIdx.x;
+    {
+        uint32_t *lt = reinterpret_cast<uint32_t *>(psdr_dyn_lds + off_term);
+        for (int i = threadIdx.x; i < cx.sc.d.num_tris; i += kBlock) lt[i] = term_g[i];
+        __syncthreads();
+        term = lt;
+    }
+#endif
+    uint32_t nrays = 0;
+    const long long nceil = (n + kBlock - 1) / kBlock * kBlock;
+    for (long long jb = (long long) blockIdx.x * kBlock; jb < nceil; jb += (long long) gridDim.x * kBlock) {
+        const long long j = jb + threadIdx.x;
+        const bool in = j < n;
+        int pixel = 0x7fffffff, s_in = 0;
+        if (in) slot_to_pixel(j, nsp, pixel, s_in);
+        Rng rng;
+        if constexpr (SEEDED) {
+            const ulonglong2 sd = in ? seed[j] : ulonglong2{0ull, 0ull};
+            rng.init_seeded(sd.x, sd.y, cx.jump);
+        } else {
+            rng.init((uint64_t) pixel * (uint64_t) spp + (uint64_t) (s_begin + s_in), cx.jump);
+        }
+        const float j0 = rng.next(), j1 = rng.next();
+        const int W = cx.sc.d.width;
+        const float sx = ((float) (pixel % W) + j0) / (float) W, sy = ((float) (pixel / W) + j1) / (float) cx.sc.d.height;
+        const TangentView<0, kTermFlags> tv0{};
+        const RayT<float> ray = primary_ray<float>(cx.sc, tv0, sx, sy);
+        Vec3f r; float rd[KK][3];
+        li_path_term<K, PARK>(cx.sc, tv, st, cx.lp, rng, ray, in, nrays, pk, term, r, rd);
+        const bool fx = isfinite(r.x), fy = isfinite(r.y), fz = isfinite(r.z);
+        float v[NV];
+        v[0] = (in && fx) ? r.x * inv_spp : 0.f; v[1] = (in && fy) ? r.y * inv_spp : 0.f; v[2] = (in && fz) ? r.z * inv_spp : 0.f;
+#pragma unroll
+        for (int k = 0; k < K; ++k) {
+            v[3 + 3 * k] = (in && fx && isfinite(rd[k][0])) ? rd[k][0] * inv_spp : 0.f;
+            v[4 + 3 * k] = (in && fy && isfinite(rd[k][1])) ? rd[k][1] * inv_spp : 0.f;
+            v[5 + 3 * k] = (in && fz && isfinite(rd[k][2])) ? rd[k][2] * inv_spp : 0.f;
+        }
+        const bool head = wave_segmented_sum<NV>(pixel, v);
+        if (head && in) {
+            float *p = img + (size_t) pixel * 3;
+            if (own) {
+                p[0] = v[0]; p[1] = v[1]; p[2] = v[2];
+#pragma unroll
+                for (int k = 0; k < K; ++k) { float *q = dimg + (size_t) k * plane + (size_t) pixel * 3; q[0] = v[3 + 3 * k]; q[1] = v[4 + 3 * k]; q[2] = v[5 + 3 * k]; }
+            } else {
+                if (v[0] != 0.f) atomicAdd(p, v[0]);
+                if (v[1] != 0.f) atomicAdd(p + 1, v[1]);
+                if (v[2] != 0.f) atomicAdd(p + 2, v[2]);
+#pragma unroll
+                for (int k = 0; k < K; ++k) {
+                    float *q = dimg + (size_t) k * plane + (size_t) pixel * 3;
+                    if (v[3 + 3 * k] != 0.f) atomicAdd(q, v[3 + 3 * k]);
+                    if (v[4 + 3 * k] != 0.f) atomicAdd(q + 1, v[4 + 3 * k]);
+                    if (v[5 + 3 * k] != 0.f) atomicAdd(q + 2, v[5 + 3 * k]);
+                }
+            }
+        }
+    }
+    count_rays(counters, nrays);
+}
+
+template <bool SEEDED>
+__global__ __launch_bounds__(kBlock, PSDR_WAVES_C_NOTREE) void k_camera_term(LaunchCtx cx, TangentView<0, kTermFlags> tv, int spp, int s_begin, SlotDiv nsp, long long n, float inv_spp,
+                                                                             float *__restrict__ img, unsigned long long *counters, int own, const ulonglong2 *__restrict__ seed,
+                                                                             const uint32_t *__restrict__ term_g, int off_term) {
+    term_kernel_body<0, SEEDED, PSDR_TERM_PARK_C != 0>(cx, tv, spp, s_begin, nsp, n, inv_spp, img, nullptr, 0, counters, own, seed, term_g, off_term);
+}
+template <bool SEEDED>
+__global__ __launch_bounds__(kBlock, PSDR_LOGD_WAVES_K1) void k_camera_logd_term(LaunchCtx cx, TangentView<1, kTermFlags> tv, int spp, int s_begin, SlotDiv nsp, long long n, float inv_spp,
+                                                                                 float *__restrict__ img, float *__restrict__ dimg, long long plane, unsigned long long *counters, int own,
+                                                                                 const ulonglong2 *__restrict__ seed, const uint32_t *__restrict__ term_g, int off_term) {
+    if (counters[kLogdGateWord] != 1ull) return;
+    term_kernel_body<1, SEEDED, true>(cx, tv, spp, s_begin, nsp, n, inv_spp, img, dimg, plane, counters, own, seed, term_g, off_term);
+}
+
+}
+
+namespace psdr_host {
+struct TermPlan { LaunchCtx cx; int lds, park, table, off_term; const uint32_t *term_g; };
+static bool term_plan(psdr_scene_s *h, const LaunchCtx &cx0, int cols, int waves, TermPlan &p) {
+    p.table = term_table_bytes(h);
+    if (p.table == 0) return false;
+    constexpr int kCuLds = 160 * 1024;
+    p.lds = (lds_bytes(cx0, h) + 15) / 16 * 16;
+    p.park = cols * kBlock * 4;
+    const int limit = h->opt.lds_budget > 0 ? std::min(h->opt.lds_budget, kCuLds / waves) : kCuLds / waves;
+    if (p.lds + p.park + p.table > limit) return false;
+    p.cx = cx0;
+    p.cx.off_park = p.lds;
+    p.off_term = p.lds + p.park;
+    p.term_g = h->d_term + (h->opt.terminal_rows == 2 ? h->desc.num_tris : 0);
+    return true;
+}
+
+int term_render_c_launch_8(psdr_scene_s *h, const psdr_render_opts *o, const LaunchCtx &cx0, float *img, hipStream_t s, bool *ran) {
+    *ran = false;
+    TermPlan p;
+    if (!term_plan(h, cx0, PSDR_TERM_PARK_C != 0 ? ParkLayout<0>::cols : 0, PSDR_WAVES_C_NOTREE, p)) return 0;
+    const long long WH = (long long) h->desc.width * h->desc.height;
+    const int nsp = o->spp_end - o->spp_begin;
+    const long long n = WH * nsp;
+    const int own = (h->opt.own_pixels != 0 && nsp <= 64 && 64 % nsp == 0) ? 1 : 0;
+    const dim3 grid(launch_blocks(h, n, camera_blocks_per_cu(h, n)));
+    const int bytes = p.lds + p.park + p.table;
+    const TangentView<0, kTermFlags> tv{};
+    const ulonglong2 *seed = seed_table(h, o, WH, nsp, n, s);
+    if (seed != nullptr)
+        hipLaunchKernelGGL(HIP_KERNEL_NAME(k_camera_term<true>), grid, dim3(kBlock), bytes, s, p.cx, tv, o->spp, o->spp_begin, SlotDiv(nsp), n, 1.f / (float) o->spp, img, h->d_counters, own, seed,
+                           p.term_g, p.off_term);
+    else
+        hipLaunchKernelGGL(HIP_KERNEL_NAME(k_camera_term<false>), grid, dim3(kBlock), bytes, s, p.cx, tv, o->spp, o->spp_begin, SlotDiv(nsp), n, 1.f / (float) o->spp, img, h->d_counters, own, seed,
+                           p.term_g, p.off_term);
+    if (seed != nullptr) h->seed_launches++;
+    h->term_c_launches++;
+    *ran = true;
+    return 0;
+}
+int term_logd_launch_8(psdr_scene_s *h, const psdr_render_opts *o, const LaunchCtx &cx0, const psdr::TangentView<1, psdr::kSceneTiny> &tv, float *img, float *dimg, hipStream_t s, bool *ran) {
+    *ran = false;
+    if (h->opt.logd_park == 0) return 0;
+    TermPlan p;
+    if (!term_plan(h, cx0, ParkLayout<1>::cols, PSDR_LOGD_WAVES_K1, p)) return 0;
+    const long long WH = (long long) h->desc.width * h->desc.height;
+    const int nsp = o->spp_end - o->spp_begin;
+    const long long n = WH * nsp;
+    const int own = (h->opt.own_pixels != 0 && nsp <= 64 && 64 % nsp == 0) ? 1 : 0;
+    const dim3 grid(launch_blocks(h, n, camera_blocks_per_cu(h, n)));
+    const int bytes = p.lds + p.park + p.table;
+    const ulonglong2 *seed = seed_table(h, o, WH, nsp, n, s);
+    if (seed != nullptr)
+        hipLaunchKernelGGL(HIP_KERNEL_NAME(k_camera_logd_term<true>), grid, dim3(kBlock), bytes, s, p.cx, tv, o->spp, o->spp_begin, SlotDiv(nsp), n, 1.f / (float) o->spp, img, dimg, WH * 3,
+                           h->d_counters, own, seed, p.term_g, p.off_term);
+    else
+        hipLaunchKernelGGL(HIP_KERNEL_NAME(k_camera_logd_term<false>), grid, dim3(kBlock), bytes, s, p.cx, tv, o->spp, o->spp_begin, SlotDiv(nsp), n, 1.f / (float) o->spp, img, dimg, WH * 3,
+                           h->d_counters, own, seed, p.term_g, p.off_term);
+    h->logd_lean_launches++;
+    if (seed != nullptr) { h->logd_lean_seeded++; h->seed_launches++; }
+    h->logd_lean_lds = p.lds; h->logd_lean_park = p.park + p.table;
+    h->term_d_launches++;
+    *ran = true;
+    return 0;
+}
+}
diff --git a/psdr-cuda_amd/psdr_cuda/_abi.py b/psdr-cuda_amd/psdr_cuda/_abi.py
--- a/psdr-cuda_amd/psdr_cuda/_abi.py
+++ b/psdr-cuda_amd/psdr_cuda/_abi.py
@@ -78,7 +78,7 @@
 HIP_SYMBOLS = (
     "psdr_last_error", "psdr_version", "psdr_abi_struct_sizes", "psdr_scene_create", "psdr_scene_destroy", "psdr_scene_set_option", "psdr_scene_set_tables",
     "psdr_bvh_build", "psdr_bvh_stats", "psdr_scene_info", "psdr_trace", "psdr_render_c", "psdr_render_d_fwd", "psdr_render_d_rev",
-    "psdr_guide_build", "psdr_get_counters", "psdr_scene_rev_layout", "psdr_scene_seed_info", "psdr_scene_logd_info",
+    "psdr_guide_build", "psdr_get_counters", "psdr_scene_rev_layout", "psdr_scene_seed_info", "psdr_scene_logd_info", "psdr_scene_term_info",
     "psdr_geo_world_vertices_fwd", "psdr_geo_world_vertices_rev", "psdr_geo_tri_rows_fwd", "psdr_geo_tri_rows_rev", "psdr_geo_sec_edges_fwd", "psdr_geo_sec_edges_rev", "psdr_geo_prim_edges_fwd", "psdr_geo_prim_edges_rev",
     "psdr_geo_compact_edges_fwd", "psdr_geo_compact_edges_rev", "psdr_geo_emitter_tables",
     "psdr_geo_world_vertices_jvp", "psdr_geo_tri_rows_jvp", "psdr_geo_sec_edges_jvp", "psdr_geo_prim_edges_jvp", "psdr_geo_compact_edges_jvp",
@@ -124,6 +124,7 @@
     lib.psdr_scene_rev_layout.argtypes = [vp, C.POINTER(i32)]
     lib.psdr_scene_seed_info.argtypes = [vp, C.POINTER(C.c_int64)]
     lib.psdr_scene_logd_info.argtypes = [vp, C.POINTER(C.c_int64)]
+    lib.psdr_scene_term_info.argtypes = [vp, C.POINTER(C.c_int64)]
     lib.psdr_geo_world_vertices_fwd.argtypes = [i32, vp, vp, vp, vp, vp]
     lib.psdr_geo_world_vertices_rev.argtypes = [i32, vp, vp, vp, vp, vp, vp, vp]
     lib.psdr_geo_tri_rows_fwd.argtypes = [i32, i32, vp, vp, vp, vp, i32, vp]
@@ -193,6 +194,13 @@
     return {"launches": int(out[0]), "lean": int(out[1]), "lean_seeded": int(out[2]), "lean_lds_bytes": int(out[3])}
 
 
+def term_info(handle):
+    lib = load_hip()
+    out = (C.c_int64 * 4)()
+    check(lib, lib.psdr_scene_term_info(handle, out))
+    return {"render_c": int(out[0]), "logd": int(out[1]), "table": int(out[2]), "max_rows": int(out[3])}
+
+
 def make_opts(integrator=INTEGRATOR_DIRECT, bsdf_samples=1, light_samples=1, max_depth=1, hide_emitters=False,
               field=0, spp=1, sppe=0, sppse=0, spp_range=None, sppe_range=None, sppse_range=None,
               rng_offset=(0, 0, 0), flags=0):
```
